# haoyuzhao123/CGRayTracing

Hardware: AMD Instinct MI355X
Metric: Mrays/sec (primary+secondary) at 1920x1080 spp=64 (higher is better)
Workload: dtype f64

## Files before the change

### cgraytracing_amd/_capi.py

```python
from __future__ import annotations

import ctypes as C
import os

import sys

_HERE = os.path.dirname(os.path.abspath(__file__))
CGRT_VERSION = 112
LIB_PATH = os.path.join(_HERE, "libcgrt.so")
if os.environ.get("CGRT_LIB"):
    if os.environ.get("CGRT_DEV_LIBS") == "1":
        LIB_PATH = os.environ["CGRT_LIB"]
        print("cgraytracing_amd: DEVELOPMENT library %s (CGRT_LIB + CGRT_DEV_LIBS=1)" % LIB_PATH, file=sys.stderr)
    else:
        print("cgraytracing_amd: CGRT_LIB ignored (set CGRT_DEV_LIBS=1 to load a development build)", file=sys.stderr)

CGRT_OK = 0
CGRT_NCOUNTERS = 8
CNT_RAYS, CNT_HITPOINTS, CNT_WAVE_ITERS, CNT_NODE_TESTS, CNT_TRI_TESTS = 0, 1, 2, 3, 4


class CgrtError(RuntimeError):
    def __init__(self, code, msg):
        super().__init__("libcgrt error %d: %s" % (code, msg))
# ... 99 lines not shown
    "cgrt_scene_add_mesh_triangles": (C.c_int, [C.c_void_p, C.c_void_p, C.c_int, _DP, C.c_double, C.c_double,
                                                C.c_int]),
    "cgrt_scene_add_bezier": (C.c_int, [C.c_void_p, C.c_void_p, C.c_int, _DP, _DP, C.c_double, C.c_double]),
    "cgrt_scene_commit": (C.c_int, [C.c_void_p, C.c_int]),
    "cgrt_scene_get_stats": (C.c_int, [C.c_void_p, C.POINTER(SceneStats)]),
    "cgrt_scene_tree_sizes": (C.c_int, [C.c_void_p, C.c_int, C.POINTER(C.c_int32), C.POINTER(C.c_int32),
                                        C.POINTER(C.c_int32)]),
    "cgrt_scene_tree_dump": (C.c_int, [C.c_void_p, C.c_int, C.c_void_p, C.c_void_p, C.c_void_p, C.c_void_p]),
    "cgrt_trace_grid": (C.c_int, [C.c_void_p, C.POINTER(Camera), C.POINTER(Grid), C.c_void_p, C.c_void_p,
                                  C.c_void_p, C.c_void_p]),
    "cgrt_unpermute_stripes": (C.c_int, [C.c_void_p, C.c_int, C.c_int, C.c_int, C.c_int, C.c_int, C.c_int, C.c_int, C.c_void_p,
                                         C.c_void_p]),
    "cgrt_trace_grid_host": (C.c_int, [C.c_void_p, C.POINTER(Camera), C.POINTER(Grid), C.c_void_p, C.c_void_p,
                                       C.c_void_p]),
    "cgrt_trace_grid_hitpoints": (C.c_int, [C.c_void_p, C.POINTER(Camera), C.POINTER(Grid), C.c_void_p, C.c_uint64,
                                            C.POINTER(C.c_uint64)]),
    "cgrt_ppm_render": (C.c_int, [C.c_void_p, C.POINTER(Camera), C.POINTER(Grid), C.POINTER(Photons),
                                  C.POINTER(PpmResult)]),
    "cgrt_ppm_session_create": (C.c_int, [C.c_void_p, C.POINTER(Camera), C.POINTER(Grid), C.POINTER(Photons), C.c_int,
                                          C.POINTER(C.c_void_p)]),
    "cgrt_ppm_session_create_rays": (C.c_int, [C.c_void_p, C.POINTER(Rays), C.POINTER(RayPixels), C.POINTER(Photons), C.c_int,
                                               C.POINTER(C.c_void_p)]),
    "cgrt_ppm_session_destroy": (None, [C.c_void_p]),
    "cgrt_ppm_session_add_photons": (C.c_int, [C.c_void_p, C.c_int64]),
    "cgrt_ppm_session_add_photon_rays": (C.c_int, [C.c_void_p, C.POINTER(PhotonRays)]),
    "cgrt_photon_emit": (C.c_int, [C.POINTER(Photons), C.c_int64, C.c_int64, C.c_void_p, C.c_void_p, C.c_void_p, C.c_void_p, C.c_void_p,
                                   C.c_void_p]),
    "cgrt_photon_emit_host": (C.c_int, [C.POINTER(Photons), C.c_int64, C.c_int64, C.c_void_p, C.c_void_p, C.c_void_p, C.c_void_p,
                                        C.c_void_p]),
    "cgrt_photon_ray_events": (C.c_int, [C.c_void_p, C.POINTER(PhotonRays), C.c_uint64, C.c_int64, C.c_int, C.c_void_p, C.c_void_p]),
    "cgrt_ppm_session_image": (C.c_int, [C.c_void_p, C.c_void_p, C.c_void_p]),
    "cgrt_ppm_session_image_device": (C.c_int, [C.c_void_p, C.c_void_p, C.c_void_p, C.c_void_p]),
    "cgrt_ppm_session_hitpoints": (C.c_int, [C.c_void_p, C.c_void_p, C.c_uint64, C.POINTER(C.c_uint64)]),
    "cgrt_ppm_session_get_info": (C.c_int, [C.c_void_p, C.POINTER(PpmSessionInfo)]),
    "cgrt_tonemap_rgb8": (C.c_int, [C.c_int, C.c_void_p, C.c_int, C.c_int, C.c_void_p]),
    "cgrt_write_png": (C.c_int, [C.c_char_p, C.c_int, C.c_int, C.c_void_p]),
    "cgrt_photon_events": (C.c_int, [C.c_void_p, C.POINTER(Photons), C.c_int, C.c_int64, C.c_int32, C.c_void_p,
                                     C.c_void_p]),
    "cgrt_scene_bvh_dump": (C.c_int, [C.c_void_p, C.c_int, C.POINTER(C.c_int32), C.c_void_p, C.c_void_p]),
    "cgrt_scene_bvh_order": (C.c_int, [C.c_void_p, C.c_int, C.POINTER(C.c_int32), C.c_void_p]),
    "cgrt_scene_wide_dump": (C.c_int, [C.c_void_p, C.c_int, C.POINTER(C.c_int32), C.POINTER(C.c_int32), C.c_void_p, C.c_void_p]),
    "cgrt_lens_samples": (C.c_int, [C.c_uint64, C.c_void_p, C.c_void_p, C.c_int, C.c_double, C.c_void_p]),
    "cgrt_surface_colors": (C.c_int, [C.c_void_p, C.c_int, C.c_void_p, C.c_int, C.c_void_p]),
    "cgrt_trace_grid_variant": (C.c_int, [C.c_void_p, C.POINTER(Camera), C.POINTER(Grid), C.c_char_p, C.c_size_t]),
    "cgrt_scene_last_tile_order": (C.c_int, [C.c_void_p, C.c_void_p, C.c_void_p, C.c_void_p, C.c_int64, C.POINTER(C.c_int64)]),
    "cgrt_scene_last_sphere_masks": (C.c_int, [C.c_void_p, C.c_void_p, C.c_int64, C.POINTER(C.c_int64)]),
    "cgrt_scene_last_sure_tiles": (C.c_int, [C.c_void_p, C.c_void_p, C.c_int64, C.POINTER(C.c_int64)]),
    "cgrt_scene_last_sample_relay": (C.c_int, [C.c_void_p, C.POINTER(C.c_int64), C.POINTER(C.c_int32), C.POINTER(C.c_int64)]),
    "cgrt_scene_last_relay_form": (C.c_int, [C.c_void_p, C.POINTER(C.c_int32), C.POINTER(C.c_int32)]),
    "cgrt_relay_start_host": (C.c_int, [C.c_int32, C.c_int32, C.c_int32, C.c_int64, C.c_int32, C.c_int64, C.c_int64, C.c_int64, C.c_void_p,
                                        C.c_void_p, C.c_int32, C.c_int32, C.c_void_p, C.c_int64, C.POINTER(C.c_int64)]),
    "cgrt_scene_last_relay_start": (C.c_int, [C.c_void_p, C.c_void_p, C.c_int64, C.c_void_p, C.c_int64, C.POINTER(C.c_int64),
                                              C.POINTER(C.c_int64), C.POINTER(C.c_int32)]),
    "cgrt_scene_last_lens_stage": (C.c_int, [C.c_void_p, C.POINTER(C.c_int64), C.POINTER(C.c_int64)]),
    "cgrt_scene_last_tile_order_reused": (C.c_int, [C.c_void_p, C.POINTER(C.c_int32)]),
    "cgrt_trace_grid_diffuse_variant": (C.c_int, [C.c_void_p, C.c_void_p, C.c_void_p, C.c_char_p, C.c_size_t]),
    "cgrt_scene_last_diffuse_tiles": (C.c_int, [C.c_void_p, C.POINTER(C.c_int64)]),
    "cgrt_scene_last_inkernel_diffuse_tiles": (C.c_int, [C.c_void_p, C.POINTER(C.c_int64)]),
    "cgrt_trace_rays": (C.c_int, [C.c_void_p, C.POINTER(Rays), C.POINTER(RayResults), C.c_void_p, C.c_void_p]),
    "cgrt_trace_rays_host": (C.c_int, [C.c_void_p, C.POINTER(Rays), C.POINTER(RayResults), C.c_void_p]),
    "cgrt_ray_hit_attributes": (C.c_int, [C.c_void_p, C.POINTER(Rays), C.c_void_p, C.c_void_p, C.POINTER(HitAttributes), C.c_void_p]),
    "cgrt_ray_hit_attributes_host": (C.c_int, [C.c_void_p, C.POINTER(Rays), C.c_void_p, C.c_void_p, C.POINTER(HitAttributes)]),
    "cgrt_trace_rays_variant": (C.c_int, [C.c_void_p, C.POINTER(Rays), C.POINTER(RayResults), C.c_char_p, C.c_size_t]),
    "cgrt_trace_rays_hitpoints": (C.c_int, [C.c_void_p, C.POINTER(Rays), C.c_void_p, C.c_uint64, C.POINTER(C.c_uint64)]),
    "cgrt_occlusion_rays": (C.c_int, [C.c_void_p, C.POINTER(Rays), C.POINTER(Occlusion), C.c_void_p, C.c_void_p]),
    "cgrt_occlusion_rays_host": (C.c_int, [C.c_void_p, C.POINTER(Rays), C.POINTER(Occlusion), C.c_void_p]),
    "cgrt_occlusion_rays_variant": (C.c_int, [C.c_void_p, C.POINTER(Rays), C.c_char_p, C.c_size_t]),
    "cgrt_camera_rays": (C.c_int, [C.POINTER(Camera), C.POINTER(Grid), C.c_void_p, C.c_void_p, C.c_void_p, C.c_void_p]),
    "cgrt_camera_rays_host": (C.c_int, [C.POINTER(Camera), C.POINTER(Grid), C.c_void_p, C.c_void_p, C.c_void_p]),
    "cgrt_intersect_rays": (C.c_int, [C.c_void_p, C.c_int, C.c_void_p, C.c_void_p, C.c_void_p, C.c_int,
                                      C.c_void_p, C.c_void_p, C.c_void_p]),
    "cgrt_math_probe": (C.c_int, [C.c_int, C.c_int, C.c_void_p, C.c_int64, C.c_void_p]),
}

_lib = None


def lib():
    global _lib
    if _lib is None:
        if not os.path.exists(LIB_PATH):
            raise ImportError(
                "cgraytracing_amd: %s not found -- build the HIP library first "
                "(make -C cgraytracing_amd/csrc, or __graft_entry__.build()). There is no CPU fallback." % LIB_PATH)
        try:
            import torch
        except ImportError:
            pass
        L = C.CDLL(LIB_PATH)
        for name, (res, args) in SIGNATURES.items():
            fn = getattr(L, name)
            fn.restype = res
            fn.argtypes = args
        if L.cgrt_version() != CGRT_VERSION:
            raise ImportError("cgraytracing_amd: %s is ABI version %d, this binding needs %d -- rebuild it (make -C cgraytracing_amd/csrc)"
                              % (LIB_PATH, L.cgrt_version(), CGRT_VERSION))
        _lib = L
    return _lib


def check(rc):
    if rc < 0:
        raise CgrtError(rc, lib().cgrt_last_error().decode("utf-8", "replace"))
    return rc
```

### cgraytracing_amd/csrc/cgrt_eye.hpp

```cpp
#ifndef CGRT_EYE_HPP
#define CGRT_EYE_HPP
#include "cgrt_lens_stage.h"
#include "cgrt_scene_walk.hpp"
#include "cgrt_sphere_mask.h"
#include "cgrt_sure_first.h"

struct Pending {
    V3 o, d, adj;
    int32_t depth_left;
    uint32_t path;
};

#ifndef CGRT_DIFF_WAVES
#define CGRT_DIFF_WAVES 8
#endif
#ifndef CGRT_DIFF_DOF_WAVES
#define CGRT_DIFF_DOF_WAVES 6
#endif
static constexpr int kDiffWaves = CGRT_DIFF_WAVES, kDiffDofWaves = CGRT_DIFF_DOF_WAVES;
#ifndef CGRT_BEZ_WAVES
#define CGRT_BEZ_WAVES 2
#endif
static constexpr int kBezWaves = CGRT_BEZ_WAVES;
#ifndef CGRT_TREE_WAVES
#define CGRT_TREE_WAVES 3
#endif
#ifndef CGRT_SCHED_TREE_WAVES
#define CGRT_SCHED_TREE_WAVES CGRT_TREE_WAVES
#endif
static constexpr int kTreeWaves = CGRT_TREE_WAVES;
static constexpr int kSchedTreeWaves = CGRT_SCHED_TREE_WAVES;

__host__ __device__ __forceinline__ void lens_disc(uint64_t k_smp, double &sx, double &sy) {
    uint64_t ctr = k_smp;
    while (true) {
        ctr += kGolden;
        const uint64_t z = fin64(ctr);
        const double ux = div_rand_max((uint32_t)(z >> 33)), uy = div_rand_max((uint32_t)((z >> 2) & 0x7fffffffu));
        sx = ux * 2.0 - 1;
        sy = uy * 2.0 - 1;
        if (sx * sx + sy * sy < 1) break;
    }
}

struct HitpointSink {
    double *rec;
    unsigned long long *count;
    unsigned long long cap;
};

template <int NT>
__device__ __forceinline__ bool wave_has_tile(const GridParams &g, int tile_block, int tile_grid) {
    using TG = TileGeom<NT>;
    const int wave = threadIdx.x >> 6;
    const int wtiles_x = (g.W + kWaveTileW - 1) / kWaveTileW, wtiles_y = (g.rows + kWaveTileH - 1) / kWaveTileH;
    int tile_x, tile_y;
    if (tile_grid < 0) {
        const int tiles_x = (g.W + TG::W - 1) / TG::W;
        tile_x = tile_block % tiles_x;
        tile_y = tile_block / tiles_x;
    } else {
        const int tile_blocks = tile_grid / g.chunks;
        if (!tile_of_block(g, tile_block % tile_blocks, tile_x, tile_y, TG::W, TG::H)) return false;
    }
    const int wx = tile_x * (TG::W / kWaveTileW) + (NT == 256 ? (wave & 1) : 0);
    const int wy = tile_y * (TG::H / kWaveTileH) + (NT == 256 ? (wave >> 1) : 0);
    if (!(wx < wtiles_x && wy < wtiles_y)) return false;
    if (g.hidx && g.hidx[wy * wtiles_x + wx] >= 0) return false;
    if (g.light && (g.light[wy * wtiles_x + wx] != 0) != (g.light_mode != 0)) return false;
    return true;
}

struct RelayWg {
    int slot = -1, chunk = 0, s0 = 0, s1 = 0;
};

template <bool TREES, bool BEZ, bool DOF, bool GLASS, bool SPH, bool STATS, bool HPS, int NT, bool HEAVY, bool SPILL = false, bool HFONLY = false,
          bool DIFF = false, bool PAIR = false, bool PARK = false, bool LSTAGE = false, bool COST = false>
__device__ __forceinline__ void trace_grid_body(const DeviceScene &sc, const GridParams &g, float *__restrict__ rgb,
                                                uint32_t *__restrict__ nhit_out, unsigned long long *__restrict__ counters,
                                                const HitpointSink &hps, int tile_block, int tile_grid, const RelayWg rw = RelayWg{}) {
    using TG = TileGeom<NT>;
    static_assert(!PARK || (PAIR && NT == kRelayThreads), "PARK: a relayed tile's later chunks");
    static_assert(!DIFF || (SPH && !GLASS && !HPS && !HEAVY && !STATS && !SPILL), "DIFF: the sphere loop, first hits only");
    static_assert(!PAIR || (SPH && GLASS && !HPS && !HEAVY && !STATS && !SPILL), "PAIR: the glass sphere variants of the tile order");
    static_assert(!LSTAGE || (DIFF && DOF && !PAIR), "LSTAGE: the thin-lens terminal-diffuse body inside a PAIR launch");
    static_assert(!COST || PAIR, "COST: the PAIR variants with a start table");
    static_assert(!LSTAGE || lens_batch_lds(NT) <= (size_t)kLdsLevels * pending_level_bytes(NT), "the lens batches fit the PAIR launch's pending-ray levels");
    const long long tl_t0 = g.timeline ? wall_clock64() : 0;
    if (!HEAVY && !g.timeline) {
        if (!__syncthreads_or((int)wave_has_tile<NT>(g, tile_block, tile_grid))) return;
    }
    constexpr size_t level_bytes = pending_level_bytes(NT), stack_bytes = (size_t)kLdsLevels * level_bytes;
    constexpr bool WALK = TREES && !HFONLY;
    {
        constexpr WgLds chk = wg_lds(wg_ask_trace(NT, TREES, BEZ, GLASS, SPILL, HFONLY), 3, 5, true);
        static_assert(chk.pending == 0 && chk.objs == (GLASS ? stack_bytes : 0) && chk.staging - chk.objs == 3 * sizeof(ObjRec) &&
                          chk.bez - chk.staging == (SPILL ? (NT / 64) * sizeof(ObjRec) : 0) &&
                          chk.nodes - chk.bez == (BEZ ? (NT / 64) * sizeof(BezLds) : 0) &&
                          chk.wstack - chk.nodes == (WALK ? 5 * sizeof(NodeRec) : 0) && chk.has.nodes == WALK &&
                          chk.has.wstack == (WALK && !GLASS && !BEZ),
                      "trace_grid_body's carve-up and cgrt_wg_lds.h");
    }
    extern __shared__ __align__(16) unsigned char lds_raw[];
    ObjRec *lobjs = reinterpret_cast<ObjRec *>(lds_raw + (GLASS ? stack_bytes : 0));
    unsigned char *lrest = reinterpret_cast<unsigned char *>(lobjs + sc.n_lds);
    LdsAux aux;
    if (SPILL) {
        aux.spill = reinterpret_cast<ObjRec *>(lrest) + (threadIdx.x >> 6);
        lrest += (NT / 64) * sizeof(ObjRec);
    }
    aux.bl = BEZ ? reinterpret_cast<volatile BezLds *>(lrest) + (threadIdx.x >> 6) : nullptr;
    if (BEZ) lrest += (NT / 64) * sizeof(BezLds);
    NodeRec *lnodes = reinterpret_cast<NodeRec *>(lrest);
    aux.lnodes = (WALK && sc.cached_tree >= 0) ? lnodes : nullptr;
    aux.wstack = (WALK && !GLASS && !BEZ && sc.has_wide)
                     ? reinterpret_cast<uint2 *>(lrest + ((sc.cached_tree >= 0 ? (size_t)sc.cached_nodes * sizeof(NodeRec) : 0)))
                     : nullptr;
    if (WALK && sc.cached_tree >= 0) {
        const uint4 *src = reinterpret_cast<const uint4 *>(sc.nodes + sc.trees[sc.cached_tree].node_begin);
        uint4 *dst = reinterpret_cast<uint4 *>(lnodes);
        const int n16 = sc.cached_nodes * (int)(sizeof(NodeRec) / 16);
        for (int k = threadIdx.x; k < n16; k += NT) dst[k] = src[k];
    }

    {
        const uint4 *src = reinterpret_cast<const uint4 *>(sc.objs);
        uint4 *dst = reinterpret_cast<uint4 *>(lobjs);
// ... 22 lines not shown
        live = have_tile && (w < g.W) && (j < g.rows) && (h < g.H);
        const double px = (2.0 * ((double)w / g.W) - 1) * g.half_width;
        const double py = (2.0 * ((double)h / g.H) - 1) * g.half_width * g.H / g.W;
        pdir = normalized(mk(px, py, 0) - camorg);
        pof = pdir * ((g.focus_plane - camorg.z) / pdir.z) + camorg;
        k_pix = pixel_key(g.seed, (uint64_t)h * (uint64_t)g.W + (uint64_t)w);
    };
    if (!heavy) {
        const int nb = tile_block;
        int tile_x, tile_y;
        if (tile_grid < 0) {
            const int tiles_x = (g.W + TG::W - 1) / TG::W;
            tile_x = nb % tiles_x;
            tile_y = nb / tiles_x;
        } else {
            const int tile_blocks = tile_grid / g.chunks;
            chunk = nb / tile_blocks;
            if (!tile_of_block(g, nb % tile_blocks, tile_x, tile_y, TG::W, TG::H)) return;
        }
        wx = tile_x * (TG::W / kWaveTileW) + (NT == 256 ? (wave & 1) : 0);
        wy = tile_y * (TG::H / kWaveTileH) + (NT == 256 ? (wave >> 1) : 0);
        have_tile = wx < wtiles_x && wy < wtiles_y;
        if (have_tile && g.hidx && g.hidx[wy * wtiles_x + wx] >= 0) have_tile = false;
        if (have_tile && g.light && (g.light[wy * wtiles_x + wx] != 0) != (g.light_mode != 0)) have_tile = false;
        s_end = (g.chunks > 1) ? ((chunk + 1) * g.chunk_spp < g.spp ? (chunk + 1) * g.chunk_spp : g.spp) : (PAIR && rw.slot >= 0 ? rw.s1 : g.spp);
        set_pixel(lane & 15, lane >> 4);
    }
    const bool masked = DIFF && g.wmask != nullptr;
    uint32_t smask = 0u;
    if (masked) {
        smask = load_uniform(g.wmask + __builtin_amdgcn_readfirstlane(have_tile ? wy * wtiles_x + wx : 0));
        if (sc.n_lds < 32) smask &= (1u << sc.n_lds) - 1u;
    }
    uint32_t sure = (uint32_t)kSureNone;
    if (DIFF && g.wsure != nullptr && have_tile) {
        const uint32_t wt = (uint32_t)__builtin_amdgcn_readfirstlane(wy * wtiles_x + wx);
        sure = (load_uniform(reinterpret_cast<const uint32_t *>(g.wsure) + (wt >> 2)) >> ((wt & 3u) * 8u)) & 0xffu;
        if (sure >= (uint32_t)sc.n_lds) sure = (uint32_t)kSureNone;
    }
    uint64_t k_smp = 0;

    double acc_r = 0, acc_g = 0, acc_b = 0;
    uint32_t my_hits = 0, my_rays = 0, my_nodes = 0, my_tris = 0, wave_iters = 0;
    uint32_t hp_seq = 0;

    Pending deep[2];
    Pending sib;
    bool sib_valid = false;
    unsigned char *lslot = lds_raw;
    int sp = 0;
    int s = (g.chunks > 1) ? chunk * g.chunk_spp : (PAIR && rw.slot >= 0 ? rw.s0 : 0);
    double *park = nullptr;
    uint32_t park_n = 0;
    if (PARK)
        park = reinterpret_cast<double *>(g.relay + relay_layout((size_t)g.relay_cap, g.relay_k, g.relay_slots).rvals) +
               ((size_t)rw.slot * (size_t)(g.relay_k - 1) + (size_t)(rw.chunk - 1)) * (size_t)g.relay_slots * (3 * NT) + threadIdx.x;
    bool have = false;
    V3 o = camorg, d = pdir, adj = mk(1, 1, 1);
    int depth_left = 0;
    uint32_t path = 1;
    int unit_next = 0, unit_end = 0, hrank = 0;
    int unit_pix = 0, unit_smp = 0, unit_rank = 0;
    bool unit_open = false;
    constexpr bool PRE = HEAVY && TREES && !BEZ && !STATS && !SPILL;
    bool pre_valid = false;
    double pre_len = 0;
    int32_t pre_tri = -1;

    const bool staging = LSTAGE && g.lens_batch != 0;
    uint64_t *const lens_slot = reinterpret_cast<uint64_t *>(lrest) + threadIdx.x;
    static_assert(lens_slot_at(1, 0, NT) == NT * sizeof(uint64_t) && lens_slot_at(0, 1, NT) == sizeof(uint64_t), "lens_slot's strides");
    int batch_first = 0, batch_end = 0;
    auto stage_lens = [&](int first, int count) {
        uint32_t rejected = 0u;
        for (int b = 0; b < count; b++) {
            const LensSlot a = lens_stage_first(k_pix, (uint64_t)(g.sample_offset + first + b));
            lens_slot[b * NT] = a.v;
            rejected |= a.done ? 0u : (1u << b);
        }
        if (!live) rejected = 0u;
        while (__ballot(rejected != 0u) != 0ull) {
            if (rejected != 0u) {
                const int b = __ffs((int)rejected) - 1;
                const LensSlot a = lens_stage_retry(lens_slot[b * NT]);
                lens_slot[b * NT] = a.v;
                if (a.done) rejected &= rejected - 1u;
            }
        }
        batch_first = first;
        batch_end = first + count;
    };
    auto start_sample = [&](int smp) {
        if (LSTAGE && staging) {
            double sx, sy;
            lens_point(lens_slot[(smp - batch_first) * NT], sx, sy);
            o = camorg + mk(sx, sy, 0) * g.lens_radius;
            d = normalized(pof - o);
            k_smp = 0;
        } else if (DOF) {
            k_smp = sample_key(k_pix, (uint64_t)(g.sample_offset + smp));
            double sx, sy;
            lens_disc(k_smp, sx, sy);
            o = camorg + mk(sx, sy, 0) * g.lens_radius;
            d = normalized(pof - o);
        } else {
            k_smp = sample_key(k_pix, (uint64_t)(g.sample_offset + smp));
            o = camorg;
            d = pdir;
        }
// ... 92 lines not shown
            if (!have && live && s < s_end) {
                start_sample(s);
                s++;
            }
            if (__ballot(have) == 0ull) break;
        }
        wave_iters++;
        UTILP(heavy ? 0 : 11, have);
        RayKey rk{k_smp, path, false, 0u};
        if (PRE) {
            rk.pre_valid = have && pre_valid;
            rk.pre_obj = g.prim_obj;
            rk.pre_len = pre_len;
            rk.pre_tri = pre_tri;
            rk.pre_counter = pre_tri >= 0 ? 1 : 0;
            pre_valid = false;
        }
        const SceneHit hit =
            intersect_scene<TREES, BEZ, SPH, STATS, SPILL, PRE, HFONLY, !SPH, PAIR, DIFF>(lobjs, sc.n_lds, sc.n_objs, sc, o, d, rk, have, aux, my_nodes, my_tris,
                                                                                          masked, smask);
        if (have) {
            my_rays++;
            have = false;
            if (hit.id >= 0) {
                const ObjMat ob = load_mat<SPILL>(lobjs, sc.n_lds, sc.objs, hit.id);
                V3 P = o, n = d, n_old = d;
                bool into = true;
                auto surface = [&]() {
                    P = o + d * hit.t;
                    n = SPH ? normalized(P - load_centre<SPILL>(lobjs, sc.n_lds, sc.objs, hit.id)) : hit.n;
                    n_old = n;
                    into = true;
                    if (dot(n, d) > 0) {
                        n = -n;
                        into = false;
                    }
                };
                if (!SPH) surface();
                V3 f = ob.col;
                if (!SPH && ob.kind == KIND_PLANE && ob.tex >= 0) {
                    V3 c;
                    if (texture_color(sc.texs[ob.tex], sc.texels, P, c)) f = c;
                }
                const double refl = ob.refl, transp = ob.transp;
                if (DIFF || (refl < kEps && transp < kEps)) {
                    UTIL(heavy ? 7 : 12);
                    const V3 hf = DIFF ? f : mulv(f, adj);
                    if (heavy) {
                        double *q = g.dvals + ((((size_t)unit_rank * g.spp + unit_smp) * g.maxhp + hp_seq) * 64 + unit_pix) * 3;
                        q[0] = hf.x;
                        q[1] = hf.y;
                        q[2] = hf.z;
                    } else if (PARK) {
                        if (park_n < (uint32_t)g.relay_slots) {
                            double *q = park + (size_t)park_n * (3 * NT);
                            q[0] = hf.x;
                            q[NT] = hf.y;
                            q[2 * NT] = hf.z;
                        }
                        park_n++;
                    } else {
                        acc_r += hf.x;
                        acc_g += hf.y;
                        acc_b += hf.z;
                    }
                    my_hits++;
                    if (HPS && SPH) surface();
                    if (HPS) {
                        const unsigned long long here = __ballot(true);
                        unsigned long long base = 0ull;
                        if (lane == (int)__ffsll((long long)here) - 1) base = atomicAdd(hps.count, (unsigned long long)__popcll(here));
                        base = (unsigned long long)__shfl((long long)base, (int)__ffsll((long long)here) - 1);
                        const unsigned long long k = base + (unsigned long long)__popcll(here & lanes_below);
                        if (k < hps.cap) {
                            double *q = hps.rec + 10 * k;
                            q[0] = hf.x; q[1] = hf.y; q[2] = hf.z;
                            q[3] = P.x; q[4] = P.y; q[5] = P.z;
                            q[6] = n.x; q[7] = n.y; q[8] = n.z;
                            q[9] = (double)((((unsigned long long)(s - 1) * (unsigned long long)g.W * g.rows +
                                              (unsigned long long)j * g.W + w) << 4) | (unsigned long long)hp_seq);
                        }
                    }
                    if (HPS || heavy) hp_seq++;
                } else if (depth_left > 1) {
                    if (SPH) surface();
                    if (transp < kEps) {
                        const V3 nd = d - n * 2.0 * dot(n, d);
                        adj = mulv(f, adj) * refl;
                        o = P + n * kEps;
                        d = nd;
                        depth_left--;
                        path = path * 2;
                        have = true;
                    } else if (GLASS) {
                        UTIL(heavy ? 8 : 13);
                        const double nc = 1.0, nt = 1.33;
                        const double nnt = into ? nc / nt : nt / nc;
                        const double ddn = dot(d, n);
                        const V3 refl_dir = d - n_old * 2.0 * dot(n_old, d);
                        const double cos2t = 1 - nnt * nnt * (1 - ddn * ddn);
                        if (cos2t < 0) {
                            o = P + n * kEps;
                            d = refl_dir;
                        } else {
                            const V3 refr_dir =
                                normalized(d * nnt - n_old * ((into ? 1 : -1) * (ddn * nnt + sqrt_cr(cos2t))));
                            const double a = nt - nc, b = nt + nc, R0 = a * a / (b * b);
// ... 38 lines not shown
                d = sib.d;
                adj = sib.adj;
                depth_left = sib.depth_left;
                path = sib.path;
                sib_valid = false;
                have = true;
            }
            if (GLASS && !have && sp > 0) {
                UTIL(heavy ? 10 : 14);
                --sp;
                if (sp < kLdsLevels) {
                    const double *q = reinterpret_cast<const double *>(lslot + sp * level_bytes) + threadIdx.x;
                    o = mk(q[0 * NT], q[1 * NT], q[2 * NT]);
                    d = mk(q[3 * NT], q[4 * NT], q[5 * NT]);
                    adj = mk(q[6 * NT], q[7 * NT], q[8 * NT]);
                    const uint32_t meta = reinterpret_cast<const uint32_t *>(
                        lslot + sp * level_bytes + kPendDoubles * NT * sizeof(double))[threadIdx.x];
                    depth_left = (int)(meta >> 8);
                    path = meta & 0xffu;
                } else {
                    const Pending &pe = deep[sp - kLdsLevels];
                    o = pe.o;
                    d = pe.d;
                    adj = pe.adj;
                    depth_left = pe.depth_left;
                    path = pe.path;
                }
                have = true;
            }
        }
    }

    if (g.probe) {
        if (lane == 0 && have_tile) {
            const long long dt = (long long)clock64() - cost_t0;
            const uint32_t wt = (uint32_t)(wy * wtiles_x + wx);
            g.cost[wt] = (COST && g.probe == 2) ? wave_iters : dt > 0 ? (dt < 0xffffffffll ? (uint32_t)dt : 0xffffffffu) : 1u;
        }
        return;
    }
    if (heavy) {
    } else if (g.chunks > 1) {
        if (have_tile && (w < g.W) && (j < g.rows)) {
            const size_t px = ((size_t)chunk * g.rows + (size_t)j) * g.W + (size_t)w;
            g.partial[3 * px + 0] = acc_r;
            g.partial[3 * px + 1] = acc_g;
            g.partial[3 * px + 2] = acc_b;
            if (g.partial_nhit) g.partial_nhit[px] = my_hits;
        }
    } else {
        uint32_t px_hits = my_hits;
        bool store = true;
        if (PAIR && rw.slot >= 0) {
            const size_t slot = (size_t)rw.slot, k = (size_t)g.relay_k;
            const RelayLayout rl = relay_layout((size_t)g.relay_cap, g.relay_k, g.relay_slots);
            uint32_t *arrive = reinterpret_cast<uint32_t *>(g.relay) + slot;
            double *racc = reinterpret_cast<double *>(g.relay + rl.racc) + slot * (3 * NT) + threadIdx.x;
            uint32_t *rhits = reinterpret_cast<uint32_t *>(g.relay + rl.rhits) + slot * k * NT + threadIdx.x;
            uint32_t *rcount = reinterpret_cast<uint32_t *>(g.relay + rl.rcount) + slot * (k - 1) * NT + threadIdx.x;
            if (PARK) {
                rcount[(size_t)(rw.chunk - 1) * NT] = park_n;
            } else {
                racc[0] = acc_r;
                racc[NT] = acc_g;
                racc[2 * NT] = acc_b;
            }
            rhits[(size_t)rw.chunk * NT] = my_hits;
            __shared__ unsigned int relay_last;
            asm volatile("s_waitcnt vmcnt(0)" ::: "memory");
            __syncthreads();
            if (threadIdx.x == 0) {
                __builtin_amdgcn_fence(__ATOMIC_RELEASE, "agent");
                asm volatile("s_waitcnt vmcnt(0)" ::: "memory");
                const unsigned int ticket = __hip_atomic_fetch_add(arrive, 1u, __ATOMIC_RELAXED, __HIP_MEMORY_SCOPE_AGENT);
                const bool last = ticket == (unsigned int)g.relay_k - 1u;
                if (last) {
                    __builtin_amdgcn_fence(__ATOMIC_ACQUIRE, "agent");
                    asm volatile("s_waitcnt vmcnt(0)" ::: "memory");
                    __hip_atomic_store(arrive, 0u, __ATOMIC_RELAXED, __HIP_MEMORY_SCOPE_AGENT);
                }
                relay_last = last ? 1u : 0u;
            }
            __syncthreads();
            store = relay_last != 0u;
            if (store) {
                acc_r = racc[0];
                acc_g = racc[NT];
                acc_b = racc[2 * NT];
                px_hits = rhits[0];
                for (int c = 1; c < g.relay_k; c++) {
                    px_hits += rhits[(size_t)c * NT];
                    uint32_t n = rcount[(size_t)(c - 1) * NT];
                    if (n > (uint32_t)g.relay_slots) n = (uint32_t)g.relay_slots;
                    uint32_t n_max = n;
                    for (int off = 32; off > 0; off >>= 1) {
                        const uint32_t o2 = (uint32_t)__shfl_xor((int)n_max, off);
                        n_max = o2 > n_max ? o2 : n_max;
                    }
                    n_max = (uint32_t)__builtin_amdgcn_readfirstlane((int)n_max);
                    const double *q = reinterpret_cast<const double *>(g.relay + rl.rvals) +
                                      (slot * (k - 1) + (size_t)(c - 1)) * (size_t)g.relay_slots * (3 * NT) + threadIdx.x;
                    for (uint32_t i0 = 0; i0 < n_max; i0 += kRelayBatch) {
                        double v[kRelayBatch][3];
#pragma unroll
                        for (int u = 0; u < kRelayBatch; u++) {
                            v[u][0] = q[(size_t)(i0 + u) * (3 * NT)];
                            v[u][1] = q[(size_t)(i0 + u) * (3 * NT) + NT];
                            v[u][2] = q[(size_t)(i0 + u) * (3 * NT) + 2 * NT];
                        }
#pragma unroll
                        for (int u = 0; u < kRelayBatch; u++) {
                            if (i0 + u < n) {
                                acc_r += v[u][0];
                                acc_g += v[u][1];
                                acc_b += v[u][2];
                            }
                        }
                    }
                }
            }
        }
        const float v0 = (float)(acc_r * g.inv_spp_total), v1 = (float)(acc_g * g.inv_spp_total),
                    v2 = (float)(acc_b * g.inv_spp_total);
#pragma unroll
        for (int k = 0; k < 3; k++) {
            const int idx = k * 64 + lane;
            const int row = idx / (kWaveTileW * 3), c = idx % (kWaveTileW * 3);
            const int src = row * kWaveTileW + c / 3, ch = c % 3;
            const float a0 = __shfl(v0, src), a1 = __shfl(v1, src), a2 = __shfl(v2, src);
            const float v = ch == 0 ? a0 : (ch == 1 ? a1 : a2);
            const int jj = wy * kWaveTileH + row, ww = wx * kWaveTileW + c / 3;
            if (store && have_tile && jj < g.rows && ww < g.W) {
                float *dst = rgb + ((size_t)jj * g.W + ww) * 3 + ch;
                *dst = g.accumulate ? *dst + v : v;
            }
        }
        if (store && nhit_out && have_tile && (w < g.W) && (j < g.rows)) nhit_out[(size_t)j * g.W + w] = px_hits;
    }

    if (g.timeline) {
        __shared__ unsigned int tl_rays;
        if (threadIdx.x == 0) tl_rays = 0;
        __syncthreads();
        atomicAdd(&tl_rays, my_rays);
        __syncthreads();
        if (threadIdx.x == 0) {
            unsigned long long *q = g.timeline + 4 * (size_t)blockIdx.x;
            const unsigned hw = __builtin_amdgcn_s_getreg((31 << 11) | 4), xcc = __builtin_amdgcn_s_getreg((3 << 11) | 20);
            if (q[0] == 0ull) q[0] = (unsigned long long)tl_t0;
            q[1] = (unsigned long long)wall_clock64();
            q[2] = (unsigned long long)hw | ((unsigned long long)xcc << 32);
            q[3] = ((unsigned long long)(wx & 0xffff) | ((unsigned long long)(wy & 0xffff) << 16)) + ((q[3] >> 32) << 32) + ((unsigned long long)tl_rays << 32);
        }
    }
    if (counters) {
        unsigned long long r = my_rays, hh = my_hits, nn = my_nodes, tt = my_tris;
        for (int off = 32; off > 0; off >>= 1) {
            r += __shfl_xor(r, off);
            hh += __shfl_xor(hh, off);
            if (STATS) {
                nn += __shfl_xor(nn, off);
                tt += __shfl_xor(tt, off);
            }
        }
        if (lane == 0 && (r | (unsigned long long)wave_iters) != 0ull) {
            atomicAdd(&counters[CGRT_CNT_RAYS], r);
            atomicAdd(&counters[CGRT_CNT_HITPOINTS], hh);
            atomicAdd(&counters[CGRT_CNT_WAVE_ITERS], (unsigned long long)wave_iters);
            if (STATS) {
                atomicAdd(&counters[CGRT_CNT_NODE_TESTS], nn);
                atomicAdd(&counters[CGRT_CNT_TRI_TESTS], tt);
            }
        }
    }
}

__device__ __forceinline__ unsigned long long *wg_counters_begin(unsigned long long *wg, const unsigned long long *counters) {
    if (!counters) return nullptr;
    if (threadIdx.x < CGRT_NCOUNTERS) wg[threadIdx.x] = 0ull;
    __syncthreads();
    return wg;
}
__device__ __forceinline__ void wg_counters_end(const unsigned long long *wg, unsigned long long *counters) {
    if (!counters) return;
    __syncthreads();
    if (threadIdx.x < CGRT_NCOUNTERS && wg[threadIdx.x] != 0ull) atomicAdd(&counters[threadIdx.x], wg[threadIdx.x]);
}

template <bool TREES, bool BEZ, bool DOF, bool GLASS, bool SPH, bool STATS, bool HPS = false, int NT = 256, bool SPILL = false, bool HFONLY = false,
          bool DIFF = false, bool PAIR = false, bool START = false>
__global__ __launch_bounds__(NT, DIFF ? (DOF ? kDiffDofWaves : kDiffWaves) : BEZ ? kBezWaves : ((TREES && !HFONLY) ? kTreeWaves : 4)) void trace_grid_kernel(DeviceScene sc, GridParams g, float *__restrict__ rgb,
                                                             uint32_t *__restrict__ nhit_out,
                                                             unsigned long long *__restrict__ counters,
                                                             HitpointSink hps = HitpointSink{nullptr, nullptr, 0}) {
    int tile_block = (int)blockIdx.x, tile_grid = (int)gridDim.x;
    unsigned entry = blockIdx.x;
    RelayWg rw;
    if (g.tile_order) {
        if (g.tile_order == kOrderFull || g.tile_order == kOrderDiffuse) {
            const unsigned first_diffuse = load_uniform(g.plan + 3);
            if (g.tile_order == kOrderDiffuse) entry += first_diffuse;
            if (g.tile_order == kOrderDiffuse ? entry >= load_uniform(g.plan + kOrderClasses) : entry >= first_diffuse) return;
        } else if (PAIR && g.relay_k > 1) {
            const unsigned n_tiles = load_uniform(g.plan + kOrderClasses);
            const unsigned n01 = load_uniform(g.plan + 2), n012 = load_uniform(g.plan + 3);
            RelayBlock rb{n_tiles, 0, false};
            bool tabled = false;
            if (START && g.relay_start_at != 0u) {
                const unsigned n_split = relay_split_entries(n01, n012, (unsigned)g.relay_cap, g.relay_extent);
                tabled = blockIdx.x < n012 + ((unsigned)g.relay_k - 1u) * n_split;
                if (tabled) {
                    rb = relay_start_block(load_uniform(g.plan + g.relay_start_at + blockIdx.x), n_split);
                    if (rb.chunk >= g.relay_k) return;
                }
            }
            if (!tabled) rb = relay_block_ordered(blockIdx.x, (unsigned)g.relay_k, n01, n012, n_tiles, (unsigned)g.relay_cap, g.relay_extent, g.relay_order);
            entry = rb.entry;
            if (entry >= n_tiles) return;
            if (rb.split) {
                rw.slot = (int)entry;
                rw.chunk = rb.chunk;
                rw.s0 = relay_first_sample(rb.chunk, g.relay_chunk_spp);
                rw.s1 = relay_end_sample(rb.chunk, g.relay_chunk_spp, g.spp);
            }
        }
        tile_block = (int)load_uniform(g.border + entry);
        tile_grid = -1;
    }
    __shared__ unsigned long long wg_cnt[CGRT_NCOUNTERS];
    unsigned long long *wc = wg_counters_begin(wg_cnt, counters);
    if (PAIR && g.tile_order == kOrderAllDiffuse && entry >= load_uniform(g.plan + 3))
        trace_grid_body<false, false, DOF, false, true, false, false, NT, false, false, false, true, false, false, DOF>(sc, g, rgb, nhit_out, wc, hps, tile_block, tile_grid);
    else if (PAIR && rw.chunk > 0)
        trace_grid_body<TREES, BEZ, DOF, GLASS, SPH, STATS, HPS, NT, false, SPILL, HFONLY, DIFF, PAIR, PAIR, false, START>(sc, g, rgb, nhit_out, wc, hps, tile_block, tile_grid, rw);
    else
        trace_grid_body<TREES, BEZ, DOF, GLASS, SPH, STATS, HPS, NT, false, SPILL, HFONLY, DIFF, PAIR, false, false, START>(sc, g, rgb, nhit_out, wc, hps, tile_block, tile_grid, rw);
    wg_counters_end(wg_cnt, counters);
}
template <bool TREES, bool BEZ, bool DOF, bool GLASS, bool SPH, bool STATS, int NT = 256>
__global__ __launch_bounds__(NT, BEZ ? kBezWaves : (TREES ? kSchedTreeWaves : 4)) void trace_grid_sched_kernel(DeviceScene sc, GridParams g,
                                                                                         float *__restrict__ rgb,
                                                                                         uint32_t *__restrict__ nhit_out,
                                                                                         unsigned long long *__restrict__ counters) {
    const HitpointSink none{nullptr, nullptr, 0};
    const bool heavy_first = (int)blockIdx.x < g.heavy_blocks;
    __shared__ unsigned long long wg_cnt[CGRT_NCOUNTERS];
    unsigned long long *wc = wg_counters_begin(wg_cnt, counters);
    if (NT == 64) {
        if (heavy_first)
            trace_grid_body<TREES, BEZ, DOF, GLASS, SPH, STATS, false, NT, true>(sc, g, rgb, nhit_out, wc, none, 0, 1);
        else
            trace_grid_body<TREES, BEZ, DOF, GLASS, SPH, STATS, false, NT, false>(sc, g, rgb, nhit_out, wc, none,
                                                                                  (int)blockIdx.x - g.heavy_blocks,
                                                                                  (int)gridDim.x - g.heavy_blocks);
        wg_counters_end(wg_cnt, counters);
        return;
    }
    const bool queued = g.border != nullptr;
    __shared__ unsigned tile_entry;
    for (int phase = 0; phase < 2; phase++) {
        if ((phase == 0) == heavy_first) {
            if (queued || heavy_first)
                trace_grid_body<TREES, BEZ, DOF, GLASS, SPH, STATS, false, NT, true>(sc, g, rgb, nhit_out, wc, none, 0, 1);
        } else {
            const unsigned n_entries = queued ? load_uniform(g.plan + 3) : (heavy_first ? 0u : 1u);
            unsigned served = 0;
            while (true) {
                unsigned e = served++;
                if (queued) {
                    __syncthreads();
                    if (threadIdx.x == 0) tile_entry = atomicAdd(&g.plan[4], 1u);
                    __syncthreads();
                    e = tile_entry;
                }
                if (e >= n_entries) break;
                trace_grid_body<TREES, BEZ, DOF, GLASS, SPH, STATS, false, NT, false>(
// ... 140 lines not shown
__global__ __launch_bounds__(256) void sure_first_kernel(GridParams g, DeviceScene sc, int tiles_x, const unsigned char *__restrict__ tcls,
                                                         const uint32_t *__restrict__ wmask, unsigned char *__restrict__ wsure) {
    const int wtiles_x = (g.W + kWaveTileW - 1) / kWaveTileW, wtiles_y = (g.rows + kWaveTileH - 1) / kWaveTileH;
    const int wt = blockIdx.x * blockDim.x + threadIdx.x;
    if (wt >= wtiles_x * wtiles_y) return;
    const int wx = wt % wtiles_x, wy = wt / wtiles_x;
    int win = -1;
    if (tcls[(wy / (kTileH / kWaveTileH)) * tiles_x + wx / (kTileW / kWaveTileW)] == 3) {
        const TileRays tr = wave_tile_rays(g, wx, wy);
        const ObjRec *objs = sc.objs;
        win = sphere_sure_first(g, tr, sc.n_objs, [objs](int i) { return SureSphere{vec3d(objs[i].a[0], objs[i].a[1], objs[i].a[2]), objs[i].s0}; },
                                wmask[wt]);
    }
    wsure[wt] = (unsigned char)(win >= 0 ? win : kSureNone);
}

struct RelayStartArgs {
    RelayItems r;
    uint32_t tiles_x, wtiles_x, wtiles_y;
};
__device__ __forceinline__ RelayItems relay_items_of(const RelayStartArgs &a, const uint32_t *plan) {
    RelayItems r = a.r;
    r.n01 = plan[2];
    r.n012 = plan[3];
    r.n_tiles = plan[kOrderClasses];
    return r;
}
__global__ __launch_bounds__(kRelayThreads) void relay_weight_kernel(RelayStartArgs a, const uint32_t *__restrict__ plan, const uint32_t *__restrict__ list,
                                                                     const uint32_t *__restrict__ wcost, unsigned long long *__restrict__ weight) {
    const RelayItems r = relay_items_of(a, plan);
    const uint32_t i = blockIdx.x * kRelayThreads + threadIdx.x;
    if (i >= relay_items_total(r)) return;
    const RelayBlock b = relay_item(i, r);
    weight[i] = relay_item_weight(b, relay_tile_cost(wcost, list[b.entry], a.tiles_x, a.wtiles_x, a.wtiles_y), r);
}
__global__ __launch_bounds__(kRelayThreads) void relay_start_kernel(RelayStartArgs a, const uint32_t *__restrict__ plan,
                                                                    const unsigned long long *__restrict__ weight, uint32_t *__restrict__ start) {
    const RelayItems r = relay_items_of(a, plan);
    const uint32_t t = relay_items_total(r), i = blockIdx.x * kRelayThreads + threadIdx.x;
    if (blockIdx.x * kRelayThreads >= t) return;
    __shared__ unsigned long long w_s[kRelayThreads];
    const unsigned long long wi = i < t ? weight[i] : 0ull;
    uint32_t rank = 0;
    for (uint32_t j0 = 0; j0 < t; j0 += kRelayThreads) {
        __syncthreads();
        if (j0 + threadIdx.x < t) w_s[threadIdx.x] = weight[j0 + threadIdx.x];
        __syncthreads();
        const uint32_t n = min((uint32_t)kRelayThreads, t - j0);
        for (uint32_t u = 0; u < n; u++) rank += relay_item_before(w_s[u], j0 + u, wi, i) ? 1u : 0u;
    }
    if (i < t) start[rank] = relay_start_word(relay_item(i, r));
}

__global__ __launch_bounds__(1024) void plan_kernel(const uint32_t *__restrict__ cost_in, const unsigned char *__restrict__ light, int n,
                                                    unsigned kmax, unsigned long long divisor, uint32_t *__restrict__ plan,
                                                    uint32_t *__restrict__ order, int32_t *__restrict__ hidx,
                                                    uint32_t *__restrict__ border, int wtiles_x, int wtiles_y, int tw, int th) {
    auto cost = [&](int i) -> uint32_t { return (light && light[i]) ? 0u : cost_in[i]; };
    __shared__ unsigned long long part[1024];
    __shared__ unsigned base_s, hist[128];
    __shared__ unsigned long long thr_s;
    auto bin_of = [](uint32_t c) { return c < 4u ? (int)c : (31 - __clz((int)c)) * 4 + (int)((c >> (29 - __clz((int)c))) & 3u); };
    if (threadIdx.x < 128) hist[threadIdx.x] = 0;
    __syncthreads();
    unsigned long long t = 0;
    for (int i = threadIdx.x; i < n; i += 1024) {
        const uint32_t c = cost(i);
        t += c;
        atomicAdd(&hist[bin_of(c)], 1u);
    }
    part[threadIdx.x] = t;
    __syncthreads();
    for (int off = 512; off > 0; off >>= 1) {
        if ((int)threadIdx.x < off) part[threadIdx.x] += part[threadIdx.x + off];
        __syncthreads();
    }
    if (threadIdx.x == 0) {
        unsigned long long thr = part[0] / divisor;
        if (thr < 1) thr = 1;
        unsigned above = 0;
        int b = 127;
        for (; b >= 0; b--) {
            if (above + hist[b] > kmax) break;
            above += hist[b];
        }
        if (b >= 0) {
            const unsigned long long edge = b < 4 ? (unsigned long long)b
                                                  : (((4ull + (unsigned long long)(b & 3) + 1ull) << (b / 4)) >> 2) - 1ull;
            if (edge > thr) thr = edge;
        }
        thr_s = thr;
        base_s = 0;
    }
    __syncthreads();
    const unsigned long long thr = thr_s;
    if (threadIdx.x == 0) {
        unsigned off = 0;
        for (int b = 127; b >= 0; b--) {
            const unsigned long long lo = b < 4 ? (unsigned long long)b : ((4ull + (unsigned long long)(b & 3)) << (b / 4)) >> 2;
            const unsigned c = hist[b];
            if (lo > thr) {
                hist[b] = off;
                off += c;
            } else {
                hist[b] = 0xffffffffu;
            }
// ... 200 lines not shown
```

### cgraytracing_amd/csrc/cgrt_frame.h

```cpp
#ifndef CGRT_FRAME_H
#define CGRT_FRAME_H
#include <algorithm>
#include <cmath>
#include <cstddef>
#include <cstdint>
#include <cstdio>
#include <cstdlib>
#include <string>

#include "../../include/cgrt.h"
#include "cgrt_lens_stage.h"
#include "cgrt_relay.h"

struct GridParams {
    int32_t W, H, rows, row_offset, stripe_rows, stripe_rank, stripe_nranks;
    int32_t spp, sample_offset, max_depth;
    int32_t accumulate;
    int32_t xcd_tiles;
    int32_t chunks, chunk_spp;
    double *partial;
    uint32_t *partial_nhit;
    const unsigned char *light;
    int32_t light_mode, tile_order;
    const uint32_t *wmask;
    const uint32_t *order;
    const uint32_t *border;
    uint32_t *cost;
    const int32_t *hidx;
    uint32_t *plan;
    double *dvals;
    unsigned char *dcnt;
    double *pconst;
    int32_t probe, heavy_blocks, items_per_tile, units_per_item, maxhp;
    const double *prim_len;
    const int32_t *prim_tri;
    int32_t prim_obj;
    int32_t prim_done;
    int32_t pw_refill, pw_rounds;
    unsigned long long *timeline;
    double inv_spp_total;
    uint64_t seed;
    double cam[3], half_width, focus_plane, lens_radius;
    unsigned char *relay;
    int32_t relay_k, relay_chunk_spp, relay_cap, relay_slots;
    int32_t relay_extent, relay_order;
    int32_t lens_batch;
    uint32_t relay_start_at;
    const unsigned char *wsure;
};
static_assert(sizeof(GridParams) == 336, "GridParams is a kernel argument: its layout is fixed");

static constexpr int kTileW = 32, kTileH = 8, kThreads = 256;
static constexpr int kOrderSpheresMax = 16, kOrderClasses = 4, kOrderPlanWords = 8, kOrderArrived = 5;
static constexpr int kOrderAll = 1, kOrderFull = 2, kOrderDiffuse = 3, kOrderAllDiffuse = 4;
struct OrderSpheres {
    double s[kOrderSpheresMax][4];
    uint32_t n, transp;
};
static constexpr size_t align256(size_t b) { return (b + 255) & ~(size_t)255; }
struct Region {
    size_t at, bytes;
    template <class T> T *in(unsigned char *base) const { return bytes ? reinterpret_cast<T *>(base + at) : nullptr; }
};
struct TileOrderLayout {
    Region plan{}, list{}, tile_cls{}, wave_cls{}, wmask{}, wsure{};
    Region wcost{}, weight{}, start{};
    size_t total = 0;
};
inline TileOrderLayout tile_order_layout(size_t n_tiles, size_t n_wt, bool sure = false, size_t start_words = 0) {
    TileOrderLayout L;
    size_t end = 0;
    const auto take = [&end](size_t bytes) { end += bytes; return Region{end - bytes, bytes}; };
    L.plan = take(kOrderPlanWords * sizeof(uint32_t));
    L.list = take(n_tiles * sizeof(uint32_t));
    end = align256(end);
    L.tile_cls = take(n_tiles);
    end = align256(end);
    L.wave_cls = take(n_wt);
    end = align256(end);
    L.wmask = take(n_wt * sizeof(uint32_t));
    if (sure) {
        end = align256(end);
        L.wsure = take(n_wt);
    }
    if (start_words) {
        end = align256(end);
        L.wcost = take(n_wt * sizeof(uint32_t));
        end = align256(end);
        L.weight = take(start_words * sizeof(uint64_t));
        end = align256(end);
        L.start = take(start_words * sizeof(uint32_t));
    }
    L.total = align256(end);
    return L;
}
static constexpr int kSphereMaskMax = 32;
inline bool order_all_special(const OrderSpheres &sp, const cgrt_camera &cam) {
    for (uint32_t i = 0; i < sp.n; i++) {
        double r = sp.s[i][3] * (1 + 1e-9) + 1e-6;
        if (cam.lens_radius > 0) {
            const double f = cam.focus_plane - cam.cam[2];
            const double s_lo = (sp.s[i][2] - r - cam.cam[2]) / f, s_hi = (sp.s[i][2] + r - cam.cam[2]) / f;
            if (!(f > 0) || !(s_lo > 0) || !(cam.cam[2] < 0)) return true;
            r += cam.lens_radius * std::max(std::fabs(1 - s_lo), std::fabs(1 - s_hi));
        }
        const double vx = sp.s[i][0] - cam.cam[0], vy = sp.s[i][1] - cam.cam[1], vz = sp.s[i][2] - cam.cam[2];
        if (!(std::sqrt(vx * vx + vy * vy + vz * vz) > r)) return true;
    }
    return false;
}
static constexpr int kWaveTileW = 16, kWaveTileH = 4;
static constexpr int kXcds = 8, kSuperW = 4, kSuperH = 4, kSuperTiles = kSuperW * kSuperH;

inline int tile_grid_blocks(int W, int rows, bool xcd_tiles, int tile_w = kTileW, int tile_h = kTileH) {
    const int tiles_x = (W + tile_w - 1) / tile_w, tiles_y = (rows + tile_h - 1) / tile_h;
    if (!xcd_tiles) return tiles_x * tiles_y;
    const int sx = (tiles_x + kSuperW - 1) / kSuperW, sy = (tiles_y + kSuperH - 1) / kSuperH;
    const int nsuper = sx * sy;
    return ((nsuper + kXcds - 1) / kXcds) * kXcds * kSuperTiles;
}

inline GridParams grid_params(const cgrt_camera *cam, const cgrt_grid *grid) {
    GridParams g{};
    g.W = grid->width;
    g.H = grid->height;
    g.rows = grid->rows;
    g.row_offset = grid->row_offset;
    g.stripe_rows = grid->stripe_rows;
    g.stripe_rank = grid->stripe_rank;
    g.stripe_nranks = grid->stripe_nranks;
    g.spp = grid->spp;
    g.sample_offset = grid->sample_offset;
    g.max_depth = grid->max_depth;
    g.accumulate = (grid->flags & CGRT_GRID_ACCUMULATE) ? 1 : 0;
    g.inv_spp_total = 1.0 / (double)grid->spp_total;
    g.seed = grid->seed;
    for (int k = 0; k < 3; k++) g.cam[k] = cam->cam[k];
    g.half_width = cam->half_width;
    g.focus_plane = cam->focus_plane;
    g.lens_radius = cam->lens_radius;
    g.chunks = 1;
    g.chunk_spp = grid->spp;
    g.items_per_tile = 1;
    g.units_per_item = 256;
    g.maxhp = 16;
    g.prim_obj = -1;
    g.pw_refill = 16;
    g.pw_rounds = 8;
    return g;
}

struct EyeKnobs {
    bool force_reorder = false;
    long long defer_bytes = 0;
    int heavy_div = 32, units_per_item = 256;
    bool no_primwalk = false, pw_no_finish = false;
    int pw_refill = 16, pw_rounds = 8;
    int lds_pad = 0;
    bool no_hfonly = false, no_tile_queue = false, plan_dump = false;
    bool no_sure_tiles = false;
    bool no_order_reuse = false;
    int relay_chunks = kRelayDefaultChunks;
    long long relay_tiles = 0;
    int relay_mirror = -1;
    int relay_order = -1;
    int relay_start = -1;
    int relay_probe_spp = kRelayProbeSpp;
    int lens_stage = -1;
    const char *timeline_file = nullptr;
};
inline const char *env_str(const char *name) { const char *e = std::getenv(name); return e ? e : ""; }
inline bool env_on(const char *name) { const char *e = env_str(name); return *e && *e != '0'; }
inline int env_positive(const char *name, int def) { const int v = std::atoi(env_str(name)); return v > 0 ? v : def; }
inline int relay_order_named(const char *e) {
    const std::string v(e);
    if (v == "chunks_first" || v == "0") return kRelayChunksFirst;
    if (v == "mirror_first" || v == "1") return kRelayMirrorFirst;
    if (v == "interleaved" || v == "2") return kRelayInterleaved;
    return -1;
}
inline int relay_start_named(const char *e) {
    const std::string v(e);
    if (v == "list" || v == "0") return kRelayStartList;
    if (v == "cost" || v == "1") return kRelayStartCost;
    return -1;
}
static constexpr int kLensStageOff = 0, kLensStageLds = 1;
static constexpr int kLensStageDefault = kLensStageLds;
inline int lens_stage_named(const char *e) {
    const std::string v(e);
    if (v == "off" || v == "0") return kLensStageOff;
    if (v == "lds" || v == "1") return kLensStageLds;
    return -1;
}
inline EyeKnobs eye_knobs() {
    static const EyeKnobs once = [] {
        EyeKnobs k;
        k.force_reorder = env_on("CGRT_FORCE_REORDER");
        k.defer_bytes = std::atoll(env_str("CGRT_DEFER_BYTES"));
        k.heavy_div = env_positive("CGRT_HEAVY_DIV", 32);
        k.units_per_item = (env_positive("CGRT_UNITS_PER_ITEM", 256) + 63) / 64 * 64;
        k.no_primwalk = env_on("CGRT_NO_PRIMWALK");
        k.pw_no_finish = env_on("CGRT_PW_NO_FINISH");
        k.pw_refill = env_positive("CGRT_PW_REFILL", 16);
        k.pw_rounds = env_positive("CGRT_PW_ROUNDS", 8);
        k.lds_pad = std::atoi(env_str("CGRT_LDS_PAD"));
        k.no_hfonly = env_on("CGRT_NO_HFONLY");
        k.no_tile_queue = env_on("CGRT_NO_TILE_QUEUE");
        k.plan_dump = env_on("CGRT_PLAN_DUMP");
        k.no_order_reuse = env_on("CGRT_NO_ORDER_REUSE");
        k.no_sure_tiles = env_on("CGRT_NO_SURE_TILES");
        k.relay_chunks = std::min(std::max(env_positive("CGRT_RELAY_CHUNKS", kRelayDefaultChunks), 2), kRelayMaxChunks);
        k.relay_tiles = std::atoll(env_str("CGRT_RELAY_TILES"));
        if (*env_str("CGRT_RELAY_MIRROR")) k.relay_mirror = env_on("CGRT_RELAY_MIRROR") ? 1 : 0;
        k.relay_order = relay_order_named(env_str("CGRT_RELAY_ORDER"));
        k.relay_start = relay_start_named(env_str("CGRT_RELAY_START"));
        if (k.relay_start < 0 && *env_str("CGRT_RELAY_START"))
            std::fprintf(stderr, "cgrt: CGRT_RELAY_START=%s names no start order of this library (list, cost): the default is used\n", env_str("CGRT_RELAY_START"));
        {
            const int ps = std::atoi(env_str("CGRT_RELAY_PROBE_SPP"));
            if (ps == 1 || ps == 2 || ps == 4) k.relay_probe_spp = ps;
        }
        k.lens_stage = lens_stage_named(env_str("CGRT_LENS_STAGE"));
        if (k.lens_stage < 0 && *env_str("CGRT_LENS_STAGE"))
            std::fprintf(stderr, "cgrt: CGRT_LENS_STAGE=%s names no form of this library (off, lds): the default is used\n", env_str("CGRT_LENS_STAGE"));
        return k;
    }();
    EyeKnobs k = once;
    k.timeline_file = *env_str("CGRT_TIMELINE_FILE") ? env_str("CGRT_TIMELINE_FILE") : nullptr;
    return k;
}

struct FrameInputs {
    cgrt_grid grid;
    cgrt_camera cam;
    bool sched, spill, stats, glass;
    int nt;
    bool has_mesh, has_bezier, prim_finish, light_ok;
    int prim_obj;
    EyeKnobs knobs;
    size_t mem_total;
    int n_cu, waves_per_simd;
    bool image = false, sph = false, pair = false;
    bool order_ok = false, aux_stream = false, all_spheres = false;
    int n_objs = 0, n_lds = 0;
    bool all_special = false;
};

struct ScratchLayout {
    Region partial{}, partial_nhit{}, cost{}, order{}, hidx{}, border{}, plan{}, light{}, dvals{}, dcnt{}, pconst{}, prim_len{}, prim_tri{};
    size_t total = 0;
    void place(GridParams &g, unsigned char *base, bool nhit) const {
        g.partial = partial.in<double>(base);
        g.partial_nhit = nhit ? partial_nhit.in<uint32_t>(base) : nullptr;
        g.cost = cost.in<uint32_t>(base);
        g.order = order.in<uint32_t>(base);
        g.hidx = hidx.in<int32_t>(base);
        g.border = border.in<uint32_t>(base);
        g.plan = plan.in<uint32_t>(base);
        g.light = light.in<unsigned char>(base);
        g.dvals = dvals.in<double>(base);
        g.dcnt = dcnt.in<unsigned char>(base);
        g.pconst = pconst.in<double>(base);
        g.prim_len = prim_len.in<double>(base);
        g.prim_tri = prim_tri.in<int32_t>(base);
    }
};

struct TileOrderPlan {
    bool on = false;
    enum Class3 { None, SecondLaunch, InKernel } class3 = None;
    bool masks = false;
    bool sure = false;
    int lens_stage = kLensStageOff;
};

struct FramePlan {
    int chunks = 1, chunk_spp = 0;
    bool xcd_tiles = false;
    int maxhp = 1;
    int tile_blocks = 0;
    size_t grid_dim = 0;
    int wtiles_x = 0, wtiles_y = 0;
    size_t n_wt = 0, tile_bytes = 0, kmax = 0;
    bool use_prim = false;
    bool split_light = false, tile_queue = false, prim_done = false;
    int wave_slots = 0, items_per_tile = 1, heavy_blocks = 0;
    unsigned long long plan_div = 0;
    ScratchLayout scratch;
    TileOrderPlan order;
    int relay_k = 1, relay_chunk_spp = 0, relay_slots = 0;
    size_t relay_tile_bytes = 0, relay_cap = 0, relay_bytes = 0;
    int relay_extent = kRelayGlass, relay_order = kRelayChunksFirst;
    int relay_start = kRelayStartList, relay_probe_spp = 0;
    size_t relay_start_words = 0;
};

inline bool relay_engaged(int32_t flags, int32_t spp, size_t n_tiles, int n_cu) {
    if ((flags & CGRT_GRID_NO_SAMPLE_RELAY) || spp < 2 * kRelayMinChunkSpp) return false;
    return (flags & CGRT_GRID_SAMPLE_RELAY) || n_tiles >= (size_t)4 * (size_t)n_cu;
}

static constexpr int kRelayDefaultExtent = kRelayMirror, kRelayDefaultOrder = kRelayInterleaved;
inline int relay_extent_of(int32_t flags, const EyeKnobs &kn) {
    if (flags & CGRT_GRID_RELAY_MIRROR) return kRelayMirror;
    if (flags & CGRT_GRID_RELAY_NO_MIRROR) return kRelayGlass;
    if (kn.relay_mirror >= 0) return kn.relay_mirror ? kRelayMirror : kRelayGlass;
    return (flags & CGRT_GRID_SAMPLE_RELAY) ? kRelayGlass : kRelayDefaultExtent;
}
inline int relay_order_of(int32_t flags, const EyeKnobs &kn) {
    const int32_t f = flags & CGRT_GRID_RELAY_ORDER_MASK;
    if (f) return f == CGRT_GRID_RELAY_MIRROR_FIRST ? kRelayMirrorFirst : f == CGRT_GRID_RELAY_INTERLEAVED ? kRelayInterleaved : kRelayChunksFirst;
    if (kn.relay_order >= 0) return kn.relay_order;
    return (flags & CGRT_GRID_SAMPLE_RELAY) ? kRelayChunksFirst : kRelayDefaultOrder;
}

inline int relay_start_of(int32_t flags, const EyeKnobs &kn) {
    if (flags & CGRT_GRID_NO_RELAY_COST_START) return kRelayStartList;
    if (flags & CGRT_GRID_RELAY_COST_START) return kRelayStartCost;
    if (kn.relay_start >= 0) return kn.relay_start;
    const bool names_order = (flags & CGRT_GRID_RELAY_ORDER_MASK) || kn.relay_order >= 0;
    return !names_order && !(flags & CGRT_GRID_SAMPLE_RELAY) ? kRelayStartCost : kRelayStartList;
}

inline FramePlan frame_plan(const FrameInputs &in, size_t kmax) {
    const cgrt_grid &gr = in.grid;
    const EyeKnobs &kn = in.knobs;
    FramePlan p;
    p.chunk_spp = gr.spp;
    p.xcd_tiles = !in.spill && in.has_mesh && !in.has_bezier;
    p.maxhp = in.glass ? 16 : 1;
    const size_t npx = (size_t)gr.rows * gr.width;
    if ((gr.flags & CGRT_GRID_SPLIT_SAMPLES) && gr.spp >= 32 && !in.spill) {
        int chunks = std::min(gr.spp / 16, 16);
        while (chunks > 1 && (size_t)chunks * npx * 28 > ((size_t)4 << 30)) chunks--;
        if (chunks > 1) {
            p.chunk_spp = (gr.spp + chunks - 1) / chunks;
            p.chunks = (gr.spp + p.chunk_spp - 1) / p.chunk_spp;
        }
    }
    const bool one_wave = in.nt == 64;
    const int waves_per_block = in.nt / 64;
    p.tile_blocks = one_wave ? tile_grid_blocks(gr.width, gr.rows, false, kWaveTileW, kWaveTileH)
                             : tile_grid_blocks(gr.width, gr.rows, p.xcd_tiles);
    p.grid_dim = (size_t)p.tile_blocks * p.chunks;
    TileOrderPlan &o = p.order;
    const bool split_asked = (gr.flags & CGRT_GRID_SPLIT_SAMPLES) != 0;
    o.on = in.image && p.chunks == 1 && !p.xcd_tiles && in.nt == kThreads && in.order_ok && !(gr.flags & CGRT_GRID_NO_TILE_ORDER);
    if (o.on && !in.all_special) {
        if (in.sph && !in.spill && !in.stats && in.aux_stream && (gr.flags & CGRT_GRID_DIFFUSE_TILES) && !split_asked && !kn.timeline_file)
            o.class3 = TileOrderPlan::SecondLaunch;
        else if (in.pair)
            o.class3 = TileOrderPlan::InKernel;
    }
    o.masks = o.class3 != TileOrderPlan::None && in.all_spheres && in.n_objs <= kSphereMaskMax && in.n_objs == in.n_lds &&
              !(gr.flags & CGRT_GRID_NO_SPHERE_MASKS);
    o.sure = o.masks && !(gr.flags & CGRT_GRID_NO_SURE_TILES) && !kn.no_sure_tiles;
    if (o.class3 == TileOrderPlan::InKernel && in.cam.lens_radius > 0 && !(gr.flags & CGRT_GRID_NO_LENS_STAGE))
        o.lens_stage = kn.lens_stage >= 0 ? kn.lens_stage : kLensStageDefault;
    if (o.on && in.pair && o.class3 != TileOrderPlan::SecondLaunch && !split_asked &&
        relay_engaged(gr.flags, gr.spp, (size_t)p.tile_blocks, in.n_cu)) {
        const RelayChunks rc = relay_chunks(gr.spp, (gr.flags & CGRT_GRID_SAMPLE_RELAY_4) ? kRelayMaxChunks : kn.relay_chunks);
        if (rc.k > 1) {
            p.relay_slots = relay_slots(rc.chunk_spp, gr.max_depth);
            p.relay_tile_bytes = relay_tile_bytes(rc.k, p.relay_slots);
            p.relay_cap = relay_cap((size_t)p.tile_blocks, rc.k, p.relay_slots, relay_budget(in.mem_total), kn.relay_tiles);
            if (p.relay_cap > 0) {
                p.relay_k = rc.k;
                p.relay_chunk_spp = rc.chunk_spp;
                p.relay_bytes = relay_layout(p.relay_cap, rc.k, p.relay_slots).total;
                p.relay_extent = relay_extent_of(gr.flags, kn);
                p.relay_order = relay_order_of(gr.flags, kn);
                p.relay_start = (size_t)p.tile_blocks < kRelayStartMaxTiles ? relay_start_of(gr.flags, kn) : kRelayStartList;
                if (p.relay_start == kRelayStartCost) {
                    p.relay_probe_spp = std::min(kn.relay_probe_spp, (int)gr.spp);
                    p.relay_start_words = relay_start_words((size_t)p.tile_blocks, rc.k, p.relay_cap);
                }
            }
        }
    }
    p.wtiles_x = (gr.width + kWaveTileW - 1) / kWaveTileW;
    p.wtiles_y = (gr.rows + kWaveTileH - 1) / kWaveTileH;
    p.n_wt = (size_t)p.wtiles_x * p.wtiles_y;
    p.use_prim = in.sched && in.prim_obj >= 0 && !kn.no_primwalk && !(gr.flags & CGRT_GRID_STATS);
    const size_t units = (size_t)gr.spp * 64;
    const size_t vals = units * (size_t)p.maxhp * 3 * sizeof(double), cnt = (units + 7) & ~(size_t)7, pconst = 7 * 64 * sizeof(double),
                 plen = p.use_prim ? units * sizeof(double) : 0, ptri = p.use_prim ? units * sizeof(int32_t) : 0;
    p.tile_bytes = vals + cnt + pconst + plen + ptri;
    p.kmax = in.sched ? kmax : 0;

    ScratchLayout &L = p.scratch;
    size_t end = 0;
    const auto take = [&end](size_t bytes, bool used = true) { end += bytes; return Region{end - bytes, used ? bytes : 0}; };
    if (p.chunks > 1) {
        L.partial = take((size_t)p.chunks * npx * 3 * sizeof(double));
        L.partial_nhit = take((size_t)p.chunks * npx * sizeof(uint32_t));
    }
    L.total = end = align256(end);
    if (!in.sched) return p;
    const size_t np = (p.n_wt + 8) * sizeof(uint32_t), sched_bytes = align256(4 * np + 64 * sizeof(uint32_t) + align256(p.n_wt));
    L.total += sched_bytes + (p.kmax ? p.kmax * p.tile_bytes + 256 : 0);
    if (p.kmax == 0) return p;
    p.split_light = in.light_ok && p.chunks == 1 && !in.stats;
    p.tile_queue = p.chunks == 1 && !one_wave && !kn.no_tile_queue;
    p.prim_done = p.use_prim && in.prim_finish && !kn.pw_no_finish;
    p.wave_slots = in.n_cu * 4 * in.waves_per_simd;
    p.plan_div = (unsigned long long)p.wave_slots * (unsigned long long)kn.heavy_div;
    p.items_per_tile = (int)((units + kn.units_per_item - 1) / kn.units_per_item);
    const size_t fill = (size_t)p.wave_slots / waves_per_block;
    p.heavy_blocks = (int)std::min((p.kmax * (size_t)p.items_per_tile + waves_per_block - 1) / waves_per_block, fill);
    if (p.tile_queue) p.grid_dim = fill;
    const size_t sched_at = end;
    L.cost = take(np);
    L.order = take(np);
    L.hidx = take(np);
    L.border = take(np, p.tile_queue);
    L.plan = take(64 * sizeof(uint32_t));
    L.light = take(p.n_wt, p.split_light);
    end = sched_at + sched_bytes;
    L.dvals = take(p.kmax * vals);
    L.dcnt = take(p.kmax * cnt);
    L.pconst = take(p.kmax * pconst);
    L.prim_len = take(p.kmax * plen);
    L.prim_tri = take(p.kmax * ptri);
    return p;
}

inline size_t max_heavy_tiles(const FrameInputs &in) {
    if (!in.sched) return 0;
// ... 31 lines not shown
```

### cgraytracing_amd/csrc/cgrt_hip.hip

```cpp
#include <hip/hip_runtime.h>

#include <algorithm>
#include <atomic>
#include <chrono>
#include <cmath>
#include <cstdio>
#include <cstdlib>
#include <cstring>
#include <exception>
#include <map>
#include <mutex>
#include <string>
#include <type_traits>
#include <vector>

#include "../../include/cgrt.h"
#include "cgrt_build.h"
#include "cgrt_rng.hpp"
#include "cgrt_types.h"

#include "cgrt_device_math.hpp"
#include "cgrt_grid.hpp"
#include "cgrt_traverse.hpp"
#include "cgrt_bezier.hpp"
// ... 752 lines not shown
    in.pair = L.k.pair;
    in.order_ok = s->order.ok;
    in.aux_stream = s->aux_stream != nullptr;
    in.all_spheres = d.all_spheres != 0;
    in.n_objs = d.n_objs;
    in.n_lds = d.n_lds;
    in.all_special = order_all_special(s->order.spheres, *cam);
    return in;
}

static int probe_and_plan(const cgrt_scene *s, const EyeLaunch &L, const EyeKnobs &kn, const FramePlan &p, const GridParams &g,
                          unsigned char *scratch, hipStream_t st, float *rgb, uint32_t *nhit, unsigned long long *cnt) {
    const ScratchLayout &at = p.scratch;
    unsigned char *light = at.light.in<unsigned char>(scratch);
    if (light)
        hipLaunchKernelGGL(classify_kernel, dim3((unsigned)((p.n_wt + 255) / 256)), dim3(256), 0, st, s->dev, g, light, (int)p.n_wt);
    GridParams gp = g;
    gp.spp = gp.chunks = gp.chunk_spp = 1;
    gp.probe = 1;
    gp.cost = at.cost.in<uint32_t>(scratch);
    gp.light = light;
    int rc = launch_eye(L, false, s->device, gp, dim3((unsigned)p.tile_blocks), st, nullptr, nullptr, nullptr);
    if (rc) return rc;
    if (light) {
        GridParams gl = g;
        gl.light = light;
        gl.light_mode = 1;
        gl.xcd_tiles = 0;
        HIP_TRY(hipEventRecord(s->ev_fork, st));
        HIP_TRY(hipStreamWaitEvent(s->aux_stream, s->ev_fork, 0));
        if ((rc = launch_eye(light_launch(s->dev, L.k.dof, kn), false, s->device, gl,
                             dim3((unsigned)tile_grid_blocks(g.W, g.rows, false)), s->aux_stream, rgb, nhit, cnt)))
            return rc;
        HIP_TRY(hipEventRecord(s->ev_join, s->aux_stream));
    }
    const int tw = L.k.nt == 64 ? 1 : kTileW / kWaveTileW, th = L.k.nt == 64 ? 1 : kTileH / kWaveTileH;
    hipLaunchKernelGGL(plan_kernel, dim3(1), dim3(1024), 0, st, gp.cost, light, (int)p.n_wt, (unsigned)p.kmax, p.plan_div,
                       at.plan.in<uint32_t>(scratch), at.order.in<uint32_t>(scratch), at.hidx.in<int32_t>(scratch),
                       at.border.in<uint32_t>(scratch), p.wtiles_x, p.wtiles_y, tw, th);
    return CGRT_OK;
}

static EyeLaunch start_twin(EyeLaunch L) {
    L.k.start = true;
    return L;
}
static int relay_cost_start(const cgrt_scene *s, const EyeLaunch &L, const FramePlan &p, GridParams &g, hipStream_t st) {
    TileOrderState &o = s->order;
    const TileOrderLayout &at = o.at;
    unsigned char *base = reinterpret_cast<unsigned char *>(o.buf.p);
    uint32_t *wcost = at.wcost.in<uint32_t>(base), *start = at.start.in<uint32_t>(base);
    unsigned long long *weight = at.weight.in<unsigned long long>(base);
    if (!wcost || !start || !weight) return CGRT_OK;
    const TileOrderState::CostKey ck{g.seed, g.max_depth, p.relay_probe_spp};
    const TileOrderState::TableKey tk{g.spp, g.relay_k, g.relay_chunk_spp, g.relay_cap, g.relay_extent, 0};
    const bool have_cost = o.reused && o.cost_valid && std::memcmp(&ck, &o.cost_key, sizeof(ck)) == 0;
    const bool have_table = have_cost && o.table_valid && std::memcmp(&tk, &o.table_key, sizeof(tk)) == 0;
    o.cost_valid = o.table_valid = false;
    if (!have_cost) {
        HIP_TRY(hipMemsetAsync(wcost, 0, at.wcost.bytes, st));
        GridParams gp = g;
        gp.probe = 2;
        gp.cost = wcost;
        gp.spp = gp.chunk_spp = p.relay_probe_spp;
        gp.sample_offset = 0;
        gp.accumulate = 0;
        gp.tile_order = kOrderFull;
        gp.relay = nullptr;
        gp.relay_k = 0;
        gp.relay_start_at = 0;
        if (int rc = launch_eye(start_twin(L), false, s->device, gp, dim3((unsigned)p.grid_dim), st, nullptr, nullptr, nullptr)) return rc;
    }
    if (!have_table) {
        const int tiles_x = (g.W + kTileW - 1) / kTileW;
        const RelayStartArgs a{RelayItems{(uint32_t)g.relay_k, 0, 0, 0, (uint32_t)g.relay_cap, g.relay_extent, g.relay_chunk_spp, g.spp},
                               (uint32_t)tiles_x, (uint32_t)p.wtiles_x, (uint32_t)p.wtiles_y};
        const dim3 grid((unsigned)((p.relay_start_words + kRelayThreads - 1) / kRelayThreads));
        hipLaunchKernelGGL(relay_weight_kernel, grid, dim3(kRelayThreads), 0, st, a, g.plan, g.border, wcost, weight);
        hipLaunchKernelGGL(relay_start_kernel, grid, dim3(kRelayThreads), 0, st, a, g.plan, weight, start);
    }
    if (o.valid && (have_table || (hipPeekAtLastError() == hipSuccess && hipEventRecord(o.ev, st) == hipSuccess))) {
        if (!have_table) o.stream = st;
        o.cost_key = ck;
        o.table_key = tk;
        o.cost_valid = o.table_valid = true;
    } else if (o.valid) {
        (void)hipGetLastError();
        o.valid = false;
    }
    g.relay_start_at = (uint32_t)((at.start.at - at.plan.at) / sizeof(uint32_t));
    o.start_words = p.relay_start_words;
    o.start_wtiles = p.n_wt;
    o.start_reused = have_table;
    return CGRT_OK;
}

static int primary_walk(const cgrt_scene *s, const EyeLaunch &L, const GridParams &g, hipStream_t st, unsigned long long *cnt) {
    PrimWalkArgs pw;
    pw.len = const_cast<double *>(g.prim_len);
    pw.tri = const_cast<int32_t *>(g.prim_tri);
    pw.obj = s->dev.prim_obj;
    pw.tree = s->host.objs[(size_t)s->dev.prim_obj].tree;
    pw.finish = g.prim_done;
    pw.pad_ = 0;
    pw.counters = cnt;
    const size_t staged = (size_t)(pw.finish ? s->dev.n_objs : pw.obj + 1);
    return launch_checked(L.k.dof ? &primary_walk_kernel<true> : &primary_walk_kernel<false>, "primary_walk_kernel", s->device,
                          dim3((unsigned)s->n_cu * 4), dim3(kThreads), primary_walk_lds(staged), st, s->dev, g, pw);
}

static int write_timeline(const char *file, const DevBuf &tl, size_t n_blocks, const GridParams &g, int nt, hipStream_t st) {
    std::vector<unsigned long long> rec(n_blocks * 4);
    HIP_TRY(hipStreamSynchronize(st));
    HIP_TRY(hipMemcpy(rec.data(), tl.p, rec.size() * 8, hipMemcpyDeviceToHost));
    if (FILE *f = std::fopen(file, "wb")) {
        const unsigned long long form = (unsigned long long)g.relay_k | (unsigned long long)g.relay_extent << 8 | (unsigned long long)g.relay_order << 9;
        const unsigned long long head[4] = {n_blocks, (unsigned long long)nt, (unsigned long long)g.chunks,
                                            g.relay_k > 1 ? (form << 32 | (unsigned long long)g.relay_cap) : (unsigned long long)g.xcd_tiles};
        std::fwrite(head, 8, 4, f);
        std::fwrite(rec.data(), 8, rec.size(), f);
        std::fclose(f);
    }
    return CGRT_OK;
}
static int dump_plan(const FramePlan &p, const GridParams &g, hipStream_t st) {
    uint32_t pl[8] = {0};
    HIP_TRY(hipStreamSynchronize(st));
    HIP_TRY(hipMemcpy(pl, g.plan, sizeof(pl), hipMemcpyDeviceToHost));
    std::fprintf(stderr, "cgrt plan: wave tiles %zu, heavy %u (capacity %zu), cost threshold %u, tile-queue entries %u, items per tile %d, prim walk %s\n",
                 p.n_wt, pl[0], p.kmax, pl[1], pl[3], g.items_per_tile, g.prim_len ? "on" : "off");
    return CGRT_OK;
}

extern "C" {

int cgrt_trace_grid_variant(const cgrt_scene *s, const cgrt_camera *cam, const cgrt_grid *grid, char *name, size_t cap) {
    int rc = check_grid(s, cam, grid);
    if (rc) return rc;
    if (!name || cap == 0) return fail(CGRT_ERR_INVALID, "null name buffer");
    ON_DEVICE(s->device);
    const EyeLaunch L = eye_launch(s, cam, grid, eye_knobs(), (grid->flags & CGRT_GRID_HITPOINTS) != 0);
    const EyeFlags &k = L.k;
    const bool sched = L.form == EyeForm::Sched;
    std::snprintf(name, cap, "trace_grid_%skernel<TREES=%d,BEZ=%d,DOF=%d,GLASS=%d,SPH=%d,STATS=%d,%s%sNT=%d%s>", sched ? "sched_" : "",
                  (int)k.trees, (int)k.bez, (int)k.dof, (int)k.glass, (int)k.sph, (int)k.stats,
                  sched ? "" : (k.hps ? "HPS=1," : "HPS=0,"), k.pair ? "PAIR=1," : "", k.nt, k.spill ? ",SPILL=1" : "");
    return CGRT_OK;
}

int cgrt_trace_grid(const cgrt_scene *s, const cgrt_camera *cam, const cgrt_grid *grid, float *rgb, uint32_t *nhit,
                    uint64_t *counters, void *stream) {
    int rc = check_grid(s, cam, grid);
    if (rc) return rc;
    if (!rgb) return fail(CGRT_ERR_INVALID, "null rgb");
    hipStream_t st = reinterpret_cast<hipStream_t>(stream);
    auto *cnt = reinterpret_cast<unsigned long long *>(counters);
    ON_DEVICE(s->device);
    const EyeKnobs kn = eye_knobs();
    const EyeLaunch L = eye_launch(s, cam, grid, kn, false);
    const FrameInputs in = frame_inputs(s, cam, grid, L, kn);
    FramePlan p;
    if ((rc = fit_scratch(s, in, p))) return rc;
    GridParams g = frame_params(in, p);
    unsigned char *scratch = reinterpret_cast<unsigned char *>(s->scratch.p);
    if (p.heavy_blocks > 0 && (rc = probe_and_plan(s, L, kn, p, g, scratch, st, rgb, nhit, cnt))) return rc;
    p.scratch.place(g, scratch, nhit != nullptr);
    size_t n_blocks = (size_t)p.heavy_blocks + p.grid_dim;
    TileOrderGuard guard(s->order, s->relay);
    if (p.order.on) {
        const Capturing capturing = stream_capturing(st);
        if ((rc = order_tiles(s->order, s->dev, p, g, kn.no_order_reuse, capturing, st))) return rc;
        if (p.relay_k > 1 && relay_prepare(s->relay, p, g, capturing, st)) {
            guard.relayed = true;
            n_blocks = relay_grid(p.grid_dim, p.relay_k, p.relay_cap);
            if (p.relay_start == kRelayStartCost && (rc = relay_cost_start(s, L, p, g, st))) return rc;
        }
    }
    DevBuf timeline;
    if (kn.timeline_file) {
        HIP_TRY(timeline.alloc(n_blocks * 32));
        HIP_TRY(hipMemsetAsync(timeline.p, 0, n_blocks * 32, st));
        g.timeline = timeline.as<unsigned long long>();
    }
    if (p.heavy_blocks > 0) {
        hipLaunchKernelGGL(pixel_const_kernel, dim3((unsigned)p.kmax), dim3(64), 0, st, g);
        if (g.prim_len && (rc = primary_walk(s, L, g, st, cnt))) return rc;
        if ((rc = launch_eye(L, true, s->device, g, dim3((unsigned)n_blocks), st, rgb, nhit, cnt))) return rc;
    } else if (p.order.class3 == TileOrderPlan::SecondLaunch) {
        const EyeLaunch DL = diffuse_launch(s->dev, L.k.dof);
        if ((rc = check_eye(DL, s->device))) return rc;
        GridParams gd = g;
        g.tile_order = kOrderFull;
        gd.tile_order = kOrderDiffuse;
        HIP_TRY(hipEventRecord(s->ev_fork, st));
        if ((rc = launch_eye(L, false, s->device, g, dim3((unsigned)n_blocks), st, rgb, nhit, cnt))) return rc;
        HIP_TRY(hipStreamWaitEvent(s->aux_stream, s->ev_fork, 0));
        if ((rc = launch_eye(DL, false, s->device, gd, dim3((unsigned)n_blocks), s->aux_stream, rgb, nhit, cnt))) return rc;
        HIP_TRY(hipEventRecord(s->ev_join, s->aux_stream));
    } else {
        if (p.order.class3 == TileOrderPlan::InKernel) g.tile_order = kOrderAllDiffuse;
        if ((rc = launch_eye(g.relay_start_at ? start_twin(L) : L, false, s->device, g, dim3((unsigned)n_blocks), st, rgb, nhit, cnt))) return rc;
    }
    if (p.chunks > 1)
        hipLaunchKernelGGL(finalize_chunks_kernel, dim3((unsigned)(((size_t)g.rows * g.W + 255) / 256)), dim3(256), 0, st, g, rgb, nhit);
    if (p.heavy_blocks > 0) hipLaunchKernelGGL(deferred_sum_kernel, dim3((unsigned)p.kmax), dim3(64), 0, st, g, rgb, nhit);
    if (g.light || p.order.class3 == TileOrderPlan::SecondLaunch) HIP_TRY(hipStreamWaitEvent(st, s->ev_join, 0));
    const hipError_t launch_err = hipGetLastError();
    if (g.timeline && launch_err == hipSuccess && (rc = write_timeline(kn.timeline_file, timeline, n_blocks, g, L.k.nt, st))) return rc;
    if (launch_err != hipSuccess) return fail(CGRT_ERR_DEVICE, std::string("kernel launch: ") + hipGetErrorString(launch_err));
    if ((rc = guard.commit(g, st))) return rc;
    return kn.plan_dump && g.plan && !g.tile_order ? dump_plan(p, g, st) : CGRT_OK;
}

#define NEED_COMMITTED(s, args_ok)                                           \
    if (!(s) || !(args_ok)) return fail(CGRT_ERR_INVALID, "null argument"); \
    if (!(s)->committed) return fail(CGRT_ERR_INVALID, "scene not committed")

int cgrt_scene_last_tile_order(const cgrt_scene *s, uint32_t *plan5, uint32_t *list, uint8_t *cls, int64_t cap, int64_t *n_tiles) {
    NEED_COMMITTED(s, n_tiles);
    ON_DEVICE(s->device);
    return last_tile_order(s->order, plan5, list, cls, cap, n_tiles);
}
int cgrt_scene_last_sphere_masks(const cgrt_scene *s, uint32_t *masks, int64_t cap, int64_t *n_wave_tiles) {
    NEED_COMMITTED(s, n_wave_tiles);
    ON_DEVICE(s->device);
    return last_sphere_masks(s->order, masks, cap, n_wave_tiles);
}
int cgrt_scene_last_sure_tiles(const cgrt_scene *s, uint8_t *sure, int64_t cap, int64_t *n_wave_tiles) {
    NEED_COMMITTED(s, n_wave_tiles);
    ON_DEVICE(s->device);
    return last_sure_tiles(s->order, sure, cap, n_wave_tiles);
}
int cgrt_scene_last_tile_order_reused(const cgrt_scene *s, int32_t *reused) {
    NEED_COMMITTED(s, reused);
    *reused = s->order.reused ? 1 : 0;
    return CGRT_OK;
}
int cgrt_scene_last_diffuse_tiles(const cgrt_scene *s, int64_t *n_tiles) {
    NEED_COMMITTED(s, n_tiles);
    ON_DEVICE(s->device);
    return last_class3_tiles(s->order, TileOrderPlan::SecondLaunch, n_tiles);
}
int cgrt_scene_last_inkernel_diffuse_tiles(const cgrt_scene *s, int64_t *n_tiles) {
    NEED_COMMITTED(s, n_tiles);
    ON_DEVICE(s->device);
    return last_class3_tiles(s->order, TileOrderPlan::InKernel, n_tiles);
}
int cgrt_scene_last_lens_stage(const cgrt_scene *s, int64_t *lds_tiles, int64_t *area_tiles) {
    NEED_COMMITTED(s, lds_tiles && area_tiles);
    ON_DEVICE(s->device);
    return last_lens_stage(s->order, lds_tiles, area_tiles);
}
int cgrt_scene_last_sample_relay(const cgrt_scene *s, int64_t *tiles, int32_t *chunks, int64_t *parked_values) {
    NEED_COMMITTED(s, tiles && chunks && parked_values);
    ON_DEVICE(s->device);
    return last_sample_relay(s->order, s->relay, tiles, chunks, parked_values);
}
int cgrt_scene_last_relay_form(const cgrt_scene *s, int32_t *mirror, int32_t *order) {
    NEED_COMMITTED(s, mirror && order);
    last_relay_form(s->order, s->relay, mirror, order);
    return CGRT_OK;
}

int cgrt_scene_last_relay_start(const cgrt_scene *s, uint32_t *start, int64_t start_cap, uint32_t *wcost, int64_t cost_cap, int64_t *t,
                                int64_t *n_wave_tiles, int32_t *reused) {
    NEED_COMMITTED(s, t && n_wave_tiles && reused);
    ON_DEVICE(s->device);
    return last_relay_start(s->order, s->relay, start, start_cap, wcost, cost_cap, t, n_wave_tiles, reused);
}

int cgrt_trace_grid_diffuse_variant(const cgrt_scene *s, const cgrt_camera *cam, const cgrt_grid *grid, char *name, size_t cap) {
    int rc = check_grid(s, cam, grid);
    if (rc) return rc;
    if (!name || cap == 0) return fail(CGRT_ERR_INVALID, "null name buffer");
    ON_DEVICE(s->device);
    const EyeKnobs kn = eye_knobs();
    const EyeLaunch L = eye_launch(s, cam, grid, kn, false);
    name[0] = 0;
    if (frame_plan(frame_inputs(s, cam, grid, L, kn), 0).order.class3 == TileOrderPlan::SecondLaunch)
        diffuse_name(diffuse_launch(s->dev, L.k.dof), name, cap);
    return CGRT_OK;
}

}


using RaysKernel = void (*)(DeviceScene, RayParams, unsigned long long *);
struct RaysKernels {
    int id;
    RaysKernel fn;
};
template <int T, int B, int G, int P, int S, int SP, int F, int NT = kThreads>
static constexpr RaysKernels rk() {
    return {RayFlags{T != 0, B != 0, G != 0, P != 0, S != 0, SP != 0, F != 0, NT}.id(),
            &trace_rays_kernel<T != 0, B != 0, G != 0, P != 0, S != 0, SP != 0, F != 0, NT>};
}
static const RaysKernels kRaysKernels[] = {
    rk<1, 1, 0, 0, 0, 0, 0, 64>(), rk<1, 1, 1, 0, 0, 0, 0, 64>(),
    rk<1, 0, 0, 0, 0, 0, 0>(), rk<1, 0, 1, 0, 0, 0, 0>(), rk<1, 0, 0, 0, 1, 0, 0>(), rk<1, 0, 1, 0, 1, 0, 0>(),
    rk<0, 0, 0, 1, 0, 0, 0>(), rk<0, 0, 1, 1, 0, 0, 0>(), rk<0, 0, 0, 0, 0, 0, 0>(), rk<0, 0, 1, 0, 0, 0, 0>(),
    rk<0, 0, 0, 1, 0, 1, 0>(), rk<0, 0, 1, 1, 0, 1, 0>(), rk<1, 1, 1, 0, 0, 1, 0>(),
    rk<1, 1, 0, 0, 0, 0, 1, 64>(), rk<1, 0, 0, 0, 0, 0, 1>(), rk<1, 0, 0, 0, 1, 0, 1>(), rk<0, 0, 0, 1, 0, 0, 1>(),
    rk<0, 0, 0, 0, 0, 0, 1>(), rk<0, 0, 0, 1, 0, 1, 1>(), rk<1, 1, 0, 0, 0, 1, 1>(),
};
static const RaysKernels *rays_kernels(const RayFlags &f) {
    for (const RaysKernels &e : kRaysKernels)
        if (e.id == f.id()) return &e;
    return nullptr;
}
using CaptureKernel = void (*)(DeviceScene, RayParams, RaySink);
struct CaptureKernels {
    int id;
    CaptureKernel fn;
};
template <int T, int B, int G, int P, int SP, int NT = kThreads>
static constexpr CaptureKernels ck() {
    return {RayFlags{T != 0, B != 0, G != 0, P != 0, false, SP != 0, false, NT}.id(),
            &capture_rays_kernel<T != 0, B != 0, G != 0, P != 0, SP != 0, NT>};
}
static const CaptureKernels kCaptureKernels[] = {
    ck<1, 1, 0, 0, 0, 64>(), ck<1, 1, 1, 0, 0, 64>(),
// ... 612 lines not shown
    HIP_TRY(hipMemcpy(d_d, dir3, (size_t)n * 24, hipMemcpyHostToDevice));
    unsigned long long *d_keys = nullptr;
    if (keys) {
        HIP_TRY(b_keys.alloc((size_t)n * 8));
        d_keys = b_keys.as<unsigned long long>();
        HIP_TRY(hipMemcpy(d_keys, keys, (size_t)n * 8, hipMemcpyHostToDevice));
    }
    hipLaunchKernelGGL(intersect_rays_kernel, dim3((n + 63) / 64), dim3(64), 0, 0, s->dev, obj, d_o, d_d, d_keys, n,
                       d_hit, d_len, d_n);
    HIP_TRY(hipGetLastError());
    HIP_TRY(hipDeviceSynchronize());
    HIP_TRY(hipMemcpy(hit, d_hit, (size_t)n * 4, hipMemcpyDeviceToHost));
    HIP_TRY(hipMemcpy(len, d_len, (size_t)n * 8, hipMemcpyDeviceToHost));
    HIP_TRY(hipMemcpy(normal3, d_n, (size_t)n * 24, hipMemcpyDeviceToHost));
    return CGRT_OK;
}

int cgrt_surface_colors(const cgrt_scene *s, int obj, const double *points3, int n, double *colors3) {
    if (!s || !s->committed) return fail(CGRT_ERR_INVALID, "scene not committed");
    if (obj < 0 || obj >= s->dev.n_objs || n < 0 || (n > 0 && (!points3 || !colors3))) return fail(CGRT_ERR_INVALID, "bad argument");
    if (n == 0) return CGRT_OK;
    ON_DEVICE(s->device);
    DevBuf b_p, b_c;
    HIP_TRY(b_p.alloc((size_t)n * 24));
    HIP_TRY(b_c.alloc((size_t)n * 24));
    HIP_TRY(hipMemcpy(b_p.p, points3, (size_t)n * 24, hipMemcpyHostToDevice));
    hipLaunchKernelGGL(surface_colors_kernel, dim3((n + 255) / 256), dim3(256), 0, 0, s->dev, obj, b_p.as<double>(), n,
                       b_c.as<double>());
    HIP_TRY(hipGetLastError());
    HIP_TRY(hipDeviceSynchronize());
    HIP_TRY(hipMemcpy(colors3, b_c.p, (size_t)n * 24, hipMemcpyDeviceToHost));
    return CGRT_OK;
}

int cgrt_relay_start_host(int32_t k, int32_t chunk_spp, int32_t spp, int64_t cap, int32_t extent, int64_t n01, int64_t n012, int64_t n_tiles,
                          const uint32_t *list, const uint32_t *wcost, int32_t width, int32_t rows, uint32_t *start, int64_t start_cap,
                          int64_t *t) {
    if (!t || !list || !wcost || k < 2 || k > kRelayMaxChunks || chunk_spp <= 0 || spp <= 0 || cap < 0 || width <= 0 || rows <= 0 || n01 < 0 ||
        n01 > n012 || n012 > n_tiles || (size_t)n_tiles >= kRelayStartMaxTiles || (extent != kRelayGlass && extent != kRelayMirror))
        return fail(CGRT_ERR_INVALID, "bad argument");
    const uint32_t tiles_x = (uint32_t)((width + kTileW - 1) / kTileW), tiles_y = (uint32_t)((rows + kTileH - 1) / kTileH);
    const uint32_t wtiles_x = (uint32_t)((width + kWaveTileW - 1) / kWaveTileW), wtiles_y = (uint32_t)((rows + kWaveTileH - 1) / kWaveTileH);
    if ((int64_t)tiles_x * tiles_y != n_tiles) return fail(CGRT_ERR_INVALID, "n_tiles is not the grid's tile count");
    for (int64_t e = 0; e < n012; e++)
        if (list[e] >= (uint32_t)n_tiles) return fail(CGRT_ERR_INVALID, "list names a tile beyond the grid");
    const RelayItems r{(uint32_t)k, (uint32_t)n01, (uint32_t)n012, (uint32_t)n_tiles, (uint32_t)std::min<int64_t>(cap, n_tiles), extent, chunk_spp, spp};
    *t = (int64_t)relay_items_total(r);
    if (!start || start_cap < *t || *t == 0) return CGRT_OK;
    std::vector<uint64_t> weight((size_t)*t);
    relay_start_table(r, list, wcost, tiles_x, wtiles_x, wtiles_y, weight.data(), start);
    return CGRT_OK;
}

int cgrt_lens_samples(uint64_t seed, const int64_t *pixel, const int32_t *sample, int n, double radius, double *out3) {
    if (n < 0 || (n > 0 && (!pixel || !sample || !out3))) return fail(CGRT_ERR_INVALID, "bad argument");
    for (int i = 0; i < n; i++) {
        Stream rs(stream_key(seed, (uint64_t)pixel[i], (uint64_t)sample[i], 0));
        double sx, sy;
        while (true) {
            double ux, uy;
            rs.pair(ux, uy);
            sx = ux * 2.0 - 1;
            sy = uy * 2.0 - 1;
            if (sx * sx + sy * sy < 1) break;
        }
        out3[3 * i] = sx * radius;
        out3[3 * i + 1] = sy * radius;
        out3[3 * i + 2] = 0 * radius;
    }
    return CGRT_OK;
}

int cgrt_math_probe(int device, int op, const double *in, int64_t n, double *out) {
    if (op != CGRT_PROBE_SQRT && op != CGRT_PROBE_NORMALIZED && op != CGRT_PROBE_SPHERE_LEN && op != CGRT_PROBE_SPHERE_LEN_PAIR)
        return fail(CGRT_ERR_INVALID, "cgrt_math_probe: unknown op");
    if (!in || !out) return fail(CGRT_ERR_INVALID, "cgrt_math_probe: null buffer");
    if (n < 0) return fail(CGRT_ERR_INVALID, "cgrt_math_probe: negative n");
    if (n > ((int64_t)1 << 28)) return fail(CGRT_ERR_LIMIT, "cgrt_math_probe: more than 2^28 elements");
    if (n == 0) return CGRT_OK;
    const size_t n_in = op == CGRT_PROBE_SQRT ? 1 : (op == CGRT_PROBE_NORMALIZED ? 3 : (op == CGRT_PROBE_SPHERE_LEN ? 10 : 14)),
                 n_out = op == CGRT_PROBE_NORMALIZED ? 3 : (op == CGRT_PROBE_SPHERE_LEN_PAIR ? 2 : 1);
    ON_DEVICE(device);
    DevBuf b_in, b_out;
    HIP_TRY(b_in.alloc((size_t)n * n_in * sizeof(double)));
    HIP_TRY(b_out.alloc((size_t)n * n_out * sizeof(double)));
    HIP_TRY(hipMemcpy(b_in.p, in, (size_t)n * n_in * sizeof(double), hipMemcpyHostToDevice));
    hipLaunchKernelGGL(math_probe_kernel, dim3((unsigned)((n + 255) / 256)), dim3(256), 0, 0, op, b_in.as<double>(), (long long)n,
                       b_out.as<double>());
    HIP_TRY(hipGetLastError());
    HIP_TRY(hipDeviceSynchronize());
    HIP_TRY(hipMemcpy(out, b_out.p, (size_t)n * n_out * sizeof(double), hipMemcpyDeviceToHost));
    return CGRT_OK;
}

}

#include "cgrt_ppm_plan.h"
#include "cgrt_ppm_table.hpp"
#include "cgrt_photon_trace.hpp"
#include "cgrt_ppm_apply.hpp"
#include "cgrt_ppm_session.hpp"
#include "cgrt_output.hpp"

#ifdef CGRT_UTIL
extern "C" void cgrt_util_dump(unsigned long long *out) {
    (void)hipDeviceSynchronize();
// ... 6 lines not shown
```

### cgraytracing_amd/csrc/cgrt_relay.h

```cpp
#ifndef CGRT_RELAY_H
#define CGRT_RELAY_H
#include <cstddef>
#include <cstdint>

#include "cgrt_rng.hpp"

static constexpr int kRelayMaxChunks = 4, kRelayMinChunkSpp = 16, kRelayThreads = 256;
static constexpr int kRelayDefaultChunks = 2;
static constexpr int kRelayBatch = 8;

struct RelayChunks {
    int32_t k, chunk_spp;
};
CGRT_HD RelayChunks relay_chunks(int32_t spp, int32_t max_chunks = kRelayMaxChunks) {
    int32_t k = spp / kRelayMinChunkSpp;
    if (k > max_chunks) k = max_chunks;
    if (k > kRelayMaxChunks) k = kRelayMaxChunks;
    if (k < 2) return RelayChunks{1, spp};
    const int32_t cs = (spp + k - 1) / k;
    return RelayChunks{(spp + cs - 1) / cs, cs};
}
CGRT_HD int32_t relay_first_sample(int32_t c, int32_t chunk_spp) { return c * chunk_spp; }
CGRT_HD int32_t relay_end_sample(int32_t c, int32_t chunk_spp, int32_t spp) { return (c + 1) * chunk_spp < spp ? (c + 1) * chunk_spp : spp; }

// ... 40 lines not shown
        mirror = b >= a;
        i = mirror ? b - a : b;
    }
    const uint32_t first = mirror ? n01 : 0u, s = mirror ? s_m : s_a;
    if (i < k * s) return RelayBlock{first + i / k, (int32_t)(i % k), true};
    return RelayBlock{first + (i - (k - 1) * s), 0, false};
}

static constexpr int kRelayStartList = 0, kRelayStartCost = 1;
static constexpr int kRelayProbeSpp = 2;
struct RelayItems {
    uint32_t k, n01, n012, n_tiles, cap;
    int32_t extent, chunk_spp, spp;
};
CGRT_HD uint32_t relay_items_total(const RelayItems &r) {
    return r.n012 + (r.k - 1) * relay_split_entries(r.n01, r.n012, r.cap, r.extent);
}
CGRT_HD RelayBlock relay_item(uint32_t i, const RelayItems &r) {
    return relay_block_ordered(i, r.k, r.n01, r.n012, r.n_tiles, r.cap, r.extent, kRelayChunksFirst);
}
CGRT_HD uint64_t relay_item_weight(const RelayBlock &b, uint32_t tile_cost, const RelayItems &r) {
    const int32_t samples = b.split ? relay_end_sample(b.chunk, r.chunk_spp, r.spp) - relay_first_sample(b.chunk, r.chunk_spp) : r.spp;
    return (uint64_t)tile_cost * (uint64_t)(samples > 0 ? samples : 0);
}
CGRT_HD bool relay_item_before(uint64_t wj, uint32_t j, uint64_t wi, uint32_t i) { return wj > wi || (wj == wi && j < i); }
CGRT_HD uint32_t relay_start_word(const RelayBlock &b) { return b.entry << 2 | (uint32_t)b.chunk; }
CGRT_HD RelayBlock relay_start_block(uint32_t word, uint32_t n_split) { return RelayBlock{word >> 2, (int32_t)(word & 3u), (word >> 2) < n_split}; }
static_assert(kRelayMaxChunks <= 4, "a table word holds the chunk in two bits");
static constexpr size_t kRelayStartMaxTiles = (size_t)1 << 30;
CGRT_HD size_t relay_start_words(size_t n_tiles, int32_t k, size_t cap_split) { return relay_grid(n_tiles, k, cap_split); }
CGRT_HD uint32_t relay_tile_cost(const uint32_t *wcost, uint32_t tile, uint32_t tiles_x, uint32_t wtiles_x, uint32_t wtiles_y) {
    const uint32_t tx = tile % tiles_x, ty = tile / tiles_x;
    uint32_t c = 0;
    for (uint32_t w = 0; w < 4; w++) {
        const uint32_t wx = 2 * tx + (w & 1u), wy = 2 * ty + (w >> 1);
        if (wx < wtiles_x && wy < wtiles_y && wcost[wy * wtiles_x + wx] > c) c = wcost[wy * wtiles_x + wx];
    }
    return c;
}
inline void relay_start_table(const RelayItems &r, const uint32_t *list, const uint32_t *wcost, uint32_t tiles_x, uint32_t wtiles_x,
                              uint32_t wtiles_y, uint64_t *weight, uint32_t *start) {
    const uint32_t t = relay_items_total(r);
    for (uint32_t i = 0; i < t; i++) {
        const RelayBlock b = relay_item(i, r);
        weight[i] = relay_item_weight(b, relay_tile_cost(wcost, list[b.entry], tiles_x, wtiles_x, wtiles_y), r);
    }
    for (uint32_t i = 0; i < t; i++) {
        uint32_t rank = 0;
        for (uint32_t j = 0; j < t; j++) rank += relay_item_before(weight[j], j, weight[i], i) ? 1u : 0u;
        start[rank] = relay_start_word(relay_item(i, r));
    }
}

struct RelayLayout {
    size_t racc, rhits, rcount, rvals, total;
};
CGRT_HD size_t relay_tile_bytes(int32_t k, int32_t slots) {
    const size_t t = kRelayThreads;
    return sizeof(uint32_t) + 3 * t * sizeof(double) + (size_t)k * t * sizeof(uint32_t) + (size_t)(k - 1) * t * sizeof(uint32_t) +
           (size_t)(k - 1) * (size_t)slots * 3 * t * sizeof(double);
}
CGRT_HD RelayLayout relay_layout(size_t cap, int32_t k, int32_t slots) {
    const size_t t = kRelayThreads;
    RelayLayout l;
    l.racc = (cap * sizeof(uint32_t) + 255) & ~(size_t)255;
    l.rhits = l.racc + cap * 3 * t * sizeof(double);
    l.rcount = l.rhits + cap * (size_t)k * t * sizeof(uint32_t);
    l.rvals = l.rcount + cap * (size_t)(k - 1) * t * sizeof(uint32_t);
    l.total = l.rvals + cap * (size_t)(k - 1) * (size_t)slots * 3 * t * sizeof(double);
    return l;
}
static constexpr size_t kRelayBudget = (size_t)4 << 30;
CGRT_HD size_t relay_budget(size_t mem_total) { return mem_total / 8 < kRelayBudget ? mem_total / 8 : kRelayBudget; }
CGRT_HD size_t relay_cap(size_t n_tiles, int32_t k, int32_t slots, size_t budget, long long bound = 0) {
    size_t cap = budget / relay_tile_bytes(k, slots);
    if (cap > n_tiles) cap = n_tiles;
    if (bound > 0 && cap > (size_t)bound) cap = (size_t)bound;
    while (cap > 0 && relay_layout(cap, k, slots).total > budget) cap--;
    return cap;
}

#endif
```

### cgraytracing_amd/csrc/cgrt_tile_order.hpp

```cpp
#ifndef CGRT_TILE_ORDER_HPP
#define CGRT_TILE_ORDER_HPP

enum class Capturing { None, Active, Unknown };
static Capturing stream_capturing(hipStream_t st) {
    hipStreamCaptureStatus c = hipStreamCaptureStatusNone;
    if (hipStreamIsCapturing(st, &c) != hipSuccess) {
        (void)hipGetLastError();
        return Capturing::Unknown;
    }
    return c == hipStreamCaptureStatusNone ? Capturing::None : Capturing::Active;
}

struct TileOrderState {
    OrderSpheres spheres{};
    bool ok = false;
    GrowBuf buf;
    struct Key {
        double cam[3], half_width, focus_plane, lens_radius;
        int32_t W, H, rows, row_offset, stripe_rows, stripe_rank, stripe_nranks, masks;
        uint64_t commit_gen;
        const void *buf;
    };
    static_assert(sizeof(Key) == 96, "Key is compared as bytes: no padding");
    Key key{};
    uint64_t commit_gen = 0;
    bool valid = false, reused = false;
    bool captured = false;
    hipEvent_t ev = nullptr;
    hipStream_t stream = nullptr;
    size_t tiles = 0, mask_wtiles = 0, sure_wtiles = 0;
    TileOrderLayout at;
    TileOrderPlan::Class3 class3 = TileOrderPlan::None;
    int lens_stage = kLensStageOff;
    struct CostKey {
        uint64_t seed;
        int32_t max_depth, probe_spp;
    };
    struct TableKey {
        int32_t spp, k, chunk_spp, cap, extent, pad_;
    };
    static_assert(sizeof(CostKey) == 16 && sizeof(TableKey) == 24, "compared as bytes: no padding");
    CostKey cost_key{};
    TableKey table_key{};
    bool cost_valid = false, table_valid = false, start_reused = false;
    size_t start_words = 0, start_wtiles = 0;

    void begin_launch() {
        tiles = mask_wtiles = sure_wtiles = 0;
        start_words = start_wtiles = 0;
        reused = start_reused = false;
        class3 = TileOrderPlan::None;
        lens_stage = kLensStageOff;
    }
    void release() {
        buf.release();
        if (ev) (void)hipEventDestroy(ev);
        ev = nullptr;
    }
    template <class T> int read(const Region &r, T *dst, size_t count) const {
        HIP_TRY(hipMemcpy(dst, reinterpret_cast<const unsigned char *>(buf.p) + r.at, count * sizeof(T), hipMemcpyDeviceToHost));
        return CGRT_OK;
    }
};

struct RelayState {
    GrowBuf buf;
    size_t refused = 0, zeroed = 0;
    bool dirty = false;
    hipEvent_t ev = nullptr;
    hipStream_t stream = nullptr;
    bool recorded = false;
    struct Last {
        int k = 0;
        size_t cap = 0;
        int slots = 0, extent = 0, order = 0;
    } last;

    void begin_launch() { last = Last{}; }
    void release() {
        buf.release();
        if (ev) (void)hipEventDestroy(ev);
        ev = nullptr;
    }
};

static int order_tiles(TileOrderState &o, const DeviceScene &dev, const FramePlan &p, GridParams &g, bool no_reuse, Capturing capturing,
                       hipStream_t st) {
    const int tiles_x = (g.W + kTileW - 1) / kTileW, tiles_y = (g.rows + kTileH - 1) / kTileH;
    const size_t n = (size_t)tiles_x * tiles_y;
    const bool masks = p.order.masks, sure = masks && p.order.sure;
    const TileOrderLayout at = tile_order_layout(n, p.n_wt, sure, p.relay_start_words);
    const bool grown = at.total > o.buf.cap;
    if (grown) o.valid = false;
    if (o.buf.need(at.total) != hipSuccess) {
        (void)hipGetLastError();
        return fail(CGRT_ERR_DEVICE, "cannot allocate launch scratch (tile order)");
    }
    unsigned char *base = reinterpret_cast<unsigned char *>(o.buf.p);
    uint32_t *plan = at.plan.in<uint32_t>(base), *list = at.list.in<uint32_t>(base);
    uint32_t *wmask = masks ? at.wmask.in<uint32_t>(base) : nullptr;
    unsigned char *wsure = sure ? at.wsure.in<unsigned char>(base) : nullptr;
    const TileOrderState::Key key{{g.cam[0], g.cam[1], g.cam[2]}, g.half_width, g.focus_plane, g.lens_radius, g.W, g.H, g.rows, g.row_offset,
                                  g.stripe_rows, g.stripe_rank, g.stripe_nranks, (masks ? 1 : 0) | (sure ? 2 : 0), o.commit_gen, o.buf.p};
    if (capturing != Capturing::None) o.captured = true;
    const bool plain = !o.captured && !no_reuse;
    o.reused = plain && o.valid && std::memcmp(&key, &o.key, sizeof(key)) == 0;
    if (o.reused) {
        if (st != o.stream) HIP_TRY(hipStreamWaitEvent(st, o.ev, 0));
    } else {
        o.valid = o.cost_valid = o.table_valid = false;
        if (grown) HIP_TRY(hipMemsetAsync(plan, 0, at.plan.bytes, st));
        const unsigned blocks = (unsigned)std::min((p.n_wt + 1023) / 1024, (size_t)64);
        hipLaunchKernelGGL(tile_order_kernel, dim3(blocks), dim3(1024), 0, st, g, o.spheres, dev, tiles_x, tiles_y, plan, list,
                           at.tile_cls.in<unsigned char>(base), at.wave_cls.in<unsigned char>(base), wmask);
        if (sure)
            hipLaunchKernelGGL(sure_first_kernel, dim3((unsigned)((p.n_wt + 255) / 256)), dim3(256), 0, st, g, dev, tiles_x,
                               at.tile_cls.in<unsigned char>(base), wmask, wsure);
        if (plain && hipPeekAtLastError() == hipSuccess) {
            if (!o.ev && hipEventCreateWithFlags(&o.ev, hipEventDisableTiming) != hipSuccess) {
                (void)hipGetLastError();
                o.ev = nullptr;
            }
            if (o.ev && hipEventRecord(o.ev, st) == hipSuccess) {
                o.key = key;
                o.stream = st;
                o.valid = true;
            } else {
                (void)hipGetLastError();
            }
        }
    }
    g.plan = plan;
    g.border = list;
    g.wmask = wmask;
    g.wsure = wsure;
    g.tile_order = kOrderAll;
    o.tiles = n;
    o.mask_wtiles = masks ? p.n_wt : 0;
    o.sure_wtiles = sure ? p.n_wt : 0;
    o.at = at;
    o.class3 = p.order.class3;
    o.lens_stage = p.order.lens_stage;
    return CGRT_OK;
}

static bool relay_prepare(RelayState &r, const FramePlan &p, GridParams &g, Capturing capturing, hipStream_t st) {
    if (capturing != Capturing::None) return false;
    if (r.refused && p.relay_bytes >= r.refused) return false;
    if (p.relay_bytes > r.buf.cap) {
        if (r.recorded && hipEventSynchronize(r.ev) != hipSuccess) (void)hipGetLastError();
        r.zeroed = 0;
        if (r.buf.need(p.relay_bytes) != hipSuccess) {
            (void)hipGetLastError();
            r.refused = p.relay_bytes;
            return false;
        }
    }
    if (!r.ev && hipEventCreateWithFlags(&r.ev, hipEventDisableTiming) != hipSuccess) {
        (void)hipGetLastError();
        r.ev = nullptr;
        return false;
    }
    if (r.recorded && st != r.stream && hipStreamWaitEvent(st, r.ev, 0) != hipSuccess) {
        (void)hipGetLastError();
        return false;
    }
    if (r.dirty || p.relay_cap > r.zeroed) {
        if (hipMemsetAsync(r.buf.p, 0, p.relay_cap * sizeof(uint32_t), st) != hipSuccess) {
            (void)hipGetLastError();
            return false;
        }
    }
    r.zeroed = p.relay_cap;
    r.dirty = true;
    g.relay = reinterpret_cast<unsigned char *>(r.buf.p);
    g.relay_k = p.relay_k;
    g.relay_chunk_spp = p.relay_chunk_spp;
    g.relay_cap = (int32_t)p.relay_cap;
    g.relay_slots = p.relay_slots;
    g.relay_extent = p.relay_extent;
    g.relay_order = p.relay_order;
    return true;
}

struct TileOrderGuard {
    TileOrderState &order;
    RelayState &relay;
    bool relayed = false, through = false;
    TileOrderGuard(TileOrderState &o, RelayState &r) : order(o), relay(r) {
        order.begin_launch();
        relay.begin_launch();
    }
    TileOrderGuard(const TileOrderGuard &) = delete;
    TileOrderGuard &operator=(const TileOrderGuard &) = delete;
    ~TileOrderGuard() {
        if (!through) order.valid = false;
    }
    int commit(const GridParams &g, hipStream_t st) {
        if (relayed) {
            HIP_TRY(hipEventRecord(relay.ev, st));
            relay.stream = st;
            relay.recorded = true;
            relay.last = RelayState::Last{g.relay_k, (size_t)g.relay_cap, g.relay_slots, g.relay_extent, g.relay_order};
            relay.dirty = false;
        }
        through = true;
        return CGRT_OK;
    }
};

static int last_tile_order(const TileOrderState &o, uint32_t *plan5, uint32_t *list, uint8_t *cls, int64_t cap, int64_t *n_tiles) {
    const size_t n = o.tiles;
    *n_tiles = (int64_t)n;
    if (n == 0 || cap < (int64_t)n) return CGRT_OK;
    HIP_TRY(hipDeviceSynchronize());
    int rc = CGRT_OK;
    if (plan5 && (rc = o.read(o.at.plan, plan5, kOrderClasses + 1))) return rc;
    if (list && (rc = o.read(o.at.list, list, n))) return rc;
    return cls ? o.read(o.at.tile_cls, cls, n) : CGRT_OK;
}
static int last_sphere_masks(const TileOrderState &o, uint32_t *masks, int64_t cap, int64_t *n_wave_tiles) {
    const size_t n_wt = o.mask_wtiles;
    *n_wave_tiles = (int64_t)n_wt;
    if (n_wt == 0 || o.tiles == 0 || !masks || cap < (int64_t)n_wt) return CGRT_OK;
    HIP_TRY(hipDeviceSynchronize());
    return o.read(o.at.wmask, masks, n_wt);
}
static int last_sure_tiles(const TileOrderState &o, uint8_t *sure, int64_t cap, int64_t *n_wave_tiles) {
    const size_t n_wt = o.sure_wtiles;
    *n_wave_tiles = (int64_t)n_wt;
    if (n_wt == 0 || o.tiles == 0 || !sure || cap < (int64_t)n_wt) return CGRT_OK;
    HIP_TRY(hipDeviceSynchronize());
    return o.read(o.at.wsure, sure, n_wt);
}
static int last_class3_tiles(const TileOrderState &o, TileOrderPlan::Class3 form, int64_t *n_tiles) {
    *n_tiles = 0;
    if (o.class3 != form || o.tiles == 0) return CGRT_OK;
    uint32_t plan[kOrderClasses + 1];
    HIP_TRY(hipDeviceSynchronize());
    if (int rc = o.read(o.at.plan, plan, kOrderClasses + 1)) return rc;
    *n_tiles = (int64_t)plan[kOrderClasses] - (int64_t)plan[3];
    return CGRT_OK;
}
static int last_lens_stage(const TileOrderState &o, int64_t *lds_tiles, int64_t *area_tiles) {
    *lds_tiles = *area_tiles = 0;
    return o.lens_stage == kLensStageLds ? last_class3_tiles(o, TileOrderPlan::InKernel, lds_tiles) : CGRT_OK;
}
static int last_sample_relay(const TileOrderState &o, const RelayState &r, int64_t *tiles, int32_t *chunks, int64_t *parked_values) {
    *tiles = *parked_values = 0;
    *chunks = 0;
    const RelayState::Last &l = r.last;
    if (l.k <= 1 || o.tiles == 0) return CGRT_OK;
    uint32_t plan[kOrderClasses + 1];
    HIP_TRY(hipDeviceSynchronize());
    if (int rc = o.read(o.at.plan, plan, kOrderClasses + 1)) return rc;
    const size_t n_split = relay_split_entries(plan[2], plan[3], (uint32_t)l.cap, l.extent);
    *tiles = (int64_t)n_split;
    if (n_split == 0) return CGRT_OK;
    *chunks = l.k;
    std::vector<uint32_t> cnt(n_split * (size_t)(l.k - 1) * kRelayThreads);
    const RelayLayout rl = relay_layout(l.cap, l.k, l.slots);
    HIP_TRY(hipMemcpy(cnt.data(), reinterpret_cast<const unsigned char *>(r.buf.p) + rl.rcount, cnt.size() * sizeof(uint32_t), hipMemcpyDeviceToHost));
    for (uint32_t c : cnt) *parked_values += (int64_t)c;
    return CGRT_OK;
}
static int last_relay_start(const TileOrderState &o, const RelayState &r, uint32_t *start, int64_t start_cap, uint32_t *wcost, int64_t cost_cap,
                            int64_t *t, int64_t *n_wave_tiles, int32_t *reused) {
    *t = *n_wave_tiles = 0;
    *reused = 0;
    if (o.start_words == 0 || o.tiles == 0 || r.last.k <= 1) return CGRT_OK;
    uint32_t plan[kOrderClasses + 1];
    HIP_TRY(hipDeviceSynchronize());
    if (int rc = o.read(o.at.plan, plan, kOrderClasses + 1)) return rc;
    const RelayItems ri{(uint32_t)r.last.k, plan[2], plan[3], plan[kOrderClasses], (uint32_t)r.last.cap, r.last.extent, 0, 0};
    const size_t n = relay_items_total(ri);
    if (n > o.start_words) return fail(CGRT_ERR_DEVICE, "relay start table: more workgroups than the table holds");
    *t = (int64_t)n;
    *n_wave_tiles = (int64_t)o.start_wtiles;
    *reused = o.start_reused ? 1 : 0;
    if (start && start_cap >= (int64_t)n && n > 0)
        if (int rc = o.read(o.at.start, start, n)) return rc;
    if (wcost && cost_cap >= (int64_t)o.start_wtiles && o.start_wtiles > 0)
        if (int rc = o.read(o.at.wcost, wcost, o.start_wtiles)) return rc;
    return CGRT_OK;
}
static void last_relay_form(const TileOrderState &o, const RelayState &r, int32_t *mirror, int32_t *order) {
    const bool relayed = r.last.k > 1 && o.tiles != 0;
    *mirror = relayed ? (r.last.extent == kRelayMirror ? 1 : 0) : -1;
    *order = relayed ? r.last.order : -1;
}

#endif
```

### cgraytracing_amd/engine.py

```python
from __future__ import annotations

import ctypes as C
import os
import weakref

import numpy as np

from . import _capi
from ._capi import Camera as _CCamera
from ._capi import Grid as _CGrid
from ._capi import check
from .scene import Camera


def _d3(v):
    return (C.c_double * 3)(*[float(x) for x in v])



_RELAY_ORDERS = ("chunks_first", "mirror_first", "interleaved")


_RELAY_STARTS = ("list", "cost")


def _relay_flag(sample_relay, relay_mirror=None, relay_order=None, relay_start=None):
    form = 0 if relay_mirror is None else (8192 if relay_mirror else 16384)
    if relay_start is not None:
        if relay_start not in _RELAY_STARTS:
            raise ValueError("relay_start: None, " + ", ".join(repr(o) for o in _RELAY_STARTS))
        form |= 524288 if relay_start == "cost" else 1048576
    if relay_order is not None:
        if relay_order not in _RELAY_ORDERS:
            raise ValueError("relay_order: None, " + ", ".join(repr(o) for o in _RELAY_ORDERS))
        form |= 32768 * (1 + _RELAY_ORDERS.index(relay_order))
    if sample_relay is None:
        return form
    if sample_relay is True or sample_relay is False:
        return form | (1024 if sample_relay else 2048)
    if int(sample_relay) not in (2, 4):
        raise ValueError("sample_relay: None, True, False, 2 or 4")
    return form | 1024 | (4096 if int(sample_relay) == 4 else 0)


def relay_start_host(k, chunk_spp, spp, cap, mirror, plan, tile_list, wcost, width, rows):
    lib = _capi.lib()
    lst, wc = np.ascontiguousarray(tile_list, np.uint32), np.ascontiguousarray(wcost, np.uint32)
    assert wc.size == ((width + 15) // 16) * ((rows + 3) // 4) and lst.size == int(plan[4])
    args = (int(k), int(chunk_spp), int(spp), int(cap), 1 if mirror else 0, int(plan[2]), int(plan[3]), int(plan[4]), lst.ctypes.data,
            wc.ctypes.data, int(width), int(rows))
    t = C.c_int64()
    check(lib.cgrt_relay_start_host(*args, None, 0, C.byref(t)))
    start = np.zeros(max(t.value, 1), np.uint32)
    check(lib.cgrt_relay_start_host(*args, start.ctypes.data, start.size, C.byref(t)))
    return start[:t.value]


class Scene:

    def __init__(self, objs, device=0, commit=True, build=None):
        L = _capi.lib()
        h = C.c_void_p()
        check(L.cgrt_scene_create(C.byref(h)))
        if build is not None:
            check(L.cgrt_scene_set_build(h, {"host": _capi.BUILD_HOST, "device": _capi.BUILD_DEVICE}[build]))
        self._h = h
        self._L = L
        self.device = int(device)
        self._sessions = weakref.WeakSet()
        self.obj_index = []
        tex_ids = {}
        try:
            for o in objs:
                k = o.kind
                if k == "sphere":
                    i = L.cgrt_scene_add_sphere(h, _d3(o.center), o.radius, _d3(o.surfaceColor), o.reflection,
                                                o.transparency)
                elif k == "plane":
                    tid = -1
                    t = o.texture
                    if t is not None:
                        if id(t) not in tex_ids:
                            tex_ids[id(t)] = check(L.cgrt_scene_add_texture(
                                h, t.data.ctypes.data, t.data.shape[0], t.data.shape[1], _d3(t.normal),
                                _d3(t.position), t.lenx, t.leny, int(t.isbump)))
                        tid = tex_ids[id(t)]
                    i = L.cgrt_scene_add_plane(h, _d3(o.position), _d3(o.normal), _d3(o.surfaceColor), o.reflection,
                                               o.transparency, tid)
                elif k == "mesh":
                    if o.triangles is not None:
                        i = L.cgrt_scene_add_mesh_triangles(h, o.triangles.ctypes.data, len(o.triangles),
                                                            _d3(o.surfaceColor), o.reflection, o.transparency,
                                                            o.typeofdata)
                    else:
                        i = L.cgrt_scene_add_mesh_file(h, o.filename.encode(), o.a, _d3(o.b), _d3(o.surfaceColor),
# ... 39 lines not shown
        bi = _capi.BuildInfo()
        check(self._L.cgrt_scene_build_info(self._h, C.byref(bi)))
        return {f: getattr(bi, f) for f, _ in bi._fields_}

    def tree_dump(self, t=0):
        nn, nl, nt = C.c_int32(), C.c_int32(), C.c_int32()
        check(self._L.cgrt_scene_tree_sizes(self._h, t, C.byref(nn), C.byref(nl), C.byref(nt)))
        nodes = np.zeros((nn.value, 3), np.int32)
        leaf = np.zeros((nl.value,), np.int32)
        bbox = np.zeros((nn.value, 6), np.float64)
        tris = np.zeros((nt.value, 9), np.float64)
        check(self._L.cgrt_scene_tree_dump(self._h, t, nodes.ctypes.data, leaf.ctypes.data, bbox.ctypes.data,
                                           tris.ctypes.data))
        return nodes, leaf, bbox, tris

    def bvh_dump(self, t=0):
        nn = C.c_int32()
        check(self._L.cgrt_scene_bvh_dump(self._h, t, C.byref(nn), None, None))
        n = nn.value
        box = np.zeros((8, n, 6), np.float32)
        sl = np.zeros((8, n, 2), np.int32)
        check(self._L.cgrt_scene_bvh_dump(self._h, t, C.byref(nn), box.ctypes.data, sl.ctypes.data))
        return box, sl[:, :, 0].copy(), sl[:, :, 1].copy()

    def bvh_order(self, t=0):
        nn, nl, nt = C.c_int32(), C.c_int32(), C.c_int32()
        check(self._L.cgrt_scene_tree_sizes(self._h, t, C.byref(nn), C.byref(nl), C.byref(nt)))
        lvl = C.c_int32()
        order = np.zeros(max(nt.value, 1), np.int32)
        check(self._L.cgrt_scene_bvh_order(self._h, t, C.byref(lvl), order.ctypes.data))
        return bool(lvl.value), order[: nt.value]

    def wide_dump(self, t=0):
        n, need = C.c_int32(), C.c_int32()
        check(self._L.cgrt_scene_wide_dump(self._h, t, C.byref(n), C.byref(need), None, None))
        box = np.zeros((max(n.value, 1), 4, 6), np.float32)
        ref = np.zeros((max(n.value, 1), 4), np.int32)
        check(self._L.cgrt_scene_wide_dump(self._h, t, C.byref(n), C.byref(need), box.ctypes.data, ref.ctypes.data))
        return box[: n.value], ref[: n.value], need.value

    def _structs(self, camera, width, height, rows, spp, max_depth, seed, row_offset, stripe, sample_offset,
                 spp_total, flags):
        camera = camera or Camera()
        cc = _CCamera(_d3(camera.cam), camera.half_width, camera.focus_plane, camera.lens_radius)
        s_rows, s_rank, s_n = stripe if stripe else (0, 0, 1)
        g = _CGrid(width, height, rows, row_offset, s_rows, s_rank, s_n, spp, sample_offset,
                   spp_total if spp_total else spp, max_depth, flags, seed)
        return cc, g

    def trace_grid(self, width, height, spp=1, camera=None, max_depth=5, seed=12345, rows=None, row_offset=0,
                   stripe=None, sample_offset=0, spp_total=None, out=None, nhit=None, counters=None, stream=None,
                   stats=False, accumulate=False, split_samples=False, reorder=True, force_reorder=False, tile_order=True,
                   diffuse_tiles=False, sphere_pairs=True, sphere_masks=True, sample_relay=None,
                   relay_mirror=None, relay_order=None, lens_stage=True, sure_tiles=True, relay_start=None):
        import torch

        rows = height - row_offset if rows is None else rows
        dev = torch.device("cuda", self.device)
        if out is None:
            out = torch.zeros((rows, width, 3), dtype=torch.float32, device=dev)
        if nhit is None:
            nhit = torch.zeros((rows, width), dtype=torch.int32, device=dev)
        elif nhit is False:
            nhit = None
        if counters is None:
            counters = torch.zeros((_capi.CGRT_NCOUNTERS,), dtype=torch.int64, device=dev)
        assert out.is_contiguous() and out.dtype == torch.float32 and tuple(out.shape) == (rows, width, 3)
        cc, g = self._structs(camera, width, height, rows, spp, max_depth, seed, row_offset, stripe, sample_offset,
                              spp_total, (1 if stats else 0) | (2 if accumulate else 0) | (4 if split_samples else 0) |
                              (0 if reorder else 8) | (16 if force_reorder else 0) | (0 if tile_order else 64) |
                              (128 if diffuse_tiles else 0) | (0 if sphere_pairs else 256) | (0 if sphere_masks else 512) | _relay_flag(sample_relay, relay_mirror, relay_order, relay_start) |
                              (0 if lens_stage else 131072) | (0 if sure_tiles else 262144))
        st = stream if stream is not None else torch.cuda.current_stream(dev).cuda_stream
        check(self._L.cgrt_trace_grid(self._h, C.byref(cc), C.byref(g), out.data_ptr(),
                                      nhit.data_ptr() if nhit is not None else None,
                                      counters.data_ptr(), C.c_void_p(st)))
        return out, nhit, counters

    _WANT = ("acc", "nhit", "hit")

    def camera_rays(self, width, height, spp=1, camera=None, seed=12345, rows=None, row_offset=0, stripe=None,
                    sample_offset=0, stream=None):
        import torch

        rows = height - row_offset if rows is None else rows
        dev = torch.device("cuda", self.device)
        n = spp * rows * width
        org = torch.empty((n, 3), dtype=torch.float64, device=dev)
        dirs = torch.empty((n, 3), dtype=torch.float64, device=dev)
        keys = torch.empty((n,), dtype=torch.int64, device=dev)
        cc, g = self._structs(camera, width, height, rows, spp, 1, seed, row_offset, stripe, sample_offset, None, 0)
        st = stream if stream is not None else torch.cuda.current_stream(dev).cuda_stream
        with torch.cuda.device(dev):
            check(self._L.cgrt_camera_rays(C.byref(cc), C.byref(g), org.data_ptr(), dirs.data_ptr(), keys.data_ptr(),
                                           C.c_void_p(st)))
        return org, dirs, keys

    def trace_rays(self, org, dirs, keys=None, max_depth=5, seed=12345, first_index=0, want=("acc", "nhit", "hit"),
                   counters=None, stream=None, stats=False, out=None, sign_pass=True):
        import torch

        dev = torch.device("cuda", self.device)
        for name, t in (("org", org), ("dirs", dirs)):
            if not (isinstance(t, torch.Tensor) and t.dtype == torch.float64 and t.dim() == 2 and t.shape[1] == 3 and
                    t.is_contiguous() and t.device == dev):
                raise ValueError("trace_rays: %s must be a contiguous float64 [n,3] tensor on %s" % (name, dev))
        n = org.shape[0]
        if dirs.shape[0] != n:
            raise ValueError("trace_rays: org and dirs differ in length")
        if keys is not None and not (isinstance(keys, torch.Tensor) and keys.dtype == torch.int64 and tuple(keys.shape) == (n,) and
                                     keys.is_contiguous() and keys.device == dev):
            raise ValueError("trace_rays: keys must be a contiguous int64 [n] tensor on %s" % (dev,))
        want = tuple(want)
        if not want or any(w not in self._WANT for w in want):
            raise ValueError("trace_rays: want is a non-empty subset of %r" % (self._WANT,))
        shapes = {}
        if "acc" in want:
            shapes["acc"] = ((n, 3), torch.float64)
        if "nhit" in want:
            shapes["nhit"] = ((n,), torch.int32)
        if "hit" in want:
            shapes.update(hit_obj=((n,), torch.int32), hit_t=((n,), torch.float64), hit_normal=((n, 3), torch.float64))
        res = {}
        for name, (shape, dtype) in shapes.items():
# ... 148 lines not shown
        elif not (isinstance(occ, torch.Tensor) and occ.dtype == torch.uint8 and tuple(occ.shape) == (n,) and occ.is_contiguous() and
                  occ.device == dev):
            raise ValueError("occluded: out must be a contiguous uint8 [n] tensor on %s" % (dev,))
        counters = torch.zeros((_capi.CGRT_NCOUNTERS,), dtype=torch.int64, device=dev)
        res = {"occluded": occ, "counters": counters}
        if n == 0:
            return res
        r = _capi.Rays(n, org.data_ptr(), dirs.data_ptr(), keys.data_ptr() if keys is not None else None, first_index, seed, 1,
                       (_capi.RAYS_STATS if stats else 0) | (_capi.RAYS_SKIP_TRANSPARENT if skip_transparent else 0))
        o = _capi.Occlusion(tmax.data_ptr() if tmax is not None else None, occ.data_ptr())
        st = stream if stream is not None else torch.cuda.current_stream(dev).cuda_stream
        check(self._L.cgrt_occlusion_rays(self._h, C.byref(r), C.byref(o), counters.data_ptr(), C.c_void_p(st)))
        return res

    def occluded_host(self, org, dirs, tmax=None, keys=None, seed=12345, first_index=0, skip_transparent=False, stats=False):
        org = np.ascontiguousarray(org, np.float64).reshape(-1, 3)
        dirs = np.ascontiguousarray(dirs, np.float64).reshape(-1, 3)
        n = len(org)
        if len(dirs) != n:
            raise ValueError("occluded_host: org and dirs differ in length")
        if tmax is not None:
            tmax = np.ascontiguousarray(tmax, np.float64)
            if tmax.shape != (n,):
                raise ValueError("occluded_host: tmax must have one entry per ray")
        if keys is not None:
            keys = np.ascontiguousarray(keys, np.uint64)
            if keys.shape != (n,):
                raise ValueError("occluded_host: keys must have one entry per ray")
        occ = np.zeros(max(n, 1), np.uint8)
        cnt = np.zeros((_capi.CGRT_NCOUNTERS,), np.uint64)
        r = _capi.Rays(n, org.ctypes.data, dirs.ctypes.data, keys.ctypes.data if keys is not None else None, first_index, seed, 1,
                       (_capi.RAYS_STATS if stats else 0) | (_capi.RAYS_SKIP_TRANSPARENT if skip_transparent else 0))
        o = _capi.Occlusion(tmax.ctypes.data if tmax is not None else None, occ.ctypes.data)
        check(self._L.cgrt_occlusion_rays_host(self._h, C.byref(r), C.byref(o), cnt.ctypes.data))
        return dict(occluded=occ[:n], counters=cnt, nrays=int(cnt[_capi.CNT_RAYS]))

    def occlusion_variant(self, stats=False):
        r = _capi.Rays(1, None, None, None, 0, 0, 1, _capi.RAYS_STATS if stats else 0)
        buf = C.create_string_buffer(160)
        check(self._L.cgrt_occlusion_rays_variant(self._h, C.byref(r), buf, len(buf)))
        return buf.value.decode()

    def rays_variant(self, max_depth=5, want=("acc", "nhit", "hit"), stats=False):
        full = 1 if ("acc" in want or "nhit" in want) else None
        r = _capi.Rays(1, None, None, None, 0, 0, max_depth, _capi.RAYS_STATS if stats else 0)
        o = _capi.RayResults(full, None, 1 if "hit" in want else None, None, None)
        buf = C.create_string_buffer(160)
        check(self._L.cgrt_trace_rays_variant(self._h, C.byref(r), C.byref(o), buf, len(buf)))
        return buf.value.decode()

    def trace_grid_host(self, width, height, spp=1, camera=None, max_depth=5, seed=12345, rows=None, row_offset=0,
                        stripe=None, sample_offset=0, spp_total=None, stats=False, split_samples=False, reorder=True,
                        force_reorder=False, tile_order=True, diffuse_tiles=False, sphere_pairs=True, sphere_masks=True, sample_relay=None,
                        relay_mirror=None, relay_order=None, lens_stage=True, sure_tiles=True, relay_start=None):
        rows = height - row_offset if rows is None else rows
        rgb = np.zeros((rows, width, 3), np.float32)
        nhit = np.zeros((rows, width), np.uint32)
        cnt = np.zeros((_capi.CGRT_NCOUNTERS,), np.uint64)
        cc, g = self._structs(camera, width, height, rows, spp, max_depth, seed, row_offset, stripe, sample_offset,
                              spp_total, (1 if stats else 0) | (4 if split_samples else 0) | (0 if reorder else 8) |
                              (16 if force_reorder else 0) | (0 if tile_order else 64) | (128 if diffuse_tiles else 0) |
                              (0 if sphere_pairs else 256) | (0 if sphere_masks else 512) | _relay_flag(sample_relay, relay_mirror, relay_order, relay_start) |
                              (0 if lens_stage else 131072) | (0 if sure_tiles else 262144))
        check(self._L.cgrt_trace_grid_host(self._h, C.byref(cc), C.byref(g), rgb.ctypes.data, nhit.ctypes.data,
                                           cnt.ctypes.data))
        return dict(rgb=rgb, nhit=nhit, counters=cnt, nrays=int(cnt[_capi.CNT_RAYS]),
                    nhp=int(cnt[_capi.CNT_HITPOINTS]))

    def last_tile_order(self):
        n = C.c_int64()
        check(self._L.cgrt_scene_last_tile_order(self._h, None, None, None, 0, C.byref(n)))
        if n.value == 0:
            return None
        plan, lst, cls = np.zeros(5, np.uint32), np.zeros(n.value, np.uint32), np.zeros(n.value, np.uint8)
        check(self._L.cgrt_scene_last_tile_order(self._h, plan.ctypes.data, lst.ctypes.data, cls.ctypes.data, n.value, C.byref(n)))
        return dict(plan=plan, list=lst, cls=cls)

    def last_sphere_masks(self):
        n = C.c_int64()
        check(self._L.cgrt_scene_last_sphere_masks(self._h, None, 0, C.byref(n)))
        if n.value == 0:
            return None
        masks = np.zeros(n.value, np.uint32)
        check(self._L.cgrt_scene_last_sphere_masks(self._h, masks.ctypes.data, n.value, C.byref(n)))
        return masks

    def last_sure_tiles(self):
        n = C.c_int64()
        check(self._L.cgrt_scene_last_sure_tiles(self._h, None, 0, C.byref(n)))
        if n.value == 0:
            return None
        sure = np.zeros(n.value, np.uint8)
        check(self._L.cgrt_scene_last_sure_tiles(self._h, sure.ctypes.data, n.value, C.byref(n)))
        return sure

    def last_tile_order_reused(self):
        f = C.c_int32()
        check(self._L.cgrt_scene_last_tile_order_reused(self._h, C.byref(f)))
        return bool(f.value)

    def last_sample_relay(self):
        t, k, v = C.c_int64(), C.c_int32(), C.c_int64()
        check(self._L.cgrt_scene_last_sample_relay(self._h, C.byref(t), C.byref(k), C.byref(v)))
        return dict(tiles=int(t.value), chunks=int(k.value), parked_values=int(v.value))

    def last_relay_form(self):
        m, o = C.c_int32(), C.c_int32()
        check(self._L.cgrt_scene_last_relay_form(self._h, C.byref(m), C.byref(o)))
        return None if m.value < 0 else dict(mirror=bool(m.value), order=_RELAY_ORDERS[o.value])

    def last_relay_start(self):
        t, n, r = C.c_int64(), C.c_int64(), C.c_int32()
        check(self._L.cgrt_scene_last_relay_start(self._h, None, 0, None, 0, C.byref(t), C.byref(n), C.byref(r)))
        if n.value == 0:
            return None
        start, wcost = np.zeros(max(t.value, 1), np.uint32), np.zeros(n.value, np.uint32)
        check(self._L.cgrt_scene_last_relay_start(self._h, start.ctypes.data, start.size, wcost.ctypes.data, n.value, C.byref(t),
                                                  C.byref(n), C.byref(r)))
        return dict(t=int(t.value), start=start[:t.value], wcost=wcost, reused=bool(r.value))

    def last_lens_stage(self):
        a, b = C.c_int64(), C.c_int64()
        check(self._L.cgrt_scene_last_lens_stage(self._h, C.byref(a), C.byref(b)))
        return dict(lds_tiles=int(a.value), area_tiles=int(b.value))

    def last_diffuse_tiles(self):
        n = C.c_int64()
        check(self._L.cgrt_scene_last_diffuse_tiles(self._h, C.byref(n)))
        return int(n.value)

    def last_inkernel_diffuse_tiles(self):
        n = C.c_int64()
        check(self._L.cgrt_scene_last_inkernel_diffuse_tiles(self._h, C.byref(n)))
        return int(n.value)

    def trace_grid_hitpoints(self, width, height, spp=1, camera=None, max_depth=5, seed=12345, rows=None,
                             row_offset=0, cap=None):
        rows = height - row_offset if rows is None else rows
        cap = int(cap if cap is not None else rows * width * spp * 16)
        rec = np.zeros((max(cap, 1), 10), np.float64)
        n = C.c_uint64(0)
        cc, g = self._structs(camera, width, height, rows, spp, max_depth, seed, row_offset, None, 0, None, 0)
        check(self._L.cgrt_trace_grid_hitpoints(self._h, C.byref(cc), C.byref(g), rec.ctypes.data, cap, C.byref(n)))
        m = min(int(n.value), cap)
        lab = rec[:m, 9].astype(np.int64)
        seq, lab = lab & 15, lab >> 4
        return dict(hp=rec[:m, :9].copy(), pix=lab % (rows * width), smp=lab // (rows * width), seq=seq,
                    count=int(n.value))

    def ppm_render(self, width, height, spp=1, camera=None, max_depth=5, seed=12345, nphotons=100000, photon_seed=777,
                   hashsize=1000001, light=(0.0, 19.999, 20.0), jitter=2.0, power=700.0, alpha=0.7, batch=0,
                   want_hitpoints=False, want_rgb8=False, rows=None, row_offset=0, stripe=None, initial_radius=0.0,
                   pair_cap=0):
        rows = height if rows is None else rows
        cc, g = self._structs(camera, width, height, rows, spp, max_depth, seed, row_offset, stripe, 0, None, 0)
        ph = _capi.Photons(_d3(light), jitter, power, alpha, nphotons, hashsize, batch, photon_seed, initial_radius, pair_cap)
        height = rows
        img = np.zeros((height, width, 3), np.float64)
        cap = height * width * spp * 16 if want_hitpoints else 0
        hp = np.zeros((max(cap, 1), 16), np.float64)
        rgb8 = np.zeros((height, width, 3), np.uint8)
        res = _capi.PpmResult(img.ctypes.data, rgb8.ctypes.data if want_rgb8 else None,
                              hp.ctypes.data if want_hitpoints else None, cap)
        check(self._L.cgrt_ppm_render(self._h, C.byref(cc), C.byref(g), C.byref(ph), C.byref(res)))
        out = dict(image=img, count=int(res.hp_count), n_events=int(res.n_events), n_pairs=int(res.n_pairs),
                   n_batch_halvings=int(res.n_batch_halvings),
                   ms=dict(eye=res.ms_eye, table=res.ms_table, photons=res.ms_photons, gather=res.ms_gather))
        if want_hitpoints:
            out["hp"] = hp[: int(res.hp_count)]
        if want_rgb8:
            out["rgb8"] = rgb8
        return out
# ... 311 lines not shown
```

### include/cgrt.h

```cpp
#ifndef CGRT_H
#define CGRT_H

#include <stddef.h>
#include <stdint.h>

#ifdef __cplusplus
extern "C" {
#endif

#define CGRT_VERSION 112

enum {
    CGRT_OK = 0,
    CGRT_ERR_INVALID = -1,
    CGRT_ERR_IO = -2,
    CGRT_ERR_DEVICE = -3,
    CGRT_ERR_UNSUPPORTED = -4,
    CGRT_ERR_LIMIT = -5
};

typedef struct cgrt_scene cgrt_scene;

typedef struct cgrt_camera {
    double cam[3];
    double half_width;
    double focus_plane;
    double lens_radius;
} cgrt_camera;

typedef struct cgrt_grid {
    int32_t width, height;
    int32_t rows;
    int32_t row_offset;
    int32_t stripe_rows;
    int32_t stripe_rank;
    int32_t stripe_nranks;
    int32_t spp;
    int32_t sample_offset;
    int32_t spp_total;
    int32_t max_depth;
    int32_t flags;
    uint64_t seed;
} cgrt_grid;

enum {
    CGRT_GRID_STATS = 1,
    CGRT_GRID_ACCUMULATE = 2,
    CGRT_GRID_NO_REORDER = 8,
    CGRT_GRID_FORCE_REORDER = 16,
    CGRT_GRID_NO_TILE_ORDER = 64,
    CGRT_GRID_DIFFUSE_TILES = 128,
    CGRT_GRID_NO_SPHERE_PAIRS = 256,
    CGRT_GRID_NO_SPHERE_MASKS = 512,
    CGRT_GRID_SAMPLE_RELAY = 1024,
    CGRT_GRID_NO_SAMPLE_RELAY = 2048,
    CGRT_GRID_SAMPLE_RELAY_4 = 4096,
    CGRT_GRID_RELAY_MIRROR = 8192,
    CGRT_GRID_RELAY_NO_MIRROR = 16384,
    CGRT_GRID_RELAY_CHUNKS_FIRST = 32768,
    CGRT_GRID_RELAY_MIRROR_FIRST = 65536,
    CGRT_GRID_RELAY_INTERLEAVED = 98304,
    CGRT_GRID_RELAY_ORDER_MASK = 98304,
    CGRT_GRID_RELAY_COST_START = 524288,
    CGRT_GRID_NO_RELAY_COST_START = 1048576,
    CGRT_GRID_NO_LENS_STAGE = 131072,
    CGRT_GRID_NO_SURE_TILES = 262144,
    CGRT_GRID_HITPOINTS = 32,
    CGRT_GRID_SPLIT_SAMPLES = 4
};

enum {
    CGRT_CNT_RAYS = 0,
    CGRT_CNT_HITPOINTS = 1,
    CGRT_CNT_WAVE_ITERS = 2,
    CGRT_CNT_NODE_TESTS = 3,
    CGRT_CNT_TRI_TESTS = 4,
    CGRT_NCOUNTERS = 8
};

typedef struct cgrt_scene_stats {
    int32_t n_objects, n_spheres, n_planes, n_meshes, n_beziers, n_textures, n_trees, committed;
    int64_t n_triangles;
    int64_t n_nodes;
    int64_t device_bytes;
    int64_t scene_bytes_fp64;
} cgrt_scene_stats;

int cgrt_version(void);
const char *cgrt_last_error(void);

int cgrt_scene_create(cgrt_scene **out);
void cgrt_scene_destroy(cgrt_scene *s);

enum { CGRT_BUILD_HOST = 0, CGRT_BUILD_DEVICE = 1 };
int cgrt_scene_set_build(cgrt_scene *s, int mode);

typedef struct cgrt_build_info {
    int32_t mode;
    int32_t n_device_trees;
    double ms_host_build;
    double ms_device_build;
    double ms_commit;
} cgrt_build_info;
int cgrt_scene_build_info(const cgrt_scene *s, cgrt_build_info *out);

int cgrt_scene_add_sphere(cgrt_scene *s, const double c[3], double r, const double sc[3], double refl, double transp);

int cgrt_scene_add_texture(cgrt_scene *s, const uint8_t *rgb, int rows, int cols, const double n[3],
                           const double p[3], double lx, double ly, int isbump);

int cgrt_scene_add_plane(cgrt_scene *s, const double p[3], const double n[3], const double sc[3], double refl,
                         double transp, int tex_id);

int cgrt_scene_add_mesh_file(cgrt_scene *s, const char *filename, double a, const double b[3], const double sc[3],
                             double refl, double transp, int typeofdata);
int cgrt_scene_add_mesh_triangles(cgrt_scene *s, const double *tri9, int ntri, const double sc[3], double refl,
                                  double transp, int typeofdata);
// ... 137 lines not shown
                     uint64_t *keys, uint32_t *draws, void *stream);
int cgrt_photon_emit_host(const cgrt_photons *ph, int64_t first, int64_t count, double *org3, double *dir3, double *flux3,
                          uint64_t *keys, uint32_t *draws);

int cgrt_ppm_session_image(const cgrt_ppm_session *p, double *image, uint8_t *rgb8);
int cgrt_ppm_session_image_device(const cgrt_ppm_session *p, double *image, uint8_t *rgb8, void *stream);
int cgrt_ppm_session_hitpoints(const cgrt_ppm_session *p, double *hp16, uint64_t cap, uint64_t *count);
typedef struct cgrt_ppm_session_info {
    int64_t photons_done;
    uint64_t hp_count, n_events, n_pairs, n_batch_halvings;
    int64_t device_bytes;
    double ms_eye, ms_table;
    double ms_photons;
    double ms_last_add, ms_last_image;
} cgrt_ppm_session_info;
int cgrt_ppm_session_get_info(const cgrt_ppm_session *p, cgrt_ppm_session_info *out);

int cgrt_tonemap_rgb8(int device, const double *image, int width, int height, uint8_t *rgb8);

int cgrt_write_png(const char *path, int width, int height, const uint8_t *rgb8);

int cgrt_photon_events(const cgrt_scene *s, const cgrt_photons *ph, int max_depth, int64_t first, int32_t count,
                       double *events9, uint8_t *valid);

int cgrt_photon_ray_events(const cgrt_scene *s, const cgrt_photon_rays *pr, uint64_t seed, int64_t first_index, int max_depth,
                           double *events9, uint8_t *valid);

int cgrt_intersect_rays(const cgrt_scene *s, int obj, const double *org3, const double *dir3, const uint64_t *keys,
                        int n, int32_t *hit, double *len, double *normal3);

int cgrt_surface_colors(const cgrt_scene *s, int obj, const double *points3, int n, double *colors3);

int cgrt_trace_grid_variant(const cgrt_scene *s, const cgrt_camera *cam, const cgrt_grid *grid, char *name, size_t cap);

int cgrt_scene_last_tile_order(const cgrt_scene *s, uint32_t *plan5, uint32_t *list, uint8_t *cls, int64_t cap, int64_t *n_tiles);

int cgrt_scene_last_sphere_masks(const cgrt_scene *s, uint32_t *masks, int64_t cap, int64_t *n_wave_tiles);
int cgrt_scene_last_sure_tiles(const cgrt_scene *s, uint8_t *sure, int64_t cap, int64_t *n_wave_tiles);
int cgrt_scene_last_tile_order_reused(const cgrt_scene *s, int32_t *reused);

int cgrt_trace_grid_diffuse_variant(const cgrt_scene *s, const cgrt_camera *cam, const cgrt_grid *grid, char *name, size_t cap);
int cgrt_scene_last_diffuse_tiles(const cgrt_scene *s, int64_t *n_tiles);
int cgrt_scene_last_inkernel_diffuse_tiles(const cgrt_scene *s, int64_t *n_tiles);
int cgrt_scene_last_sample_relay(const cgrt_scene *s, int64_t *tiles, int32_t *chunks, int64_t *parked_values);
int cgrt_scene_last_relay_form(const cgrt_scene *s, int32_t *mirror, int32_t *order);
int cgrt_scene_last_relay_start(const cgrt_scene *s, uint32_t *start, int64_t start_cap, uint32_t *wcost, int64_t cost_cap, int64_t *t,
                                int64_t *n_wave_tiles, int32_t *reused);
int cgrt_scene_last_lens_stage(const cgrt_scene *s, int64_t *lds_tiles, int64_t *area_tiles);

int cgrt_relay_start_host(int32_t k, int32_t chunk_spp, int32_t spp, int64_t cap, int32_t extent, int64_t n01, int64_t n012, int64_t n_tiles,
                          const uint32_t *list, const uint32_t *wcost, int32_t width, int32_t rows, uint32_t *start, int64_t start_cap,
                          int64_t *t);

int cgrt_lens_samples(uint64_t seed, const int64_t *pixel, const int32_t *sample, int n, double radius, double *out3);

enum { CGRT_PROBE_SQRT = 0, CGRT_PROBE_NORMALIZED = 1, CGRT_PROBE_SPHERE_LEN = 2, CGRT_PROBE_SPHERE_LEN_PAIR = 4  };
int cgrt_math_probe(int device, int op, const double *in, int64_t n, double *out);

#ifdef __cplusplus
}
#endif
#endif
```

Before: 99640.

## Add relay boost: split the costliest tiles into more sample chunks

Adds a 'relay boost' scheme in which the most expensive split tiles, ranked by estimated wave cost, get promoted to a separate relay area with a larger chunk count (boost_k) and smaller chunk_spp. New device kernels compute per-tile cost, rank and promote candidates, weight the chunks, and build a combined start table so heavy tiles are spread over more workgroups. The aim is to cut the tail imbalance where a few costly tiles finish last. In exchange it adds planning kernels, extra relay memory and a larger kernel argument struct.

```diff
diff --git a/cgraytracing_amd/_capi.py b/cgraytracing_amd/_capi.py
--- a/cgraytracing_amd/_capi.py
+++ b/cgraytracing_amd/_capi.py
@@ -175,6 +175,12 @@
                                         C.c_void_p, C.c_int32, C.c_int32, C.c_void_p, C.c_int64, C.POINTER(C.c_int64)]),
     "cgrt_scene_last_relay_start": (C.c_int, [C.c_void_p, C.c_void_p, C.c_int64, C.c_void_p, C.c_int64, C.POINTER(C.c_int64),
                                               C.POINTER(C.c_int64), C.POINTER(C.c_int32)]),
+    "cgrt_scene_last_relay_boost": (C.c_int, [C.c_void_p, C.POINTER(C.c_int64), C.POINTER(C.c_int32), C.POINTER(C.c_int64), C.POINTER(C.c_uint64),
+                                              C.POINTER(C.c_int32), C.POINTER(C.c_int32), C.POINTER(C.c_int32), C.c_void_p, C.c_int64]),
+    "cgrt_relay_boost_host": (C.c_int, [C.c_int32, C.c_int32, C.c_int32, C.c_int64, C.c_int32, C.c_int64, C.c_int64, C.c_int64, C.c_void_p,
+                                        C.c_void_p, C.c_int32, C.c_int32, C.c_int32, C.c_int32, C.c_int64, C.c_int32, C.c_int32, C.c_int32,
+                                        C.c_void_p, C.c_int64, C.c_void_p, C.c_int64, C.POINTER(C.c_int64), C.POINTER(C.c_int64),
+                                        C.POINTER(C.c_uint64)]),
     "cgrt_scene_last_lens_stage": (C.c_int, [C.c_void_p, C.POINTER(C.c_int64), C.POINTER(C.c_int64)]),
     "cgrt_scene_last_tile_order_reused": (C.c_int, [C.c_void_p, C.POINTER(C.c_int32)]),
     "cgrt_trace_grid_diffuse_variant": (C.c_int, [C.c_void_p, C.c_void_p, C.c_void_p, C.c_char_p, C.c_size_t]),
diff --git a/cgraytracing_amd/csrc/cgrt_eye.hpp b/cgraytracing_amd/csrc/cgrt_eye.hpp
--- a/cgraytracing_amd/csrc/cgrt_eye.hpp
+++ b/cgraytracing_amd/csrc/cgrt_eye.hpp
@@ -72,8 +72,18 @@
 }
 
 struct RelayWg {
-    int slot = -1, chunk = 0, s0 = 0, s1 = 0;
+    int slot = -1, chunk = 0, s0 = 0, s1 = 0, boost = 0;
 };
+struct RelayForm {
+    unsigned char *area;
+    size_t cap;
+    int k, slots;
+};
+template <bool COST>
+__device__ __forceinline__ RelayForm relay_form(const GridParams &g, const RelayWg &rw) {
+    if (COST && rw.boost) return RelayForm{g.relay + g.relay_boost_off, (size_t)g.boost_cap, g.boost_k, g.boost_slots};
+    return RelayForm{g.relay, (size_t)g.relay_cap, g.relay_k, g.relay_slots};
+}
 
 template <bool TREES, bool BEZ, bool DOF, bool GLASS, bool SPH, bool STATS, bool HPS, int NT, bool HEAVY, bool SPILL = false, bool HFONLY = false,
           bool DIFF = false, bool PAIR = false, bool PARK = false, bool LSTAGE = false, bool COST = false>
@@ -202,9 +212,11 @@
     int s = (g.chunks > 1) ? chunk * g.chunk_spp : (PAIR && rw.slot >= 0 ? rw.s0 : 0);
     double *park = nullptr;
     uint32_t park_n = 0;
-    if (PARK)
-        park = reinterpret_cast<double *>(g.relay + relay_layout((size_t)g.relay_cap, g.relay_k, g.relay_slots).rvals) +
-               ((size_t)rw.slot * (size_t)(g.relay_k - 1) + (size_t)(rw.chunk - 1)) * (size_t)g.relay_slots * (3 * NT) + threadIdx.x;
+    if (PARK) {
+        const RelayForm rf = relay_form<COST>(g, rw);
+        park = reinterpret_cast<double *>(rf.area + relay_layout(rf.cap, rf.k, rf.slots).rvals) +
+               ((size_t)rw.slot * (size_t)(rf.k - 1) + (size_t)(rw.chunk - 1)) * (size_t)rf.slots * (3 * NT) + threadIdx.x;
+    }
     bool have = false;
     V3 o = camorg, d = pdir, adj = mk(1, 1, 1);
     int depth_left = 0;
@@ -403,7 +415,7 @@
                         q[1] = hf.y;
                         q[2] = hf.z;
                     } else if (PARK) {
-                        if (park_n < (uint32_t)g.relay_slots) {
+                        if (park_n < (uint32_t)relay_form<COST>(g, rw).slots) {
                             double *q = park + (size_t)park_n * (3 * NT);
                             q[0] = hf.x;
                             q[NT] = hf.y;
@@ -548,12 +560,13 @@
         uint32_t px_hits = my_hits;
         bool store = true;
         if (PAIR && rw.slot >= 0) {
-            const size_t slot = (size_t)rw.slot, k = (size_t)g.relay_k;
-            const RelayLayout rl = relay_layout((size_t)g.relay_cap, g.relay_k, g.relay_slots);
-            uint32_t *arrive = reinterpret_cast<uint32_t *>(g.relay) + slot;
-            double *racc = reinterpret_cast<double *>(g.relay + rl.racc) + slot * (3 * NT) + threadIdx.x;
-            uint32_t *rhits = reinterpret_cast<uint32_t *>(g.relay + rl.rhits) + slot * k * NT + threadIdx.x;
-            uint32_t *rcount = reinterpret_cast<uint32_t *>(g.relay + rl.rcount) + slot * (k - 1) * NT + threadIdx.x;
+            const RelayForm rf = relay_form<COST>(g, rw);
+            const size_t slot = (size_t)rw.slot, k = (size_t)rf.k;
+            const RelayLayout rl = relay_layout(rf.cap, rf.k, rf.slots);
+            uint32_t *arrive = reinterpret_cast<uint32_t *>(rf.area) + slot;
+            double *racc = reinterpret_cast<double *>(rf.area + rl.racc) + slot * (3 * NT) + threadIdx.x;
+            uint32_t *rhits = reinterpret_cast<uint32_t *>(rf.area + rl.rhits) + slot * k * NT + threadIdx.x;
+            uint32_t *rcount = reinterpret_cast<uint32_t *>(rf.area + rl.rcount) + slot * (k - 1) * NT + threadIdx.x;
             if (PARK) {
                 rcount[(size_t)(rw.chunk - 1) * NT] = park_n;
             } else {
@@ -569,7 +582,7 @@
                 __builtin_amdgcn_fence(__ATOMIC_RELEASE, "agent");
                 asm volatile("s_waitcnt vmcnt(0)" ::: "memory");
                 const unsigned int ticket = __hip_atomic_fetch_add(arrive, 1u, __ATOMIC_RELAXED, __HIP_MEMORY_SCOPE_AGENT);
-                const bool last = ticket == (unsigned int)g.relay_k - 1u;
+                const bool last = ticket == (unsigned int)rf.k - 1u;
                 if (last) {
                     __builtin_amdgcn_fence(__ATOMIC_ACQUIRE, "agent");
                     asm volatile("s_waitcnt vmcnt(0)" ::: "memory");
@@ -584,18 +597,18 @@
                 acc_g = racc[NT];
                 acc_b = racc[2 * NT];
                 px_hits = rhits[0];
-                for (int c = 1; c < g.relay_k; c++) {
+                for (int c = 1; c < rf.k; c++) {
                     px_hits += rhits[(size_t)c * NT];
                     uint32_t n = rcount[(size_t)(c - 1) * NT];
-                    if (n > (uint32_t)g.relay_slots) n = (uint32_t)g.relay_slots;
+                    if (n > (uint32_t)rf.slots) n = (uint32_t)rf.slots;
                     uint32_t n_max = n;
                     for (int off = 32; off > 0; off >>= 1) {
                         const uint32_t o2 = (uint32_t)__shfl_xor((int)n_max, off);
                         n_max = o2 > n_max ? o2 : n_max;
                     }
                     n_max = (uint32_t)__builtin_amdgcn_readfirstlane((int)n_max);
-                    const double *q = reinterpret_cast<const double *>(g.relay + rl.rvals) +
-                                      (slot * (k - 1) + (size_t)(c - 1)) * (size_t)g.relay_slots * (3 * NT) + threadIdx.x;
+                    const double *q = reinterpret_cast<const double *>(rf.area + rl.rvals) +
+                                      (slot * (k - 1) + (size_t)(c - 1)) * (size_t)rf.slots * (3 * NT) + threadIdx.x;
                     for (uint32_t i0 = 0; i0 < n_max; i0 += kRelayBatch) {
                         double v[kRelayBatch][3];
 #pragma unroll
@@ -702,22 +715,30 @@
             const unsigned n01 = load_uniform(g.plan + 2), n012 = load_uniform(g.plan + 3);
             RelayBlock rb{n_tiles, 0, false};
             bool tabled = false;
+            unsigned b = blockIdx.x, bslot = 0u;
             if (START && g.relay_start_at != 0u) {
                 const unsigned n_split = relay_split_entries(n01, n012, (unsigned)g.relay_cap, g.relay_extent);
-                tabled = blockIdx.x < n012 + ((unsigned)g.relay_k - 1u) * n_split;
+                const unsigned t0 = n012 + ((unsigned)g.relay_k - 1u) * n_split;
+                const unsigned items = g.relay_boost_at != 0u ? load_uniform(g.plan + g.relay_boost_at + kBoostItems) : t0;
+                tabled = b < items;
                 if (tabled) {
-                    rb = relay_start_block(load_uniform(g.plan + g.relay_start_at + blockIdx.x), n_split);
-                    if (rb.chunk >= g.relay_k) return;
+                    rb = relay_start_block(load_uniform(g.plan + g.relay_start_at + b), n_split);
+                    if (g.relay_boost_at != 0u && rb.split) bslot = load_uniform(g.plan + g.relay_boost_at + kBoostHead + rb.entry);
+                    if (rb.chunk >= (bslot != 0u ? g.boost_k : g.relay_k) || bslot > (unsigned)g.boost_cap) return;
+                } else {
+                    b -= items - t0;
                 }
             }
-            if (!tabled) rb = relay_block_ordered(blockIdx.x, (unsigned)g.relay_k, n01, n012, n_tiles, (unsigned)g.relay_cap, g.relay_extent, g.relay_order);
+            if (!tabled) rb = relay_block_ordered(b, (unsigned)g.relay_k, n01, n012, n_tiles, (unsigned)g.relay_cap, g.relay_extent, g.relay_order);
             entry = rb.entry;
             if (entry >= n_tiles) return;
             if (rb.split) {
-                rw.slot = (int)entry;
+                const int cs = START && bslot != 0u ? g.boost_chunk_spp : g.relay_chunk_spp;
+                rw.slot = START && bslot != 0u ? (int)(bslot - 1u) : (int)entry;
+                rw.boost = START && bslot != 0u ? 1 : 0;
                 rw.chunk = rb.chunk;
-                rw.s0 = relay_first_sample(rb.chunk, g.relay_chunk_spp);
-                rw.s1 = relay_end_sample(rb.chunk, g.relay_chunk_spp, g.spp);
+                rw.s0 = relay_first_sample(rb.chunk, cs);
+                rw.s1 = relay_end_sample(rb.chunk, cs, g.spp);
             }
         }
         tile_block = (int)load_uniform(g.border + entry);
@@ -964,6 +985,75 @@
     if (i < t) start[rank] = relay_start_word(relay_item(i, r));
 }
 
+struct RelayBoostArgs {
+    RelayStartArgs a;
+    RelayBoost b;
+};
+__global__ __launch_bounds__(kRelayThreads) void relay_boost_cost_kernel(RelayBoostArgs ba, const uint32_t *__restrict__ plan, const uint32_t *__restrict__ list,
+                                                                         const uint32_t *__restrict__ wcost, uint32_t *__restrict__ ecost,
+                                                                         uint32_t *__restrict__ head) {
+    const RelayItems r = relay_items_of(ba.a, plan);
+    const uint32_t e = blockIdx.x * kRelayThreads + threadIdx.x;
+    if (e >= r.n012) return;
+    const uint32_t c = relay_tile_cost(wcost, list[e], ba.a.tiles_x, ba.a.wtiles_x, ba.a.wtiles_y);
+    ecost[e] = c;
+    if (c) atomicAdd(reinterpret_cast<unsigned long long *>(head + kBoostS), (unsigned long long)c * (unsigned long long)r.spp);
+}
+__global__ __launch_bounds__(kRelayThreads) void relay_boost_promote_kernel(RelayBoostArgs ba, const uint32_t *__restrict__ plan,
+                                                                            const uint32_t *__restrict__ ecost, uint32_t *__restrict__ head,
+                                                                            uint32_t *__restrict__ bslot) {
+    const RelayItems r = relay_items_of(ba.a, plan);
+    const uint32_t n_split = relay_split_entries(r.n01, r.n012, r.cap, r.extent), e = blockIdx.x * kRelayThreads + threadIdx.x;
+    if (blockIdx.x * kRelayThreads >= n_split) return;
+    const uint64_t S = *reinterpret_cast<const unsigned long long *>(head + kBoostS);
+    __shared__ unsigned long long k_s[kRelayThreads];
+    const uint32_t ce = e < n_split ? ecost[e] : 0u;
+    const uint64_t ke = relay_boost_key(e < n_split && relay_boost_candidate(ce, r, ba.b, S), ce);
+    uint32_t rank = 0;
+    for (uint32_t j0 = 0; j0 < n_split; j0 += kRelayThreads) {
+        __syncthreads();
+        if (j0 + threadIdx.x < n_split) {
+            const uint32_t cj = ecost[j0 + threadIdx.x];
+            k_s[threadIdx.x] = relay_boost_key(relay_boost_candidate(cj, r, ba.b, S), cj);
+        }
+        __syncthreads();
+        const uint32_t n = min((uint32_t)kRelayThreads, n_split - j0);
+        for (uint32_t u = 0; u < n; u++) rank += relay_item_before(k_s[u], j0 + u, ke, e) ? 1u : 0u;
+    }
+    if (e >= n_split) return;
+    const bool promoted = ke != 0 && rank < ba.b.cap;
+    bslot[e] = promoted ? rank + 1u : 0u;
+    if (promoted) atomicAdd(head + kBoostPromoted, 1u);
+}
+__global__ __launch_bounds__(kRelayThreads) void relay_boost_weight_kernel(RelayBoostArgs ba, const uint32_t *__restrict__ plan,
+                                                                           const uint32_t *__restrict__ ecost, const uint32_t *__restrict__ bslot,
+                                                                           uint32_t *__restrict__ head, unsigned long long *__restrict__ weight) {
+    const RelayItems r = relay_items_of(ba.a, plan);
+    const uint32_t n_split = relay_split_entries(r.n01, r.n012, r.cap, r.extent), v = blockIdx.x * kRelayThreads + threadIdx.x;
+    if (v == 0) head[kBoostItems] = relay_boost_items(r, ba.b, head[kBoostPromoted]);
+    if (v >= r.n012 * ba.b.k) return;
+    const uint32_t e = v / ba.b.k, c = v % ba.b.k;
+    const bool promoted = e < n_split && bslot[e] != 0u;
+    weight[v] = relay_boost_weight(c, relay_boost_chunks(e, promoted, n_split, r, ba.b), promoted, ecost[e], r, ba.b);
+}
+__global__ __launch_bounds__(kRelayThreads) void relay_boost_start_kernel(RelayBoostArgs ba, const uint32_t *__restrict__ plan,
+                                                                          const unsigned long long *__restrict__ weight, uint32_t *__restrict__ start) {
+    const RelayItems r = relay_items_of(ba.a, plan);
+    const uint32_t nv = r.n012 * ba.b.k, v = blockIdx.x * kRelayThreads + threadIdx.x;
+    if (blockIdx.x * kRelayThreads >= nv) return;
+    __shared__ unsigned long long w_s[kRelayThreads];
+    const unsigned long long wv = v < nv ? weight[v] : kRelayNoItem;
+    uint32_t rank = 0;
+    for (uint32_t j0 = 0; j0 < nv; j0 += kRelayThreads) {
+        __syncthreads();
+        if (j0 + threadIdx.x < nv) w_s[threadIdx.x] = weight[j0 + threadIdx.x];
+        __syncthreads();
+        const uint32_t n = min((uint32_t)kRelayThreads, nv - j0);
+        for (uint32_t u = 0; u < n; u++) rank += relay_boost_before(w_s[u], j0 + u, wv, v) ? 1u : 0u;
+    }
+    if (wv != kRelayNoItem) start[rank] = relay_start_word(RelayBlock{v / ba.b.k, (int32_t)(v % ba.b.k), false});
+}
+
 __global__ __launch_bounds__(1024) void plan_kernel(const uint32_t *__restrict__ cost_in, const unsigned char *__restrict__ light, int n,
                                                     unsigned kmax, unsigned long long divisor, uint32_t *__restrict__ plan,
                                                     uint32_t *__restrict__ order, int32_t *__restrict__ hidx,
diff --git a/cgraytracing_amd/csrc/cgrt_frame.h b/cgraytracing_amd/csrc/cgrt_frame.h
--- a/cgraytracing_amd/csrc/cgrt_frame.h
+++ b/cgraytracing_amd/csrc/cgrt_frame.h
@@ -47,8 +47,12 @@
     int32_t lens_batch;
     uint32_t relay_start_at;
     const unsigned char *wsure;
-};
-static_assert(sizeof(GridParams) == 336, "GridParams is a kernel argument: its layout is fixed");
+    uint64_t relay_boost_off;
+    uint32_t relay_boost_at;
+    int32_t boost_k, boost_chunk_spp, boost_cap, boost_slots, pad_boost_;
+};
+static_assert(sizeof(GridParams) == 368, "GridParams is a kernel argument: its layout is fixed");
+static constexpr int kBoostS = 0, kBoostPromoted = 2, kBoostItems = 3, kBoostHead = 4;
 
 static constexpr int kTileW = 32, kTileH = 8, kThreads = 256;
 static constexpr int kOrderSpheresMax = 16, kOrderClasses = 4, kOrderPlanWords = 8, kOrderArrived = 5;
@@ -65,9 +69,11 @@
 struct TileOrderLayout {
     Region plan{}, list{}, tile_cls{}, wave_cls{}, wmask{}, wsure{};
     Region wcost{}, weight{}, start{};
+    Region boost{}, ecost{}, bweight{}, bstart{};
     size_t total = 0;
 };
-inline TileOrderLayout tile_order_layout(size_t n_tiles, size_t n_wt, bool sure = false, size_t start_words = 0) {
+inline TileOrderLayout tile_order_layout(size_t n_tiles, size_t n_wt, bool sure = false, size_t start_words = 0, size_t boost_words = 0,
+                                         size_t split_cap = 0, int boost_k = 0) {
     TileOrderLayout L;
     size_t end = 0;
     const auto take = [&end](size_t bytes) { end += bytes; return Region{end - bytes, bytes}; };
@@ -90,6 +96,16 @@
         L.weight = take(start_words * sizeof(uint64_t));
         end = align256(end);
         L.start = take(start_words * sizeof(uint32_t));
+    }
+    if (start_words && boost_words) {
+        end = align256(end);
+        L.boost = take((kBoostHead + split_cap) * sizeof(uint32_t));
+        end = align256(end);
+        L.ecost = take(n_tiles * sizeof(uint32_t));
+        end = align256(end);
+        L.bweight = take(n_tiles * (size_t)boost_k * sizeof(uint64_t));
+        end = align256(end);
+        L.bstart = take((start_words + boost_words) * sizeof(uint32_t));
     }
     L.total = align256(end);
     return L;
@@ -166,6 +182,9 @@
     int relay_order = -1;
     int relay_start = -1;
     int relay_probe_spp = kRelayProbeSpp;
+    bool relay_boost_off = false;
+    uint32_t relay_boost_num = kRelayBoostNum, relay_boost_den = kRelayBoostDen;
+    long long relay_boost_tiles = -1;
     int lens_stage = -1;
     const char *timeline_file = nullptr;
 };
@@ -184,6 +203,24 @@
     if (v == "list" || v == "0") return kRelayStartList;
     if (v == "cost" || v == "1") return kRelayStartCost;
     return -1;
+}
+inline bool relay_boost_named(const char *e, bool &off, uint32_t &num, uint32_t &den) {
+    const std::string v(e);
+    if (v.empty()) return true;
+    if (v == "off" || v == "0") {
+        off = true;
+        return true;
+    }
+    const size_t slash = v.find('/');
+    if (slash == std::string::npos || slash == 0 || slash + 1 >= v.size()) return false;
+    for (size_t i = 0; i < v.size(); i++)
+        if (i != slash && (v[i] < '0' || v[i] > '9')) return false;
+    if (slash > 6 || v.size() - slash - 1 > 6) return false;
+    const unsigned long n = std::strtoul(v.c_str(), nullptr, 10), d = std::strtoul(v.c_str() + slash + 1, nullptr, 10);
+    if (n > kRelayBoostMaxTerm || d < 1 || d > kRelayBoostMaxTerm) return false;
+    num = (uint32_t)n;
+    den = (uint32_t)d;
+    return true;
 }
 static constexpr int kLensStageOff = 0, kLensStageLds = 1;
 static constexpr int kLensStageDefault = kLensStageLds;
@@ -228,6 +265,14 @@
     }();
     EyeKnobs k = once;
     k.timeline_file = *env_str("CGRT_TIMELINE_FILE") ? env_str("CGRT_TIMELINE_FILE") : nullptr;
+    if (!relay_boost_named(env_str("CGRT_RELAY_BOOST"), k.relay_boost_off, k.relay_boost_num, k.relay_boost_den)) {
+        static bool said = false;
+        if (!said)
+            std::fprintf(stderr, "cgrt: CGRT_RELAY_BOOST=%s is neither off nor a threshold num/den (integers, num <= %u, 1 <= den <= %u): the default is used\n",
+                         env_str("CGRT_RELAY_BOOST"), kRelayBoostMaxTerm, kRelayBoostMaxTerm);
+        said = true;
+    }
+    if (*env_str("CGRT_RELAY_BOOST_TILES")) k.relay_boost_tiles = std::max(std::atoll(env_str("CGRT_RELAY_BOOST_TILES")), 0ll);
     return k;
 }
 
@@ -294,6 +339,10 @@
     int relay_extent = kRelayGlass, relay_order = kRelayChunksFirst;
     int relay_start = kRelayStartList, relay_probe_spp = 0;
     size_t relay_start_words = 0;
+    bool relay_boost = false;
+    int boost_k = 0, boost_chunk_spp = 0, boost_slots = 0, boost_wg_slots = 0;
+    size_t boost_cap = 0, boost_bytes = 0, boost_words = 0, boost_grid = 0;
+    uint32_t boost_num = 0, boost_den = 1;
 };
 
 inline bool relay_engaged(int32_t flags, int32_t spp, size_t n_tiles, int n_cu) {
@@ -321,6 +370,16 @@
     if (kn.relay_start >= 0) return kn.relay_start;
     const bool names_order = (flags & CGRT_GRID_RELAY_ORDER_MASK) || kn.relay_order >= 0;
     return !names_order && !(flags & CGRT_GRID_SAMPLE_RELAY) ? kRelayStartCost : kRelayStartList;
+}
+
+static constexpr int kRelayWgPerCu = 4;
+inline bool relay_boost_of(int32_t flags, const EyeKnobs &kn) {
+    if (flags & CGRT_GRID_NO_RELAY_BOOST) return false;
+    if (flags & CGRT_GRID_RELAY_BOOST) return true;
+    if (kn.relay_boost_off) return false;
+    if ((flags & (CGRT_GRID_NO_RELAY_COST_START | CGRT_GRID_RELAY_COST_START)) || kn.relay_start >= 0) return false;
+    const bool names_order = (flags & CGRT_GRID_RELAY_ORDER_MASK) || kn.relay_order >= 0;
+    return !names_order && !(flags & CGRT_GRID_SAMPLE_RELAY);
 }
 
 inline FramePlan frame_plan(const FrameInputs &in, size_t kmax) {
@@ -375,6 +434,24 @@
                 if (p.relay_start == kRelayStartCost) {
                     p.relay_probe_spp = std::min(kn.relay_probe_spp, (int)gr.spp);
                     p.relay_start_words = relay_start_words((size_t)p.tile_blocks, rc.k, p.relay_cap);
+                    const RelayChunks rb = relay_chunks(gr.spp, kRelayMaxChunks);
+                    if (rb.k > rc.k && relay_boost_of(gr.flags, kn) && kn.relay_boost_tiles != 0) {
+                        const int bslots = relay_slots(rb.chunk_spp, gr.max_depth);
+                        const size_t base = align256(p.relay_bytes);
+                        const size_t bcap = relay_cap(p.relay_cap, rb.k, bslots, relay_boost_budget(in.mem_total, base), kn.relay_boost_tiles);
+                        if (bcap > 0) {
+                            p.relay_boost = true;
+                            p.boost_k = rb.k;
+                            p.boost_chunk_spp = rb.chunk_spp;
+                            p.boost_slots = bslots;
+                            p.boost_wg_slots = in.n_cu * kRelayWgPerCu;
+                            p.boost_cap = bcap;
+                            p.boost_bytes = relay_layout(bcap, rb.k, bslots).total;
+                            p.boost_words = p.boost_grid = relay_boost_extra(rc.k, rb.k, bcap);
+                            p.boost_num = kn.relay_boost_num;
+                            p.boost_den = kn.relay_boost_den;
+                        }
+                    }
                 }
             }
         }
diff --git a/cgraytracing_amd/csrc/cgrt_hip.hip b/cgraytracing_amd/csrc/cgrt_hip.hip
--- a/cgraytracing_amd/csrc/cgrt_hip.hip
+++ b/cgraytracing_amd/csrc/cgrt_hip.hip
@@ -828,8 +828,14 @@
     uint32_t *wcost = at.wcost.in<uint32_t>(base), *start = at.start.in<uint32_t>(base);
     unsigned long long *weight = at.weight.in<unsigned long long>(base);
     if (!wcost || !start || !weight) return CGRT_OK;
+    uint32_t *head = at.boost.in<uint32_t>(base), *ecost = at.ecost.in<uint32_t>(base), *bstart = at.bstart.in<uint32_t>(base);
+    unsigned long long *bweight = at.bweight.in<unsigned long long>(base);
+    const bool boost = p.relay_boost && g.boost_k > g.relay_k && head && ecost && bstart && bweight;
+    const RelayBoost rb = boost ? RelayBoost{(uint32_t)p.boost_k, (uint32_t)p.boost_cap, p.boost_chunk_spp, p.boost_num, p.boost_den, (uint32_t)p.boost_wg_slots}
+                                : RelayBoost{};
     const TileOrderState::CostKey ck{g.seed, g.max_depth, p.relay_probe_spp};
-    const TileOrderState::TableKey tk{g.spp, g.relay_k, g.relay_chunk_spp, g.relay_cap, g.relay_extent, 0};
+    const TileOrderState::TableKey tk{g.spp, g.relay_k, g.relay_chunk_spp, g.relay_cap, g.relay_extent, (int32_t)rb.k, (int32_t)rb.cap,
+                                      (int32_t)rb.num, (int32_t)rb.den, (int32_t)rb.slots};
     const bool have_cost = o.reused && o.cost_valid && std::memcmp(&ck, &o.cost_key, sizeof(ck)) == 0;
     const bool have_table = have_cost && o.table_valid && std::memcmp(&tk, &o.table_key, sizeof(tk)) == 0;
     o.cost_valid = o.table_valid = false;
@@ -844,7 +850,7 @@
         gp.tile_order = kOrderFull;
         gp.relay = nullptr;
         gp.relay_k = 0;
-        gp.relay_start_at = 0;
+        gp.relay_start_at = gp.relay_boost_at = 0;
         if (int rc = launch_eye(start_twin(L), false, s->device, gp, dim3((unsigned)p.grid_dim), st, nullptr, nullptr, nullptr)) return rc;
     }
     if (!have_table) {
@@ -852,8 +858,19 @@
         const RelayStartArgs a{RelayItems{(uint32_t)g.relay_k, 0, 0, 0, (uint32_t)g.relay_cap, g.relay_extent, g.relay_chunk_spp, g.spp},
                                (uint32_t)tiles_x, (uint32_t)p.wtiles_x, (uint32_t)p.wtiles_y};
         const dim3 grid((unsigned)((p.relay_start_words + kRelayThreads - 1) / kRelayThreads));
-        hipLaunchKernelGGL(relay_weight_kernel, grid, dim3(kRelayThreads), 0, st, a, g.plan, g.border, wcost, weight);
-        hipLaunchKernelGGL(relay_start_kernel, grid, dim3(kRelayThreads), 0, st, a, g.plan, weight, start);
+        if (boost) {
+            const RelayBoostArgs ba{a, rb};
+            const auto blocks = [](size_t threads) { return dim3((unsigned)((threads + kRelayThreads - 1) / kRelayThreads)); };
+            const size_t n_tiles = (size_t)p.tile_blocks;
+            HIP_TRY(hipMemsetAsync(head, 0, kBoostHead * sizeof(uint32_t), st));
+            hipLaunchKernelGGL(relay_boost_cost_kernel, blocks(n_tiles), dim3(kRelayThreads), 0, st, ba, g.plan, g.border, wcost, ecost, head);
+            hipLaunchKernelGGL(relay_boost_promote_kernel, blocks(p.relay_cap), dim3(kRelayThreads), 0, st, ba, g.plan, ecost, head, head + kBoostHead);
+            hipLaunchKernelGGL(relay_boost_weight_kernel, blocks(n_tiles * rb.k), dim3(kRelayThreads), 0, st, ba, g.plan, ecost, head + kBoostHead, head, bweight);
+            hipLaunchKernelGGL(relay_boost_start_kernel, blocks(n_tiles * rb.k), dim3(kRelayThreads), 0, st, ba, g.plan, bweight, bstart);
+        } else {
+            hipLaunchKernelGGL(relay_weight_kernel, grid, dim3(kRelayThreads), 0, st, a, g.plan, g.border, wcost, weight);
+            hipLaunchKernelGGL(relay_start_kernel, grid, dim3(kRelayThreads), 0, st, a, g.plan, weight, start);
+        }
     }
     if (o.valid && (have_table || (hipPeekAtLastError() == hipSuccess && hipEventRecord(o.ev, st) == hipSuccess))) {
         if (!have_table) o.stream = st;
@@ -864,7 +881,9 @@
         (void)hipGetLastError();
         o.valid = false;
     }
-    g.relay_start_at = (uint32_t)((at.start.at - at.plan.at) / sizeof(uint32_t));
+    g.relay_start_at = (uint32_t)(((boost ? at.bstart.at : at.start.at) - at.plan.at) / sizeof(uint32_t));
+    g.relay_boost_at = boost ? (uint32_t)((at.boost.at - at.plan.at) / sizeof(uint32_t)) : 0u;
+    o.boost = rb;
     o.start_words = p.relay_start_words;
     o.start_wtiles = p.n_wt;
     o.start_reused = have_table;
@@ -950,6 +969,7 @@
             guard.relayed = true;
             n_blocks = relay_grid(p.grid_dim, p.relay_k, p.relay_cap);
             if (p.relay_start == kRelayStartCost && (rc = relay_cost_start(s, L, p, g, st))) return rc;
+            if (g.relay_boost_at) n_blocks += p.boost_grid;
         }
     }
     DevBuf timeline;
@@ -1043,6 +1063,13 @@
     NEED_COMMITTED(s, t && n_wave_tiles && reused);
     ON_DEVICE(s->device);
     return last_relay_start(s->order, s->relay, start, start_cap, wcost, cost_cap, t, n_wave_tiles, reused);
+}
+
+int cgrt_scene_last_relay_boost(const cgrt_scene *s, int64_t *promoted, int32_t *k_boost, int64_t *boost_cap, uint64_t *cost_sum, int32_t *num,
+                                int32_t *den, int32_t *wg_slots, uint32_t *bslot, int64_t slot_cap) {
+    NEED_COMMITTED(s, promoted && k_boost && boost_cap && cost_sum && num && den && wg_slots);
+    ON_DEVICE(s->device);
+    return last_relay_boost(s->order, s->relay, promoted, k_boost, boost_cap, cost_sum, num, den, wg_slots, bslot, slot_cap);
 }
 
 int cgrt_trace_grid_diffuse_variant(const cgrt_scene *s, const cgrt_camera *cam, const cgrt_grid *grid, char *name, size_t cap) {
@@ -1761,6 +1788,35 @@
     return CGRT_OK;
 }
 
+int cgrt_relay_boost_host(int32_t k, int32_t chunk_spp, int32_t spp, int64_t cap, int32_t extent, int64_t n01, int64_t n012, int64_t n_tiles,
+                          const uint32_t *list, const uint32_t *wcost, int32_t width, int32_t rows, int32_t k_boost, int32_t boost_chunk_spp,
+                          int64_t boost_cap, int32_t num, int32_t den, int32_t wg_slots, uint32_t *start, int64_t start_cap, uint32_t *bslot,
+                          int64_t slot_cap, int64_t *t, int64_t *promoted, uint64_t *cost_sum) {
+    if (!t || !promoted || !cost_sum || !list || !wcost || k < 2 || k > kRelayMaxChunks || chunk_spp <= 0 || spp <= 0 || cap < 0 || width <= 0 ||
+        rows <= 0 || n01 < 0 || n01 > n012 || n012 > n_tiles || (size_t)n_tiles >= kRelayStartMaxTiles ||
+        (extent != kRelayGlass && extent != kRelayMirror) || k_boost < k || k_boost > kRelayMaxChunks || boost_chunk_spp <= 0 || boost_cap < 0 ||
+        num < 0 || (uint32_t)num > kRelayBoostMaxTerm || den < 1 || (uint32_t)den > kRelayBoostMaxTerm || wg_slots < 1)
+        return fail(CGRT_ERR_INVALID, "bad argument");
+    const uint32_t tiles_x = (uint32_t)((width + kTileW - 1) / kTileW), tiles_y = (uint32_t)((rows + kTileH - 1) / kTileH);
+    const uint32_t wtiles_x = (uint32_t)((width + kWaveTileW - 1) / kWaveTileW), wtiles_y = (uint32_t)((rows + kWaveTileH - 1) / kWaveTileH);
+    if ((int64_t)tiles_x * tiles_y != n_tiles) return fail(CGRT_ERR_INVALID, "n_tiles is not the grid's tile count");
+    for (int64_t e = 0; e < n012; e++)
+        if (list[e] >= (uint32_t)n_tiles) return fail(CGRT_ERR_INVALID, "list names a tile beyond the grid");
+    const RelayItems r{(uint32_t)k, (uint32_t)n01, (uint32_t)n012, (uint32_t)n_tiles, (uint32_t)std::min<int64_t>(cap, n_tiles), extent, chunk_spp, spp};
+    const RelayBoost b{(uint32_t)k_boost, (uint32_t)std::min<int64_t>(boost_cap, n_tiles), boost_chunk_spp, (uint32_t)num, (uint32_t)den, (uint32_t)wg_slots};
+    const size_t n_split = relay_split_entries(r.n01, r.n012, r.cap, r.extent);
+    const size_t most = relay_items_total(r) + relay_boost_extra(k, k_boost, std::min<size_t>(b.cap, n_split));
+    std::vector<uint64_t> weight(most + 1);
+    std::vector<uint32_t> table(most + 1), slots(n_split + 1);
+    const RelayBoosted out = relay_boost_table(r, b, list, wcost, tiles_x, wtiles_x, wtiles_y, slots.data(), weight.data(), table.data());
+    *t = (int64_t)out.items;
+    *promoted = (int64_t)out.promoted;
+    *cost_sum = out.S;
+    if (start && start_cap >= *t) std::copy(table.begin(), table.begin() + out.items, start);
+    if (bslot && slot_cap >= (int64_t)n_split) std::copy(slots.begin(), slots.begin() + n_split, bslot);
+    return CGRT_OK;
+}
+
 int cgrt_lens_samples(uint64_t seed, const int64_t *pixel, const int32_t *sample, int n, double radius, double *out3) {
     if (n < 0 || (n > 0 && (!pixel || !sample || !out3))) return fail(CGRT_ERR_INVALID, "bad argument");
     for (int i = 0; i < n; i++) {
diff --git a/cgraytracing_amd/csrc/cgrt_relay.h b/cgraytracing_amd/csrc/cgrt_relay.h
--- a/cgraytracing_amd/csrc/cgrt_relay.h
+++ b/cgraytracing_amd/csrc/cgrt_relay.h
@@ -116,6 +116,77 @@
     }
 }
 
+static constexpr uint32_t kRelayBoostMaxTerm = 4096;
+static constexpr uint32_t kRelayBoostNum = 3, kRelayBoostDen = 4;
+static constexpr uint64_t kRelayNoItem = ~(uint64_t)0;
+static_assert(kRelayStartMaxTiles <= ((size_t)1 << 32) - 1, "bslot[e] = boost slot + 1 <= tiles of a table, in a 32-bit word");
+struct RelayBoost {
+    uint32_t k, cap;
+    int32_t chunk_spp;
+    uint32_t num, den, slots;
+};
+CGRT_HD bool relay_boost_candidate(uint32_t cost, const RelayItems &r, const RelayBoost &b, uint64_t S) {
+    return b.k > r.k && (uint64_t)cost * (uint64_t)r.chunk_spp * (uint64_t)b.slots * (uint64_t)b.den > (uint64_t)b.num * S;
+}
+CGRT_HD uint64_t relay_boost_key(bool candidate, uint32_t cost) { return candidate ? (uint64_t)cost + 1u : 0u; }
+CGRT_HD uint32_t relay_boost_chunks(uint32_t e, bool promoted, uint32_t n_split, const RelayItems &r, const RelayBoost &b) {
+    return promoted ? b.k : e < n_split ? r.k : 1u;
+}
+CGRT_HD uint64_t relay_boost_weight(uint32_t c, uint32_t chunks, bool promoted, uint32_t cost, const RelayItems &r, const RelayBoost &b) {
+    if (c >= chunks) return kRelayNoItem;
+    const int32_t cs = promoted ? b.chunk_spp : r.chunk_spp;
+    const int32_t samples = chunks > 1 ? relay_end_sample((int32_t)c, cs, r.spp) - relay_first_sample((int32_t)c, cs) : r.spp;
+    return (uint64_t)cost * (uint64_t)(samples > 0 ? samples : 0);
+}
+CGRT_HD bool relay_boost_before(uint64_t wj, uint32_t j, uint64_t wi, uint32_t i) { return wj != kRelayNoItem && relay_item_before(wj, j, wi, i); }
+CGRT_HD uint32_t relay_boost_items(const RelayItems &r, const RelayBoost &b, uint32_t promoted) { return relay_items_total(r) + (b.k - r.k) * promoted; }
+CGRT_HD size_t relay_boost_extra(int32_t k, int32_t k_boost, size_t cap_boost) { return (size_t)(k_boost - k) * cap_boost; }
+struct RelayBoosted {
+    uint64_t S;
+    uint32_t promoted, items;
+};
+inline RelayBoosted relay_boost_table(const RelayItems &r, const RelayBoost &b, const uint32_t *list, const uint32_t *wcost, uint32_t tiles_x,
+                                      uint32_t wtiles_x, uint32_t wtiles_y, uint32_t *bslot, uint64_t *weight, uint32_t *start) {
+    const uint32_t n_split = relay_split_entries(r.n01, r.n012, r.cap, r.extent);
+    RelayBoosted out{0, 0, 0};
+    for (uint32_t e = 0; e < r.n012; e++) out.S += (uint64_t)relay_tile_cost(wcost, list[e], tiles_x, wtiles_x, wtiles_y) * (uint64_t)r.spp;
+    const auto key = [&](uint32_t e) {
+        const uint32_t c = relay_tile_cost(wcost, list[e], tiles_x, wtiles_x, wtiles_y);
+        return relay_boost_key(relay_boost_candidate(c, r, b, out.S), c);
+    };
+    for (uint32_t e = 0; e < n_split; e++) {
+        const uint64_t ke = key(e);
+        uint32_t rank = 0;
+        for (uint32_t j = 0; j < n_split; j++) rank += relay_item_before(key(j), j, ke, e) ? 1u : 0u;
+        bslot[e] = ke != 0 && rank < b.cap ? rank + 1u : 0u;
+        out.promoted += bslot[e] ? 1u : 0u;
+    }
+    uint32_t t = 0;
+    for (uint32_t e = 0; e < r.n012; e++) {
+        const bool p = e < n_split && bslot[e] != 0;
+        const uint32_t kc = relay_boost_chunks(e, p, n_split, r, b), cost = relay_tile_cost(wcost, list[e], tiles_x, wtiles_x, wtiles_y);
+        for (uint32_t c = 0; c < kc; c++) {
+            weight[t] = relay_boost_weight(c, kc, p, cost, r, b);
+            start[t++] = relay_start_word(RelayBlock{e, (int32_t)c, kc > 1});
+        }
+    }
+    out.items = t;
+    uint32_t *word = new uint32_t[t ? t : 1];
+    for (uint32_t i = 0; i < t; i++) word[i] = start[i];
+    for (uint32_t i = 0; i < t; i++) {
+        uint32_t rank = 0;
+        for (uint32_t j = 0; j < t; j++) rank += relay_item_before(weight[j], j, weight[i], i) ? 1u : 0u;
+        start[rank] = word[i];
+    }
+    delete[] word;
+    return out;
+}
+static constexpr size_t kRelayBoostBudget = (size_t)3 << 30;
+CGRT_HD size_t relay_boost_budget(size_t mem_total, size_t base_bytes) {
+    const size_t left = mem_total / 8 > base_bytes ? mem_total / 8 - base_bytes : 0;
+    return left < kRelayBoostBudget ? left : kRelayBoostBudget;
+}
+
 struct RelayLayout {
     size_t racc, rhits, rcount, rvals, total;
 };
diff --git a/cgraytracing_amd/csrc/cgrt_tile_order.hpp b/cgraytracing_amd/csrc/cgrt_tile_order.hpp
--- a/cgraytracing_amd/csrc/cgrt_tile_order.hpp
+++ b/cgraytracing_amd/csrc/cgrt_tile_order.hpp
@@ -37,17 +37,19 @@
         int32_t max_depth, probe_spp;
     };
     struct TableKey {
-        int32_t spp, k, chunk_spp, cap, extent, pad_;
+        int32_t spp, k, chunk_spp, cap, extent, boost_k, boost_cap, boost_num, boost_den, boost_wg_slots;
     };
-    static_assert(sizeof(CostKey) == 16 && sizeof(TableKey) == 24, "compared as bytes: no padding");
+    static_assert(sizeof(CostKey) == 16 && sizeof(TableKey) == 40, "compared as bytes: no padding");
     CostKey cost_key{};
     TableKey table_key{};
     bool cost_valid = false, table_valid = false, start_reused = false;
     size_t start_words = 0, start_wtiles = 0;
+    RelayBoost boost{};
 
     void begin_launch() {
         tiles = mask_wtiles = sure_wtiles = 0;
         start_words = start_wtiles = 0;
+        boost = RelayBoost{};
         reused = start_reused = false;
         class3 = TileOrderPlan::None;
         lens_stage = kLensStageOff;
@@ -66,6 +68,7 @@
 struct RelayState {
     GrowBuf buf;
     size_t refused = 0, zeroed = 0;
+    size_t boost_zeroed = 0, boost_zeroed_at = 0;
     bool dirty = false;
     hipEvent_t ev = nullptr;
     hipStream_t stream = nullptr;
@@ -74,6 +77,8 @@
         int k = 0;
         size_t cap = 0;
         int slots = 0, extent = 0, order = 0;
+        int boost_k = 0, boost_slots = 0;
+        size_t boost_cap = 0, boost_off = 0;
     } last;
 
     void begin_launch() { last = Last{}; }
@@ -89,7 +94,7 @@
     const int tiles_x = (g.W + kTileW - 1) / kTileW, tiles_y = (g.rows + kTileH - 1) / kTileH;
     const size_t n = (size_t)tiles_x * tiles_y;
     const bool masks = p.order.masks, sure = masks && p.order.sure;
-    const TileOrderLayout at = tile_order_layout(n, p.n_wt, sure, p.relay_start_words);
+    const TileOrderLayout at = tile_order_layout(n, p.n_wt, sure, p.relay_start_words, p.relay_boost ? p.boost_words : 0, p.relay_cap, p.boost_k);
     const bool grown = at.total > o.buf.cap;
     if (grown) o.valid = false;
     if (o.buf.need(at.total) != hipSuccess) {
@@ -146,13 +151,14 @@
 
 static bool relay_prepare(RelayState &r, const FramePlan &p, GridParams &g, Capturing capturing, hipStream_t st) {
     if (capturing != Capturing::None) return false;
-    if (r.refused && p.relay_bytes >= r.refused) return false;
-    if (p.relay_bytes > r.buf.cap) {
+    const size_t boost_at = align256(p.relay_bytes), bytes = p.relay_boost ? boost_at + p.boost_bytes : p.relay_bytes;
+    if (r.refused && bytes >= r.refused) return false;
+    if (bytes > r.buf.cap) {
         if (r.recorded && hipEventSynchronize(r.ev) != hipSuccess) (void)hipGetLastError();
-        r.zeroed = 0;
-        if (r.buf.need(p.relay_bytes) != hipSuccess) {
+        r.zeroed = r.boost_zeroed = 0;
+        if (r.buf.need(bytes) != hipSuccess) {
             (void)hipGetLastError();
-            r.refused = p.relay_bytes;
+            r.refused = bytes;
             return false;
         }
     }
@@ -172,6 +178,23 @@
         }
     }
     r.zeroed = p.relay_cap;
+    if (p.relay_boost) {
+        if (r.dirty || boost_at != r.boost_zeroed_at || p.boost_cap > r.boost_zeroed) {
+            if (hipMemsetAsync(reinterpret_cast<unsigned char *>(r.buf.p) + boost_at, 0, p.boost_cap * sizeof(uint32_t), st) != hipSuccess) {
+                (void)hipGetLastError();
+                return false;
+            }
+        }
+        r.boost_zeroed = p.boost_cap;
+        r.boost_zeroed_at = boost_at;
+        g.relay_boost_off = boost_at;
+        g.boost_k = p.boost_k;
+        g.boost_chunk_spp = p.boost_chunk_spp;
+        g.boost_cap = (int32_t)p.boost_cap;
+        g.boost_slots = p.boost_slots;
+    } else {
+        r.boost_zeroed = 0;
+    }
     r.dirty = true;
     g.relay = reinterpret_cast<unsigned char *>(r.buf.p);
     g.relay_k = p.relay_k;
@@ -202,6 +225,12 @@
             relay.stream = st;
             relay.recorded = true;
             relay.last = RelayState::Last{g.relay_k, (size_t)g.relay_cap, g.relay_slots, g.relay_extent, g.relay_order};
+            if (g.relay_boost_at) {
+                relay.last.boost_k = g.boost_k;
+                relay.last.boost_slots = g.boost_slots;
+                relay.last.boost_cap = (size_t)g.boost_cap;
+                relay.last.boost_off = (size_t)g.relay_boost_off;
+            }
             relay.dirty = false;
         }
         through = true;
@@ -261,7 +290,45 @@
     std::vector<uint32_t> cnt(n_split * (size_t)(l.k - 1) * kRelayThreads);
     const RelayLayout rl = relay_layout(l.cap, l.k, l.slots);
     HIP_TRY(hipMemcpy(cnt.data(), reinterpret_cast<const unsigned char *>(r.buf.p) + rl.rcount, cnt.size() * sizeof(uint32_t), hipMemcpyDeviceToHost));
-    for (uint32_t c : cnt) *parked_values += (int64_t)c;
+    if (l.boost_k == 0 || o.boost.k == 0) {
+        for (uint32_t c : cnt) *parked_values += (int64_t)c;
+        return CGRT_OK;
+    }
+    std::vector<uint32_t> bslot(n_split);
+    if (int rc = o.read(Region{o.at.boost.at + kBoostHead * sizeof(uint32_t), 0}, bslot.data(), n_split)) return rc;
+    const size_t per = (size_t)(l.boost_k - 1) * kRelayThreads;
+    std::vector<uint32_t> bcnt(l.boost_cap * per);
+    const RelayLayout bl = relay_layout(l.boost_cap, l.boost_k, l.boost_slots);
+    HIP_TRY(hipMemcpy(bcnt.data(), reinterpret_cast<const unsigned char *>(r.buf.p) + l.boost_off + bl.rcount, bcnt.size() * sizeof(uint32_t), hipMemcpyDeviceToHost));
+    for (size_t e = 0; e < n_split; e++) {
+        if (bslot[e] == 0) {
+            for (size_t i = 0; i < (size_t)(l.k - 1) * kRelayThreads; i++) *parked_values += (int64_t)cnt[e * (size_t)(l.k - 1) * kRelayThreads + i];
+        } else if (bslot[e] <= l.boost_cap) {
+            for (size_t i = 0; i < per; i++) *parked_values += (int64_t)bcnt[(size_t)(bslot[e] - 1) * per + i];
+        }
+    }
+    return CGRT_OK;
+}
+static int last_relay_boost(const TileOrderState &o, const RelayState &r, int64_t *promoted, int32_t *k_boost, int64_t *boost_cap, uint64_t *cost_sum,
+                            int32_t *num, int32_t *den, int32_t *wg_slots, uint32_t *bslot, int64_t slot_cap) {
+    *promoted = *boost_cap = 0;
+    *k_boost = *num = *den = *wg_slots = 0;
+    *cost_sum = 0;
+    if (o.boost.k == 0 || r.last.boost_k == 0 || o.start_words == 0 || o.tiles == 0) return CGRT_OK;
+    uint32_t plan[kOrderClasses + 1], head[kBoostHead];
+    HIP_TRY(hipDeviceSynchronize());
+    if (int rc = o.read(o.at.plan, plan, kOrderClasses + 1)) return rc;
+    if (int rc = o.read(o.at.boost, head, kBoostHead)) return rc;
+    *promoted = (int64_t)head[kBoostPromoted];
+    *k_boost = (int32_t)o.boost.k;
+    *boost_cap = (int64_t)o.boost.cap;
+    *cost_sum = (uint64_t)head[kBoostS] | (uint64_t)head[kBoostS + 1] << 32;
+    *num = (int32_t)o.boost.num;
+    *den = (int32_t)o.boost.den;
+    *wg_slots = (int32_t)o.boost.slots;
+    const size_t n_split = relay_split_entries(plan[2], plan[3], (uint32_t)r.last.cap, r.last.extent);
+    if (bslot && n_split > 0 && slot_cap >= (int64_t)n_split)
+        return o.read(Region{o.at.boost.at + kBoostHead * sizeof(uint32_t), 0}, bslot, n_split);
     return CGRT_OK;
 }
 static int last_relay_start(const TileOrderState &o, const RelayState &r, uint32_t *start, int64_t start_cap, uint32_t *wcost, int64_t cost_cap,
@@ -273,13 +340,20 @@
     HIP_TRY(hipDeviceSynchronize());
     if (int rc = o.read(o.at.plan, plan, kOrderClasses + 1)) return rc;
     const RelayItems ri{(uint32_t)r.last.k, plan[2], plan[3], plan[kOrderClasses], (uint32_t)r.last.cap, r.last.extent, 0, 0};
-    const size_t n = relay_items_total(ri);
-    if (n > o.start_words) return fail(CGRT_ERR_DEVICE, "relay start table: more workgroups than the table holds");
+    size_t n = relay_items_total(ri);
+    const bool boosted = o.boost.k != 0 && r.last.boost_k != 0;
+    if (boosted) {
+        uint32_t head[kBoostHead];
+        if (int rc = o.read(o.at.boost, head, kBoostHead)) return rc;
+        n = head[kBoostItems];
+    }
+    if (n > (boosted ? o.at.bstart.bytes / sizeof(uint32_t) : o.start_words))
+        return fail(CGRT_ERR_DEVICE, "relay start table: more workgroups than the table holds");
     *t = (int64_t)n;
     *n_wave_tiles = (int64_t)o.start_wtiles;
     *reused = o.start_reused ? 1 : 0;
     if (start && start_cap >= (int64_t)n && n > 0)
-        if (int rc = o.read(o.at.start, start, n)) return rc;
+        if (int rc = o.read(boosted ? o.at.bstart : o.at.start, start, n)) return rc;
     if (wcost && cost_cap >= (int64_t)o.start_wtiles && o.start_wtiles > 0)
         if (int rc = o.read(o.at.wcost, wcost, o.start_wtiles)) return rc;
     return CGRT_OK;
diff --git a/cgraytracing_amd/engine.py b/cgraytracing_amd/engine.py
--- a/cgraytracing_amd/engine.py
+++ b/cgraytracing_amd/engine.py
@@ -24,8 +24,10 @@
 _RELAY_STARTS = ("list", "cost")
 
 
-def _relay_flag(sample_relay, relay_mirror=None, relay_order=None, relay_start=None):
+def _relay_flag(sample_relay, relay_mirror=None, relay_order=None, relay_start=None, relay_boost=None):
     form = 0 if relay_mirror is None else (8192 if relay_mirror else 16384)
+    if relay_boost is not None:
+        form |= 2097152 if relay_boost else 4194304
     if relay_start is not None:
         if relay_start not in _RELAY_STARTS:
             raise ValueError("relay_start: None, " + ", ".join(repr(o) for o in _RELAY_STARTS))
@@ -41,6 +43,21 @@
     if int(sample_relay) not in (2, 4):
         raise ValueError("sample_relay: None, True, False, 2 or 4")
     return form | 1024 | (4096 if int(sample_relay) == 4 else 0)
+
+
+def relay_boost_host(k, chunk_spp, spp, cap, mirror, plan, tile_list, wcost, width, rows, k_boost, boost_chunk_spp, boost_cap, num, den,
+                     wg_slots):
+    lib = _capi.lib()
+    lst, wc = np.ascontiguousarray(tile_list, np.uint32), np.ascontiguousarray(wcost, np.uint32)
+    assert wc.size == ((width + 15) // 16) * ((rows + 3) // 4) and lst.size == int(plan[4])
+    args = (int(k), int(chunk_spp), int(spp), int(cap), 1 if mirror else 0, int(plan[2]), int(plan[3]), int(plan[4]), lst.ctypes.data,
+            wc.ctypes.data, int(width), int(rows), int(k_boost), int(boost_chunk_spp), int(boost_cap), int(num), int(den), int(wg_slots))
+    t, p, S = C.c_int64(), C.c_int64(), C.c_uint64()
+    n_split = min(int(plan[3]) if mirror else int(plan[2]), int(cap))
+    start = np.zeros(max(int(plan[3]) + (int(k_boost) - 1) * n_split, 1), np.uint32)
+    bslot = np.zeros(max(n_split, 1), np.uint32)
+    check(lib.cgrt_relay_boost_host(*args, start.ctypes.data, start.size, bslot.ctypes.data, bslot.size, C.byref(t), C.byref(p), C.byref(S)))
+    return dict(start=start[:t.value], bslot=bslot[:n_split], promoted=int(p.value), S=int(S.value))
 
 
 def relay_start_host(k, chunk_spp, spp, cap, mirror, plan, tile_list, wcost, width, rows):
@@ -186,7 +203,7 @@
                    stripe=None, sample_offset=0, spp_total=None, out=None, nhit=None, counters=None, stream=None,
                    stats=False, accumulate=False, split_samples=False, reorder=True, force_reorder=False, tile_order=True,
                    diffuse_tiles=False, sphere_pairs=True, sphere_masks=True, sample_relay=None,
-                   relay_mirror=None, relay_order=None, lens_stage=True, sure_tiles=True, relay_start=None):
+                   relay_mirror=None, relay_order=None, lens_stage=True, sure_tiles=True, relay_start=None, relay_boost=None):
         import torch
 
         rows = height - row_offset if rows is None else rows
@@ -203,7 +220,7 @@
         cc, g = self._structs(camera, width, height, rows, spp, max_depth, seed, row_offset, stripe, sample_offset,
                               spp_total, (1 if stats else 0) | (2 if accumulate else 0) | (4 if split_samples else 0) |
                               (0 if reorder else 8) | (16 if force_reorder else 0) | (0 if tile_order else 64) |
-                              (128 if diffuse_tiles else 0) | (0 if sphere_pairs else 256) | (0 if sphere_masks else 512) | _relay_flag(sample_relay, relay_mirror, relay_order, relay_start) |
+                              (128 if diffuse_tiles else 0) | (0 if sphere_pairs else 256) | (0 if sphere_masks else 512) | _relay_flag(sample_relay, relay_mirror, relay_order, relay_start, relay_boost) |
                               (0 if lens_stage else 131072) | (0 if sure_tiles else 262144))
         st = stream if stream is not None else torch.cuda.current_stream(dev).cuda_stream
         check(self._L.cgrt_trace_grid(self._h, C.byref(cc), C.byref(g), out.data_ptr(),
@@ -458,7 +475,7 @@
     def trace_grid_host(self, width, height, spp=1, camera=None, max_depth=5, seed=12345, rows=None, row_offset=0,
                         stripe=None, sample_offset=0, spp_total=None, stats=False, split_samples=False, reorder=True,
                         force_reorder=False, tile_order=True, diffuse_tiles=False, sphere_pairs=True, sphere_masks=True, sample_relay=None,
-                        relay_mirror=None, relay_order=None, lens_stage=True, sure_tiles=True, relay_start=None):
+                        relay_mirror=None, relay_order=None, lens_stage=True, sure_tiles=True, relay_start=None, relay_boost=None):
         rows = height - row_offset if rows is None else rows
         rgb = np.zeros((rows, width, 3), np.float32)
         nhit = np.zeros((rows, width), np.uint32)
@@ -466,7 +483,7 @@
         cc, g = self._structs(camera, width, height, rows, spp, max_depth, seed, row_offset, stripe, sample_offset,
                               spp_total, (1 if stats else 0) | (4 if split_samples else 0) | (0 if reorder else 8) |
                               (16 if force_reorder else 0) | (0 if tile_order else 64) | (128 if diffuse_tiles else 0) |
-                              (0 if sphere_pairs else 256) | (0 if sphere_masks else 512) | _relay_flag(sample_relay, relay_mirror, relay_order, relay_start) |
+                              (0 if sphere_pairs else 256) | (0 if sphere_masks else 512) | _relay_flag(sample_relay, relay_mirror, relay_order, relay_start, relay_boost) |
                               (0 if lens_stage else 131072) | (0 if sure_tiles else 262144))
         check(self._L.cgrt_trace_grid_host(self._h, C.byref(cc), C.byref(g), rgb.ctypes.data, nhit.ctypes.data,
                                            cnt.ctypes.data))
@@ -524,6 +541,18 @@
         check(self._L.cgrt_scene_last_relay_start(self._h, start.ctypes.data, start.size, wcost.ctypes.data, n.value, C.byref(t),
                                                   C.byref(n), C.byref(r)))
         return dict(t=int(t.value), start=start[:t.value], wcost=wcost, reused=bool(r.value))
+
+    def last_relay_boost(self):
+        p, k, cap, S = C.c_int64(), C.c_int32(), C.c_int64(), C.c_uint64()
+        num, den, ws = C.c_int32(), C.c_int32(), C.c_int32()
+        tiles = self.last_sample_relay()["tiles"]
+        bslot = np.zeros(max(tiles, 1), np.uint32)
+        check(self._L.cgrt_scene_last_relay_boost(self._h, C.byref(p), C.byref(k), C.byref(cap), C.byref(S), C.byref(num), C.byref(den),
+                                                  C.byref(ws), bslot.ctypes.data, bslot.size))
+        if k.value == 0:
+            return None
+        return dict(promoted=int(p.value), k_boost=int(k.value), boost_cap=int(cap.value), S=int(S.value), num=int(num.value),
+                    den=int(den.value), wg_slots=int(ws.value), bslot=bslot[:tiles])
 
     def last_lens_stage(self):
         a, b = C.c_int64(), C.c_int64()
diff --git a/include/cgrt.h b/include/cgrt.h
--- a/include/cgrt.h
+++ b/include/cgrt.h
@@ -63,6 +63,8 @@
     CGRT_GRID_RELAY_ORDER_MASK = 98304,
     CGRT_GRID_RELAY_COST_START = 524288,
     CGRT_GRID_NO_RELAY_COST_START = 1048576,
+    CGRT_GRID_RELAY_BOOST = 2097152,
+    CGRT_GRID_NO_RELAY_BOOST = 4194304,
     CGRT_GRID_NO_LENS_STAGE = 131072,
     CGRT_GRID_NO_SURE_TILES = 262144,
     CGRT_GRID_HITPOINTS = 32,
@@ -306,6 +308,13 @@
                           const uint32_t *list, const uint32_t *wcost, int32_t width, int32_t rows, uint32_t *start, int64_t start_cap,
                           int64_t *t);
 
+int cgrt_scene_last_relay_boost(const cgrt_scene *s, int64_t *promoted, int32_t *k_boost, int64_t *boost_cap, uint64_t *cost_sum,
+                                int32_t *num, int32_t *den, int32_t *wg_slots, uint32_t *bslot, int64_t slot_cap);
+int cgrt_relay_boost_host(int32_t k, int32_t chunk_spp, int32_t spp, int64_t cap, int32_t extent, int64_t n01, int64_t n012, int64_t n_tiles,
+                          const uint32_t *list, const uint32_t *wcost, int32_t width, int32_t rows, int32_t k_boost, int32_t boost_chunk_spp,
+                          int64_t boost_cap, int32_t num, int32_t den, int32_t wg_slots, uint32_t *start, int64_t start_cap, uint32_t *bslot,
+                          int64_t slot_cap, int64_t *t, int64_t *promoted, uint64_t *cost_sum);
+
 int cgrt_lens_samples(uint64_t seed, const int64_t *pixel, const int32_t *sample, int n, double radius, double *out3);
 
 enum { CGRT_PROBE_SQRT = 0, CGRT_PROBE_NORMALIZED = 1, CGRT_PROBE_SPHERE_LEN = 2, CGRT_PROBE_SPHERE_LEN_PAIR = 4  };
```

Result: faster. 108,000, median of 6 (+8.4%).
